# YHY138/Boosting-Fine-grained-Feature-Fusion-in-3D-Point-Cloud-Registration

Hardware: AMD Instinct MI355X
Metric: point-cloud pairs/sec (forward) on ModelNet 2048-pt pairs (higher is better)
Workload: dtype f32 (emulated on the fp16 MFMA pipe: f16x3 split products); 1 GPU; ModelNet40 2048-pt pairs, 8 pairs per GPU (BASELINE configs[1] at N=1, configs[3] at N=8); pairs_per_gpu=8, global_batch=8, points_per_cloud=717, parallelism=pair-sharded dp1, precision=fp32

## Files before the change

boosting-fine-grained-feature-fusion-in-3d-point-cloud-registration_amd/csrc/ffn.hip:

```cpp
#include <algorithm>
#include <cstdlib>

#include "mfma.h"

namespace fgr {
namespace {

constexpr int kFfnD = 256;
constexpr int kFfnKS = kFfnD / 32;
constexpr int kFfnNP = kFfnD / 16;
constexpr int kFfnMaxF = 2048;
constexpr int kUnit = 1024;
constexpr int kRing = 8;
static_assert(kFfnKS * 128 == kUnit, "a W1 panel is one ring unit");
static_assert(kFfnNP / 2 * 128 == kUnit, "half of a chunk's W2 slice is one ring unit");

struct FfnArgs {
    const float* x; int64_t ldx;
    const float* ln_g; const float* ln_b; float eps;
    const u32x4* w1; const float* wsc1; const float* b1;
    const u32x4* w2; const float* wsc2; const float* b2;
    const float* bound;
    float* out; int64_t ldo;
    int M, F;
};

__device__ __forceinline__ void wait_units(int n) {
    static_assert(kRing - 2 <= 6, "extend the switch");
    switch (n) {
        case 0: wait_vm_lgkm0<0>(); break;
        case 1: wait_vm_lgkm0<4>(); break;
        case 2: wait_vm_lgkm0<8>(); break;
        case 3: wait_vm_lgkm0<12>(); break;
        case 4: wait_vm_lgkm0<16>(); break;
        case 5: wait_vm_lgkm0<20>(); break;
        default: wait_vm_lgkm0<24>(); break;
    }
}

typedef __attribute__((address_space(3))) u32x4 lds_u4;

__shared__ u32x4 g_ffn_ring0[kUnit], g_ffn_ring1[kUnit], g_ffn_ring2[kUnit], g_ffn_ring3[kUnit],
                 g_ffn_ring4[kUnit], g_ffn_ring5[kUnit], g_ffn_ring6[kUnit], g_ffn_ring7[kUnit];
static_assert(kRing == 8, "one object per slot below");

__device__ __forceinline__ u32x4* ring_slot(int s) {
    switch (s & 7) {
        case 0: return g_ffn_ring0; case 1: return g_ffn_ring1;
        case 2: return g_ffn_ring2; case 3: return g_ffn_ring3;
        case 4: return g_ffn_ring4; case 5: return g_ffn_ring5;
        case 6: return g_ffn_ring6; default: return g_ffn_ring7;
    }
}

__device__ __forceinline__ void read_issue(const u32x4* slot, int lane_u, u32x4 (&r)[16]) {
    const uint32_t a = (uint32_t)(uintptr_t)((const lds_u4*)slot + lane_u);
    asm volatile(
        "ds_read_b128 %0, %16 offset:0\n\t"
        "ds_read_b128 %1, %16 offset:1024\n\t"
        "ds_read_b128 %2, %16 offset:2048\n\t"
        "ds_read_b128 %3, %16 offset:3072\n\t"
        "ds_read_b128 %4, %16 offset:4096\n\t"
        "ds_read_b128 %5, %16 offset:5120\n\t"
        "ds_read_b128 %6, %16 offset:6144\n\t"
        "ds_read_b128 %7, %16 offset:7168\n\t"
        "ds_read_b128 %8, %16 offset:8192\n\t"
        "ds_read_b128 %9, %16 offset:9216\n\t"
        "ds_read_b128 %10, %16 offset:10240\n\t"
        "ds_read_b128 %11, %16 offset:11264\n\t"
        "ds_read_b128 %12, %16 offset:12288\n\t"
        "ds_read_b128 %13, %16 offset:13312\n\t"
        "ds_read_b128 %14, %16 offset:14336\n\t"
        "ds_read_b128 %15, %16 offset:15360"
        : "=&v"(r[0]), "=&v"(r[1]), "=&v"(r[2]), "=&v"(r[3]), "=&v"(r[4]), "=&v"(r[5]),
          "=&v"(r[6]), "=&v"(r[7]), "=&v"(r[8]), "=&v"(r[9]), "=&v"(r[10]), "=&v"(r[11]),
          "=&v"(r[12]), "=&v"(r[13]), "=&v"(r[14]), "=&v"(r[15])
        : "v"(a)
        : "memory");
}
__device__ __forceinline__ void read_wait(u32x4 (&r)[16]) {
    asm volatile("s_waitcnt lgkmcnt(0)"
                 : "+v"(r[0]), "+v"(r[1]), "+v"(r[2]), "+v"(r[3]), "+v"(r[4]), "+v"(r[5]),
                   "+v"(r[6]), "+v"(r[7]), "+v"(r[8]), "+v"(r[9]), "+v"(r[10]), "+v"(r[11]),
                   "+v"(r[12]), "+v"(r[13]), "+v"(r[14]), "+v"(r[15])
                 :
                 : "memory");
}
__device__ __forceinline__ f16x8 frag(const u32x4 (&r)[16], int j, int t) {
    return __builtin_bit_cast(f16x8, r[2 * j + t]);
}

__global__ void __launch_bounds__(256, 1) ffn_f16x3_kernel(FfnArgs p) {
    __shared__ float4 cw1[kFfnMaxF / 4], cb1[kFfnMaxF / 4];
    __shared__ float4 cw2[kFfnD / 4], cb2[kFfnD / 4];
    __shared__ float4 lng[kFfnD / 4], lnb[kFfnD / 4];

    const int nbm = (p.M + 63) / 64;
    const int t = xcd_tile(blockIdx.x, nbm);
    const int tid = threadIdx.x, wv = tid >> 6, lane = tid & 63;
    const int g = lane >> 4, c = lane & 15;
    const int mw = t * 64 + wv * 16;
    const int64_t row = min(mw + c, p.M - 1);
    const int nch = p.F / 32;
    const int nu = 4 * nch;

    float xr[kFfnKS][8];
    {
        const float* ar = p.x + row * p.ldx;
#pragma unroll
        for (int s = 0; s < kFfnKS; ++s) {
            const float4 a0 = *reinterpret_cast<const float4*>(ar + 32 * s + 8 * g);
            const float4 a1 = *reinterpret_cast<const float4*>(ar + 32 * s + 8 * g + 4);
            xr[s][0] = a0.x; xr[s][1] = a0.y; xr[s][2] = a0.z; xr[s][3] = a0.w;
            xr[s][4] = a1.x; xr[s][5] = a1.y; xr[s][6] = a1.z; xr[s][7] = a1.w;
        }
    }
    const int nf4 = p.F / 4;
    static_assert(kFfnMaxF / 4 == 2 * 256, "two float4 per thread");
    const int j0 = min(tid, nf4 - 1), j1 = min(tid + 256, nf4 - 1);
    const float4 pw1a = reinterpret_cast<const float4*>(p.wsc1)[j0];
    const float4 pb1a = reinterpret_cast<const float4*>(p.b1)[j0];
    const float4 pw1b = reinterpret_cast<const float4*>(p.wsc1)[j1];
    const float4 pb1b = reinterpret_cast<const float4*>(p.b1)[j1];
    const int t4 = tid & (kFfnD / 4 - 1);
    const float4 pw2 = reinterpret_cast<const float4*>(p.wsc2)[t4];
    const float4 pb2 = reinterpret_cast<const float4*>(p.b2)[t4];
    const float4 pg = reinterpret_cast<const float4*>(p.ln_g)[t4];
    const float4 pbe = reinterpret_cast<const float4*>(p.ln_b)[t4];
    const float bM1 = p.bound[0], bMb = p.bound[1];

    auto unit_src = [&](int u) -> const u32x4* {
        const int ch = u >> 2, j = u & 3;
        return j < 2 ? p.w1 + (int64_t)(2 * ch + j) * kUnit
                     : p.w2 + (int64_t)ch * (2 * kUnit) + (j - 2) * kUnit;
    };
    auto dma = [&](int u, int slot) {
        const u32x4* src = unit_src(u) + wv * 64 + lane;
        __attribute__((address_space(3))) char* dst =
            (__attribute__((address_space(3))) char*)(lds_u4*)ring_slot(slot) + wv * 1024;
#pragma unroll
        for (int j = 0; j < 4; ++j)
            __builtin_amdgcn_global_load_lds((const void*)(src + j * 256),
                                             (__attribute__((address_space(3))) void*)(dst + j * 4096),
                                             16, 0, 0);
    };
#pragma unroll
    for (int u = 0; u < kRing; ++u) dma(u, u);
    wait_vm_lgkm0<4 * kRing>();
    if (tid < nf4) { cw1[tid] = pw1a; cb1[tid] = pb1a; }
    if (tid + 256 < nf4) { cw1[tid + 256] = pw1b; cb1[tid + 256] = pb1b; }
    if (tid < kFfnD / 4) { cw2[tid] = pw2; cb2[tid] = pb2; lng[tid] = pg; lnb[tid] = pbe; }
    wait_vm_lgkm0<4 * kRing - 4>();
    __builtin_amdgcn_s_barrier();
    const int lane_u = g * 16 + c;
    u32x4 wa[16], wb[16];
    read_issue(ring_slot(0), lane_u, wa);

    f16x8 af[kFfnKS][2];
    float rsS, inv_s;
    {
        float sm = 0.f;
#pragma unroll
        for (int s = 0; s < kFfnKS; ++s)
            sm += ((xr[s][0] + xr[s][1]) + (xr[s][2] + xr[s][3])) +
                  ((xr[s][4] + xr[s][5]) + (xr[s][6] + xr[s][7]));
        const float mean = xg_sum(sm) / (float)kFfnD;
        float sq = 0.f;
#pragma unroll
        for (int s = 0; s < kFfnKS; ++s)
#pragma unroll
            for (int e = 0; e < 8; ++e) {
                const float d = xr[s][e] - mean;
                sq += d * d;
            }
        const float rstd = 1.0f / sqrtf(xg_sum(sq) / (float)kFfnD + p.eps);
        float mx = 0.f, nn = 0.f;
#pragma unroll
        for (int s = 0; s < kFfnKS; ++s) {
            const int k = 32 * s + 8 * g;
            const float4 g0 = lng[k / 4], g1 = lng[k / 4 + 1];
            const float4 b0 = lnb[k / 4], b1 = lnb[k / 4 + 1];
            const float gg[8] = {g0.x, g0.y, g0.z, g0.w, g1.x, g1.y, g1.z, g1.w};
            const float bb[8] = {b0.x, b0.y, b0.z, b0.w, b1.x, b1.y, b1.z, b1.w};
#pragma unroll
            for (int e = 0; e < 8; ++e) {
                const float a = (xr[s][e] - mean) * rstd * gg[e] + bb[e];
                xr[s][e] = a;
                nn = fmaf(a, a, nn);
            }
            mx = fmaxf(mx, max3_abs(xr[s][0], xr[s][1], xr[s][2]));
            mx = fmaxf(mx, max3_abs(xr[s][3], xr[s][4], xr[s][5]));
            mx = fmaxf(mx, max3_abs(xr[s][6], xr[s][7], 0.f));
        }
        mx = xg_max(mx);
        nn = xg_sum(nn);
        const int ea = row_scale_exp(mx);
        const float sca = __builtin_ldexpf(1.f, ea);
#pragma unroll
        for (int s = 0; s < kFfnKS; ++s) {
            u32x4 h, l;
            split8_f16(xr[s], sca, h, l);
            af[s][0] = __builtin_bit_cast(f16x8, h);
            af[s][1] = __builtin_bit_cast(f16x8, l);
        }
        const float bnd = sqrtf(nn) * bM1 + bMb;
        const int eh = bnd > 0.f ? max(min(15 - __builtin_amdgcn_frexp_expf(bnd), 127), -126) : 0;
        rsS = __builtin_ldexpf(1.f, eh - ea);
        inv_s = __builtin_ldexpf(1.f, -eh);
    }
    const float sS = inv_s > 0.f ? 1.f / inv_s : 1.f;

    f32x4 accy[kFfnNP];
#pragma unroll
    for (int q = 0; q < kFfnNP; ++q) accy[q] = f32x4{0.f, 0.f, 0.f, 0.f};
    f32x4 acc1[2];
    f16x8 hb[2];
    read_wait(wa);
    for (int ch2 = 0; ch2 < nch; ch2 += 2) {
#pragma unroll
        for (int jj = 0; jj < 8; ++jj) {
            const int j = jj & 3, ch = ch2 + (jj >> 2);
            const int u = 4 * ch2 + jj;
            u32x4 (&cur)[16] = (jj & 1) ? wb : wa;
            u32x4 (&nxt)[16] = (jj & 1) ? wa : wb;
            const bool more = u + 1 < nu;
            if (more) {
                wait_units(min(kRing - 2, nu - 2 - u));
                __builtin_amdgcn_s_barrier();
                if (u + kRing < nu) dma(u + kRing, jj);
                read_issue(ring_slot(jj + 1), lane_u, nxt);
            }
            __builtin_amdgcn_sched_barrier(0);
            if (j < 2) {
                f32x4 a = f32x4{0.f, 0.f, 0.f, 0.f};
#pragma unroll
                for (int s = 0; s < kFfnKS; ++s) {
                    a = __builtin_amdgcn_mfma_f32_16x16x32_f16(frag(cur, s, 1), af[s][0], a, 0, 0, 0);
                    a = __builtin_amdgcn_mfma_f32_16x16x32_f16(frag(cur, s, 0), af[s][1], a, 0, 0, 0);
                    a = __builtin_amdgcn_mfma_f32_16x16x32_f16(frag(cur, s, 0), af[s][0], a, 0, 0, 0);
                }
                acc1[j] = a;
                if (j == 1) {
                    float hv[8];
#pragma unroll
                    for (int pp = 0; pp < 2; ++pp) {
                        const int n = 32 * ch + 16 * pp + 4 * g;
                        const float4 w4 = cw1[n / 4], b4 = cb1[n / 4];
                        hv[4 * pp + 0] = fmaxf(fmaf(acc1[pp][0], rsS * w4.x, sS * b4.x), 0.f);
                        hv[4 * pp + 1] = fmaxf(fmaf(acc1[pp][1], rsS * w4.y, sS * b4.y), 0.f);
                        hv[4 * pp + 2] = fmaxf(fmaf(acc1[pp][2], rsS * w4.z, sS * b4.z), 0.f);
                        hv[4 * pp + 3] = fmaxf(fmaf(acc1[pp][3], rsS * w4.w, sS * b4.w), 0.f);
                    }
                    u32x4 h, l;
                    split8_f16(hv, 1.f, h, l);
                    hb[0] = __builtin_bit_cast(f16x8, h);
                    hb[1] = __builtin_bit_cast(f16x8, l);
                }
            } else {
#pragma unroll
                for (int qq = 0; qq < 8; ++qq) {
                    const int q = 8 * (j - 2) + qq;
                    accy[q] = __builtin_amdgcn_mfma_f32_16x16x32_f16(frag(cur, qq, 1), hb[0], accy[q], 0, 0, 0);
                    accy[q] = __builtin_amdgcn_mfma_f32_16x16x32_f16(frag(cur, qq, 0), hb[1], accy[q], 0, 0, 0);
                    accy[q] = __builtin_amdgcn_mfma_f32_16x16x32_f16(frag(cur, qq, 0), hb[0], accy[q], 0, 0, 0);
                }
            }
            __builtin_amdgcn_sched_barrier(0);
            if (more) read_wait(nxt);
        }
    }

    const bool ok = mw + c < p.M;
    const float* xrow = p.x + row * p.ldx;
    float4 res[kFfnNP];
#pragma unroll
    for (int q = 0; q < kFfnNP; ++q) res[q] = *reinterpret_cast<const float4*>(xrow + 16 * q + 4 * g);
    float* orow = p.out + row * p.ldo;
#pragma unroll
    for (int q = 0; q < kFfnNP; ++q) {
        const int n = 16 * q + 4 * g;
        const float4 w4 = cw2[n / 4], b4 = cb2[n / 4];
        const float4 y = make_float4(fmaf(accy[q][0], w4.x * inv_s, b4.x) + res[q].x,
                                     fmaf(accy[q][1], w4.y * inv_s, b4.y) + res[q].y,
                                     fmaf(accy[q][2], w4.z * inv_s, b4.z) + res[q].z,
                                     fmaf(accy[q][3], w4.w * inv_s, b4.w) + res[q].w);
        if (ok) *reinterpret_cast<float4*>(orow + n) = y;
    }
}

constexpr int kV2Groups = 16;
constexpr int kCusFfn = 256;
#ifndef FGR_FFN_RING
#define FGR_FFN_RING 4
#endif
constexpr int kV2Ring = FGR_FFN_RING;
static_assert(kV2Groups % kV2Ring == 0, "ring slot = group index mod kV2Ring at compile time");

__device__ __forceinline__ void wait_vm_only(int n) {
    switch (n) {
        case 0: wait_vm<0>(); break;   case 4: wait_vm<4>(); break;
        case 8: wait_vm<8>(); break;   case 12: wait_vm<12>(); break;
        case 16: wait_vm<16>(); break; case 20: wait_vm<20>(); break;
        case 24: wait_vm<24>(); break; default: wait_vm<28>(); break;
    }
}

__device__ __forceinline__ float gelu_scaled(float sz, float isq) {
    const float a = sz * isq, t = fabsf(a), s = a * a;
    float r = fmaf(-1.72853470e-5f, t, 3.83197126e-4f);
    const float u = fmaf(-3.88396438e-3f, t, 2.42546219e-2f);
    r = fmaf(r, s, u);
    r = fmaf(r, t, -1.06777877e-1f);
    r = fmaf(r, t, -6.34846687e-1f);
    r = fmaf(r, t, -1.28717512e-1f);
    r = fmaf(r, t, -t);
    const float e = 0.5f * __expf(r);
    const float tail = a < 0.f ? e : 1.f - e;
    float q = -5.96761703e-4f;
    q = fmaf(q, s, 4.99119423e-3f);
    q = fmaf(q, s, -2.67681349e-2f);
    q = fmaf(q, s, 1.12819925e-1f);
    q = fmaf(q, s, -3.76125336e-1f);
    q = fmaf(q, s, 1.28379166e-1f);
    const float mid = fmaf(0.5f, fmaf(q, a, a), 0.5f);
    return sz * (t > 0.927734375f ? tail : mid);
}

template <int RT, int ACT = FGR_ACT_RELU>
__global__ void __launch_bounds__(256, 1) ffn_nsplit_kernel(FfnArgs p) {
    static_assert(RT >= 1 && RT <= 4, "row tiles");
    static_assert(ACT == FGR_ACT_RELU || ACT == FGR_ACT_GELU, "activation");
    __shared__ u32x4 act[RT * kFfnKS * 2 * 64];
    __shared__ u32x4 hbuf[2][4][RT][2][64];
    __shared__ float4 cw1[kFfnMaxF / 4], cb1[kFfnMaxF / 4];
    __shared__ float4 cw2[kFfnD / 4], cb2[kFfnD / 4];
    __shared__ float4 lng[kFfnD / 4], lnb[kFfnD / 4];
    __shared__ float2 rowpar[64];

    constexpr int BR = 16 * RT;
    const int nbm = (p.M + BR - 1) / BR;
    const int t = xcd_tile(blockIdx.x, nbm);
    const int tid = threadIdx.x, wv = tid >> 6, lane = tid & 63;
    const int g = lane >> 4, c = lane & 15;
    const int r0 = t * BR;
    const int nst = p.F / 128;

    const int nf4 = p.F / 4;
    const int j0 = min(tid, nf4 - 1), j1 = min(tid + 256, nf4 - 1);
    const float4 pw1a = reinterpret_cast<const float4*>(p.wsc1)[j0];
    const float4 pb1a = reinterpret_cast<const float4*>(p.b1)[j0];
    const float4 pw1b = reinterpret_cast<const float4*>(p.wsc1)[j1];
    const float4 pb1b = reinterpret_cast<const float4*>(p.b1)[j1];
    const int t4 = tid & (kFfnD / 4 - 1);
    const float4 pw2 = reinterpret_cast<const float4*>(p.wsc2)[t4];
    const float4 pb2 = reinterpret_cast<const float4*>(p.b2)[t4];
    const float4 pg = reinterpret_cast<const float4*>(p.ln_g)[t4];
    const float4 pbe = reinterpret_cast<const float4*>(p.ln_b)[t4];
    __builtin_amdgcn_sched_barrier(0);
    float xr[kFfnKS][8];
    {
        const int64_t row = min(r0 + 16 * min(wv, RT - 1) + c, p.M - 1);
        const float* ar = p.x + row * p.ldx;
#pragma unroll
        for (int s = 0; s < kFfnKS; ++s) {
            const float4 a0 = *reinterpret_cast<const float4*>(ar + 32 * s + 8 * g);
            const float4 a1 = *reinterpret_cast<const float4*>(ar + 32 * s + 8 * g + 4);
            xr[s][0] = a0.x; xr[s][1] = a0.y; xr[s][2] = a0.z; xr[s][3] = a0.w;
            xr[s][4] = a1.x; xr[s][5] = a1.y; xr[s][6] = a1.z; xr[s][7] = a1.w;
        }
    }
    {
        if (tid < nf4) { cw1[tid] = pw1a; cb1[tid] = pb1a; }
        if (tid + 256 < nf4) { cw1[tid + 256] = pw1b; cb1[tid + 256] = pb1b; }
        if (tid < kFfnD / 4) { cw2[tid] = pw2; cb2[tid] = pb2; lng[tid] = pg; lnb[tid] = pbe; }
    }
    const float bM1 = p.bound[0], bMb = p.bound[1];
    __syncthreads();

    {
        float sm = 0.f;
#pragma unroll
        for (int s = 0; s < kFfnKS; ++s)
            sm += ((xr[s][0] + xr[s][1]) + (xr[s][2] + xr[s][3])) +
                  ((xr[s][4] + xr[s][5]) + (xr[s][6] + xr[s][7]));
        const float mean = xg_sum(sm) / (float)kFfnD;
        float sq = 0.f;
#pragma unroll
        for (int s = 0; s < kFfnKS; ++s)
#pragma unroll
            for (int e = 0; e < 8; ++e) {
                const float d = xr[s][e] - mean;
                sq += d * d;
            }
        const float rstd = 1.0f / sqrtf(xg_sum(sq) / (float)kFfnD + p.eps);
        float mx = 0.f, nn = 0.f;
#pragma unroll
        for (int s = 0; s < kFfnKS; ++s) {
            const int k = 32 * s + 8 * g;
            const float4 g0 = lng[k / 4], g1 = lng[k / 4 + 1];
            const float4 b0 = lnb[k / 4], b1 = lnb[k / 4 + 1];
            const float gg[8] = {g0.x, g0.y, g0.z, g0.w, g1.x, g1.y, g1.z, g1.w};
            const float bb[8] = {b0.x, b0.y, b0.z, b0.w, b1.x, b1.y, b1.z, b1.w};
#pragma unroll
            for (int e = 0; e < 8; ++e) {
                const float a = (xr[s][e] - mean) * rstd * gg[e] + bb[e];
                xr[s][e] = a;
                nn = fmaf(a, a, nn);
            }
            mx = fmaxf(mx, max3_abs(xr[s][0], xr[s][1], xr[s][2]));
            mx = fmaxf(mx, max3_abs(xr[s][3], xr[s][4], xr[s][5]));
            mx = fmaxf(mx, max3_abs(xr[s][6], xr[s][7], 0.f));
        }
        mx = xg_max(mx);
        nn = xg_sum(nn);
        const int ea = row_scale_exp(mx);
        const float sca = __builtin_ldexpf(1.f, ea);
        if (wv < RT) {
#pragma unroll
            for (int s = 0; s < kFfnKS; ++s) {
                u32x4 h, l;
                split8_f16(xr[s], sca, h, l);
                act[((wv * kFfnKS + s) * 2 + 0) * 64 + lane] = h;
                act[((wv * kFfnKS + s) * 2 + 1) * 64 + lane] = l;
            }
        }
        const float bnd = sqrtf(nn) * bM1 + bMb;
        const int eh = bnd > 0.f ? max(min(15 - __builtin_amdgcn_frexp_expf(bnd), 127), -126) : 0;
        if (g == 0 && wv < RT)
            rowpar[16 * wv + c] = make_float2(__builtin_ldexpf(1.f, eh - ea), __builtin_ldexpf(1.f, eh));
    }
    __syncthreads();

    auto issue = [&](int st, int j, u32x4 (&slot)[4]) {
        if (j < 8) {
            const int ch = 4 * st + wv;
#pragma unroll
            for (int e = 0; e < 4; ++e) {
                const int pp = e >> 1, tt = e & 1;
                slot[e] = p.w1[(int64_t)(2 * ch + pp) * kUnit + (j * 2 + tt) * 64 + lane];
            }
        } else {
            const int ch = 4 * st + ((j - 8) >> 1), q0 = 4 * wv + 2 * ((j - 8) & 1);
#pragma unroll
            for (int e = 0; e < 4; ++e) {
                const int qq = e >> 1, tt = e & 1;
                slot[e] = p.w2[((int64_t)(ch * kFfnNP + q0 + qq) * 2 + tt) * 64 + lane];
            }
        }
    };
    u32x4 ring[kV2Ring][4];
    f32x4 accy[RT][4];
#pragma unroll
    for (int rt = 0; rt < RT; ++rt)
#pragma unroll
        for (int q = 0; q < 4; ++q) accy[rt][q] = f32x4{0.f, 0.f, 0.f, 0.f};
#pragma unroll
    for (int j = 0; j < kV2Ring - 1; ++j) issue(0, j, ring[j]);
    u32x4 fa[2][2 * RT];
    auto read_act = [&](int s, u32x4 (&f)[2 * RT]) {
#pragma unroll
        for (int rt = 0; rt < RT; ++rt) {
            f[2 * rt + 0] = act[((rt * kFfnKS + s) * 2 + 0) * 64 + lane];
            f[2 * rt + 1] = act[((rt * kFfnKS + s) * 2 + 1) * 64 + lane];
        }
    };
    auto read_h = [&](int buf, int sw, u32x4 (&f)[2 * RT]) {
#pragma unroll
        for (int rt = 0; rt < RT; ++rt) {
            f[2 * rt + 0] = hbuf[buf][sw][rt][0][lane];
            f[2 * rt + 1] = hbuf[buf][sw][rt][1][lane];
        }
    };

    for (int st = 0; st < nst; ++st) {
        const int ch = 4 * st + wv;
        const int stn = min(st + 1, nst - 1);
        f32x4 acc1[RT][2];
#pragma unroll
        for (int rt = 0; rt < RT; ++rt) acc1[rt][0] = acc1[rt][1] = f32x4{0.f, 0.f, 0.f, 0.f};
        read_act(0, fa[0]);
#pragma unroll
        for (int j = 0; j < kV2Groups; ++j) {
            const int jn = j + kV2Ring - 1;
            issue(jn < kV2Groups ? st : stn, jn % kV2Groups, ring[jn % kV2Ring]);
            wait_vm_only(4 * (kV2Ring - 1));
            u32x4 (&wf)[4] = ring[j % kV2Ring];
            if (j < 8) {
                u32x4 (&cur)[2 * RT] = fa[j & 1];
                if (j < 7) read_act(j + 1, fa[(j + 1) & 1]);
                __builtin_amdgcn_sched_group_barrier(0x020, 4, 0);
                if (j < 7) __builtin_amdgcn_sched_group_barrier(0x100, 2 * RT, 0);
#pragma unroll
                for (int rt = 0; rt < RT; ++rt) {
                    const f16x8 ah = __builtin_bit_cast(f16x8, cur[2 * rt + 0]);
                    const f16x8 al = __builtin_bit_cast(f16x8, cur[2 * rt + 1]);
#pragma unroll
                    for (int pp = 0; pp < 2; ++pp) {
                        const f16x8 wh = __builtin_bit_cast(f16x8, wf[2 * pp]);
                        const f16x8 wl = __builtin_bit_cast(f16x8, wf[2 * pp + 1]);
                        acc1[rt][pp] = __builtin_amdgcn_mfma_f32_16x16x32_f16(wl, ah, acc1[rt][pp], 0, 0, 0);
                        acc1[rt][pp] = __builtin_amdgcn_mfma_f32_16x16x32_f16(wh, al, acc1[rt][pp], 0, 0, 0);
                        acc1[rt][pp] = __builtin_amdgcn_mfma_f32_16x16x32_f16(wh, ah, acc1[rt][pp], 0, 0, 0);
                    }
                }
                __builtin_amdgcn_sched_group_barrier(0x008, 6 * RT, 0);
                __builtin_amdgcn_sched_barrier(0);
                if (j == 7) {
#pragma unroll
                    for (int rt = 0; rt < RT; ++rt) {
                        const float2 rp = rowpar[16 * rt + c];
                        float hv[8];
#pragma unroll
                        for (int pp = 0; pp < 2; ++pp) {
                            const int n = 32 * ch + 16 * pp + 4 * g;
                            const float4 w4 = cw1[n / 4], b4 = cb1[n / 4];
                            if constexpr (ACT == FGR_ACT_RELU) {
                                hv[4 * pp + 0] = fmaxf(fmaf(acc1[rt][pp][0], rp.x * w4.x, rp.y * b4.x), 0.f);
                                hv[4 * pp + 1] = fmaxf(fmaf(acc1[rt][pp][1], rp.x * w4.y, rp.y * b4.y), 0.f);
                                hv[4 * pp + 2] = fmaxf(fmaf(acc1[rt][pp][2], rp.x * w4.z, rp.y * b4.z), 0.f);
                                hv[4 * pp + 3] = fmaxf(fmaf(acc1[rt][pp][3], rp.x * w4.w, rp.y * b4.w), 0.f);
                            } else {
                                const float isq =
                                    __builtin_ldexpf(0.70710678118654752440f,
                                                     1 - __builtin_amdgcn_frexp_expf(rp.y));
                                hv[4 * pp + 0] = gelu_scaled(fmaf(acc1[rt][pp][0], rp.x * w4.x, rp.y * b4.x), isq);
                                hv[4 * pp + 1] = gelu_scaled(fmaf(acc1[rt][pp][1], rp.x * w4.y, rp.y * b4.y), isq);
                                hv[4 * pp + 2] = gelu_scaled(fmaf(acc1[rt][pp][2], rp.x * w4.z, rp.y * b4.z), isq);
                                hv[4 * pp + 3] = gelu_scaled(fmaf(acc1[rt][pp][3], rp.x * w4.w, rp.y * b4.w), isq);
                            }
                        }
                        u32x4 h, l;
                        split8_f16(hv, 1.f, h, l);
                        hbuf[st & 1][wv][rt][0][lane] = h;
                        hbuf[st & 1][wv][rt][1][lane] = l;
                    }
                    wait_lgkm0();
                    __builtin_amdgcn_s_barrier();
                    read_h(st & 1, 0, fa[0]);
                }
            } else {
                const int sw = (j - 8) >> 1, qh = (j - 8) & 1;
                u32x4 (&cur)[2 * RT] = fa[sw & 1];
                const bool pre = qh == 0 && sw < 3;
                if (pre) read_h(st & 1, sw + 1, fa[(sw + 1) & 1]);
                __builtin_amdgcn_sched_group_barrier(0x020, 4, 0);
                if (pre) __builtin_amdgcn_sched_group_barrier(0x100, 2 * RT, 0);
#pragma unroll
                for (int rt = 0; rt < RT; ++rt) {
                    const f16x8 hh = __builtin_bit_cast(f16x8, cur[2 * rt + 0]);
                    const f16x8 hl = __builtin_bit_cast(f16x8, cur[2 * rt + 1]);
#pragma unroll
                    for (int qq = 0; qq < 2; ++qq) {
                        const f16x8 wh = __builtin_bit_cast(f16x8, wf[2 * qq]);
                        const f16x8 wl = __builtin_bit_cast(f16x8, wf[2 * qq + 1]);
                        f32x4& a = accy[rt][2 * qh + qq];
                        a = __builtin_amdgcn_mfma_f32_16x16x32_f16(wl, hh, a, 0, 0, 0);
                        a = __builtin_amdgcn_mfma_f32_16x16x32_f16(wh, hl, a, 0, 0, 0);
                        a = __builtin_amdgcn_mfma_f32_16x16x32_f16(wh, hh, a, 0, 0, 0);
                    }
                }
                __builtin_amdgcn_sched_group_barrier(0x008, 6 * RT, 0);
                __builtin_amdgcn_sched_barrier(0);
            }
        }
    }
    wait_vm_only(0);

#pragma unroll
    for (int rt = 0; rt < RT; ++rt) {
        const int rr = r0 + 16 * rt + c;
        const int64_t row = min(rr, p.M - 1);
        const float inv_s = 1.f / rowpar[16 * rt + c].y;
        const float* xrow = p.x + row * p.ldx;
        float4 res[4];
#pragma unroll
        for (int q = 0; q < 4; ++q) res[q] = *reinterpret_cast<const float4*>(xrow + 16 * (4 * wv + q) + 4 * g);
        float* orow = p.out + row * p.ldo;
#pragma unroll
        for (int q = 0; q < 4; ++q) {
            const int n = 16 * (4 * wv + q) + 4 * g;
            const float4 w4 = cw2[n / 4], b4 = cb2[n / 4];
            const float4 y = make_float4(fmaf(accy[rt][q][0], w4.x * inv_s, b4.x) + res[q].x,
                                         fmaf(accy[rt][q][1], w4.y * inv_s, b4.y) + res[q].y,
                                         fmaf(accy[rt][q][2], w4.z * inv_s, b4.z) + res[q].z,
                                         fmaf(accy[rt][q][3], w4.w * inv_s, b4.w) + res[q].w);
            if (rr < p.M) *reinterpret_cast<float4*>(orow + n) = y;
        }
    }
}

__global__ void __launch_bounds__(256)
ffn_w2_split_kernel(const float* __restrict__ w, int n, int f, int64_t sn, int64_t sk,
                    float* __restrict__ wsc, u32x4* __restrict__ img) {
    const int tid = threadIdx.x, q = blockIdx.x, r0 = q * 16;
    const int ri = tid >> 4, kl = tid & 15;
    float mx = 0.f;
    if (r0 + ri < n)
        for (int j = kl; j < f; j += 16) mx = fmaxf(mx, fabsf(w[(int64_t)(r0 + ri) * sn + (int64_t)j * sk]));
    __shared__ float red[16][17];
    __shared__ float scale_inv[16];
    red[ri][kl] = mx;
    __syncthreads();
    if (tid < 16) {
        float m = 0.f;
#pragma unroll
        for (int z = 0; z < 16; ++z) m = fmaxf(m, red[tid][z]);
        const int e = row_scale_exp(m);
        const bool ok = r0 + tid < n;
        scale_inv[tid] = ok ? __builtin_ldexpf(1.f, e) : 0.f;
        wsc[r0 + tid] = ok ? __builtin_ldexpf(1.f, -e) : 0.f;
    }
    __syncthreads();
    const int np = (n + 15) / 16, units = (f / 32) * 128;
    for (int u = tid; u < units; u += 256) {
        const int i = u & 15, gg = (u >> 4) & 3, t = (u >> 6) & 1, cc = u >> 7;
        const int rr = r0 + i;
        const float sc = scale_inv[i];
        f16x8 out;
#pragma unroll
        for (int e = 0; e < 8; ++e) {
            const int col = 32 * cc + 16 * (e >> 2) + 4 * gg + (e & 3);
            const float v = rr < n ? w[(int64_t)rr * sn + (int64_t)col * sk] * sc : 0.f;
            const _Float16 h = (_Float16)v;
            out[e] = t == 0 ? h : (_Float16)(v - (float)h);
        }
        img[((int64_t)cc * np + q) * 128 + (u & 127)] = __builtin_bit_cast(u32x4, out);
    }
}

size_t ffn_image_bytes(int n, int f) { return (size_t)(f / 32) * ((n + 15) / 16) * 128 * 16; }

}
}

using namespace fgr;

extern "C" int fgr_split_weights_ffn2_bytes(int32_t n, int32_t k, size_t* bytes) {
    FGR_REQUIRE(bytes && n > 0 && k > 0 && k % 32 == 0,
                "fgr_split_weights_ffn2_bytes: bad arguments (n %d, k %d: k %% 32 == 0)", n, k);
    *bytes = ffn_image_bytes(n, k) + (size_t)((n + 15) / 16) * 16 * sizeof(float);
    return FGR_OK;
}

extern "C" int fgr_split_weights_ffn2(const float* w, int32_t n, int32_t k, int64_t stride_n,
                                      int64_t stride_k, void* img, void* stream) {
    FGR_REQUIRE(w && img && n > 0 && k > 0 && k % 32 == 0,
                "fgr_split_weights_ffn2: bad arguments (n %d, k %d)", n, k);
    FGR_REQUIRE((reinterpret_cast<uintptr_t>(img) & 15) == 0,
                "fgr_split_weights_ffn2: image not 16-B aligned");
    float* wsc = reinterpret_cast<float*>(static_cast<char*>(img) + ffn_image_bytes(n, k));
    hipLaunchKernelGGL(ffn_w2_split_kernel, dim3((unsigned)((n + 15) / 16)), dim3(256), 0,
                       as_stream(stream), w, n, k, stride_n, stride_k, wsc, (u32x4*)img);
    FGR_CHECK_LAUNCH("ffn_w2_split_kernel");
    return FGR_OK;
}

extern "C" int fgr_ffn_f16x3_supported(int32_t m, int32_t d, int32_t f) {
    return (m > 0 && d == kFfnD && f >= 64 && f % 64 == 0 && f <= kFfnMaxF) ? 1 : 0;
}

extern "C" int fgr_ffn_f16x3_act_supported(int32_t m, int32_t d, int32_t f, int32_t act) {
    if (act == FGR_ACT_RELU) return fgr_ffn_f16x3_supported(m, d, f);
    if (act == FGR_ACT_GELU) return (fgr_ffn_f16x3_supported(m, d, f) && f % 128 == 0) ? 1 : 0;
    return 0;
}

extern "C" int fgr_ffn_f16x3(const float* x, int64_t ldx, const float* gamma, const float* beta,
                             float eps, const void* w1_img, const float* b1, const void* w2_img,
                             const float* b2, const float* bound, float* out, int64_t ldo,
                             int32_t m, int32_t d, int32_t f, void* stream) {
    return fgr_ffn_f16x3_act(x, ldx, gamma, beta, eps, w1_img, b1, w2_img, b2, bound, out, ldo, m,
                             d, f, FGR_ACT_RELU, stream);
}

extern "C" int fgr_ffn_f16x3_act(const float* x, int64_t ldx, const float* gamma,
                                 const float* beta, float eps, const void* w1_img, const float* b1,
                                 const void* w2_img, const float* b2, const float* bound,
                                 float* out, int64_t ldo, int32_t m, int32_t d, int32_t f,
                                 int32_t act, void* stream) {
    FGR_REQUIRE(act == FGR_ACT_RELU || act == FGR_ACT_GELU,
                "fgr_ffn_f16x3_act: act %d (FGR_ACT_RELU or FGR_ACT_GELU)", act);
    FGR_REQUIRE(x && gamma && beta && w1_img && b1 && w2_img && b2 && bound && out && m >= 0 &&
                    ldx >= d && ldo >= d && eps >= 0.f,
                "fgr_ffn_f16x3: bad arguments");
    FGR_REQUIRE(m == 0 || fgr_ffn_f16x3_act_supported(m, d, f, act),
                "fgr_ffn_f16x3: d %d, hidden %d, act %d not supported (fgr_ffn_f16x3_act_supported)",
                d, f, act);
    const uintptr_t al = reinterpret_cast<uintptr_t>(x) | reinterpret_cast<uintptr_t>(gamma) |
                         reinterpret_cast<uintptr_t>(beta) | reinterpret_cast<uintptr_t>(w1_img) |
                         reinterpret_cast<uintptr_t>(b1) | reinterpret_cast<uintptr_t>(w2_img) |
                         reinterpret_cast<uintptr_t>(b2) | reinterpret_cast<uintptr_t>(out);
    FGR_REQUIRE((al & 15) == 0 && ldx % 4 == 0 && ldo % 4 == 0,
                "fgr_ffn_f16x3: operands must be 16-B aligned with row strides %% 4 == 0");
    FGR_REQUIRE(out + (size_t)m * ldo <= x || x + (size_t)m * ldx <= out || out == x,
                "fgr_ffn_f16x3: out overlaps x partially");
    if (m == 0) return FGR_OK;
    hipStream_t st = as_stream(stream);
    TimedCall timed_(st);
    const char* i1 = static_cast<const char*>(w1_img);
    const char* i2 = static_cast<const char*>(w2_img);
    FfnArgs a{x, ldx, gamma, beta, eps,
              (const u32x4*)i1, (const float*)(i1 + (size_t)(f / 16) * kFfnKS * 128 * 16), b1,
              (const u32x4*)i2, (const float*)(i2 + ffn_image_bytes(d, f)), b2,
              bound, out, ldo, m, f};
    const bool rt3 = (m + 47) / 48 <= kCusFfn && (m + 63) / 64 < kCusFfn;
    if (act == FGR_ACT_GELU) {
        const unsigned nb = (unsigned)((m + 47) / 48);
        hipLaunchKernelGGL((ffn_nsplit_kernel<3, FGR_ACT_GELU>), dim3(nb), dim3(256), 0, st, a);
    } else if (f % 128 == 0) {
        if (rt3)
            hipLaunchKernelGGL(ffn_nsplit_kernel<3>, dim3((unsigned)((m + 47) / 48)), dim3(256), 0, st, a);
        else
            hipLaunchKernelGGL(ffn_nsplit_kernel<4>, dim3((unsigned)((m + 63) / 64)), dim3(256), 0, st, a);
    } else
        hipLaunchKernelGGL(ffn_f16x3_kernel, dim3((unsigned)((m + 63) / 64)), dim3(256), 0, st, a);
    FGR_CHECK_LAUNCH("ffn_f16x3_kernel");
    return FGR_OK;
}
```

boosting-fine-grained-feature-fusion-in-3d-point-cloud-registration_amd/csrc/gemm_ws.hip:

```cpp
#include "mfma.h"


namespace fgr {
namespace {

constexpr int kWsKS = 8;
constexpr int kWsPanelU = kWsKS * 128;
#ifndef FGR_WS_RING
#define FGR_WS_RING 3
#endif
constexpr int kWsRing = FGR_WS_RING;
static_assert(kWsRing >= 2 && kWsRing <= 8, "vmcnt holds at most 63");
constexpr int kKvUnitsWs = 1024;
constexpr int kKvUnitVWs = 512;

struct WsArgs {
    const float* A; int64_t lda;
    const u32x4* W; const float* wsc; const float* bias;
    float* C; int64_t ldc;
    const float* R; int64_t ldr;
    int M, N;
    const float* ln_g; const float* ln_b; float eps;
    const float* add; int64_t ld_add;
    const float* g2; const float* b2; float* out2; int64_t ld_out2;
    char* kv_img; int2* kv_sc; int n_head, kv_col0;
};

__device__ __forceinline__ void wait_groups_ws(int n) {
    switch (n) {
        case 0: wait_vm<0>(); break;   case 1: wait_vm<8>(); break;
        case 2: wait_vm<16>(); break;  case 3: wait_vm<24>(); break;
        case 4: wait_vm<32>(); break;  case 5: wait_vm<40>(); break;
        case 6: wait_vm<48>(); break;  default: wait_vm<56>(); break;
    }
}

template <int NPW, int LNM, bool KV, bool RES, int ACT, int RT, int NPART>
__global__ void __launch_bounds__(256) __attribute__((amdgpu_waves_per_eu((NPART > 1 && !RES) ? 2 : 1)))
gemm_ws_kernel(WsArgs p) {
    static_assert(NPW % 4 == 0, "passes of 4 panels");
    static_assert(RT >= 1 && RT <= 4 && (!KV || RT == 4), "row tiles (K / V images: 64-row tiles)");
    constexpr int BR = 16 * RT;
    static_assert(!KV || (LNM >= 2 && !RES && ACT == FGR_ACT_NONE), "K / V images: the in_proj");
    constexpr int NPASS = NPW / 4;
    constexpr int N = 64 * NPW;
    constexpr bool kResEarly = RES && NPASS == 1;
    __shared__ u32x4 act[RT * kWsKS * 2 * 64];
    __shared__ float rowrs[BR];
    __shared__ float4 colw[N / 4], colb[N / 4];
    __shared__ float4 lng[LNM ? 64 : 1], lnb[LNM ? 64 : 1];
    __shared__ float4 lng2[LNM == 3 ? 64 : 1], lnb2[LNM == 3 ? 64 : 1];
    constexpr bool kSideLds = LNM == 3 && NPART == 1;
    __shared__ float4 side[kSideLds ? BR * 64 : 1];

    const int nblk = (p.M + BR - 1) / BR * NPART;
    int t = xcd_tile(blockIdx.x, nblk);
    const int part = t % NPART;
    t /= NPART;
    const int cb4 = part * (N / 4);
    const int tid = threadIdx.x, wv = tid >> 6, lane = tid & 63;
    const int g = lane >> 4, c = lane & 15;
    const int r0 = t * BR;
    const int rrow = r0 + 16 * min(wv, RT - 1) + c;
    const int64_t row = min(rrow, p.M - 1);
    const int pw0 = part * 4 * NPW + wv * NPW;

    float4 lpg = make_float4(0.f, 0.f, 0.f, 0.f), lpb = lpg, lpg2 = lpg, lpb2 = lpg;
    if constexpr (LNM > 0) {
        const int t4 = tid & 63;
        lpg = reinterpret_cast<const float4*>(p.ln_g)[t4];
        lpb = reinterpret_cast<const float4*>(p.ln_b)[t4];
        if constexpr (LNM == 3) {
            lpg2 = reinterpret_cast<const float4*>(p.g2)[t4];
            lpb2 = reinterpret_cast<const float4*>(p.b2)[t4];
        }
    }
    constexpr int NC4 = (N / 4 + 255) / 256;
    float4 pcw[NC4], pcb[NC4];
#pragma unroll
    for (int i = 0; i < NC4; ++i) {
        const int j = min(tid + 256 * i, N / 4 - 1);
        pcw[i] = reinterpret_cast<const float4*>(p.wsc)[cb4 + j];
        pcb[i] = p.bias ? reinterpret_cast<const float4*>(p.bias)[cb4 + j] : make_float4(0.f, 0.f, 0.f, 0.f);
    }
    __builtin_amdgcn_sched_barrier(0);
    float xr[kWsKS][8];
    float dr[LNM >= 2 ? kWsKS : 1][8];
    {
        const float* ar = p.A + row * p.lda;
#pragma unroll
        for (int s = 0; s < kWsKS; ++s) {
            const float4 a0 = *reinterpret_cast<const float4*>(ar + 32 * s + 8 * g);
            const float4 a1 = *reinterpret_cast<const float4*>(ar + 32 * s + 8 * g + 4);
            xr[s][0] = a0.x; xr[s][1] = a0.y; xr[s][2] = a0.z; xr[s][3] = a0.w;
            xr[s][4] = a1.x; xr[s][5] = a1.y; xr[s][6] = a1.z; xr[s][7] = a1.w;
        }
        if constexpr (LNM >= 2) {
            const float* dp = p.add + row * p.ld_add;
#pragma unroll
            for (int s = 0; s < kWsKS; ++s) {
                const float4 d0 = *reinterpret_cast<const float4*>(dp + 32 * s + 8 * g);
                const float4 d1 = *reinterpret_cast<const float4*>(dp + 32 * s + 8 * g + 4);
                dr[s][0] = d0.x; dr[s][1] = d0.y; dr[s][2] = d0.z; dr[s][3] = d0.w;
                dr[s][4] = d1.x; dr[s][5] = d1.y; dr[s][6] = d1.z; dr[s][7] = d1.w;
            }
        }
    }
    float4 rres[kResEarly ? RT : 1][4];
    if constexpr (kResEarly) {
        const int col0 = pw0 * 16;
#pragma unroll
        for (int rt = 0; rt < RT; ++rt) {
            const int64_t orow = min(r0 + 16 * rt + c, p.M - 1);
#pragma unroll
            for (int pp = 0; pp < 4; ++pp)
                rres[rt][pp] = *reinterpret_cast<const float4*>(p.R + orow * p.ldr + col0 + 16 * pp + 4 * g);
        }
    }
    __builtin_amdgcn_sched_barrier(0);
    auto issue = [&](int G, u32x4 (&slot)[8]) {
        const int pass = G / kWsKS, s = G % kWsKS;
#pragma unroll
        for (int e = 0; e < 8; ++e) {
            const int pp = e >> 1, tt = e & 1;
            slot[e] = p.W[(int64_t)(pw0 + 4 * pass + pp) * kWsPanelU + (s * 2 + tt) * 64 + lane];
        }
    };
    constexpr int NG = NPASS * kWsKS;
    u32x4 ring[kWsRing][8];
#pragma unroll
    for (int G = 0; G < kWsRing - 1; ++G) issue(G, ring[G]);
    __builtin_amdgcn_sched_barrier(0);

#pragma unroll
    for (int i = 0; i < NC4; ++i) {
        const int j = tid + 256 * i;
        if (j < N / 4) { colw[j] = pcw[i]; colb[j] = pcb[i]; }
    }
    float ln_mean = 0.f, ln_rstd = 0.f;
    if constexpr (LNM > 0) {
        if (tid < 64) { lng[tid] = lpg; lnb[tid] = lpb; }
        if constexpr (LNM == 3)
            if (tid < 64) { lng2[tid] = lpg2; lnb2[tid] = lpb2; }
        __syncthreads();
        float sm = 0.f;
#pragma unroll
        for (int s = 0; s < kWsKS; ++s)
            sm += ((xr[s][0] + xr[s][1]) + (xr[s][2] + xr[s][3])) +
                  ((xr[s][4] + xr[s][5]) + (xr[s][6] + xr[s][7]));
        const float mean = xg_sum(sm) / 256.f;
        float sq = 0.f;
#pragma unroll
        for (int s = 0; s < kWsKS; ++s)
#pragma unroll
            for (int e = 0; e < 8; ++e) {
                const float d = xr[s][e] - mean;
                sq += d * d;
            }
        const float rstd = 1.0f / sqrtf(xg_sum(sq) / 256.f + p.eps);
        ln_mean = mean;
        ln_rstd = rstd;
        if (kSideLds && wv < RT) {
#pragma unroll
            for (int s = 0; s < kWsKS; ++s) {
                const int k = 32 * s + 8 * g;
                const float4 h0 = lng2[k / 4], h1 = lng2[k / 4 + 1];
                const float4 c0 = lnb2[k / 4], c1 = lnb2[k / 4 + 1];
                float4* o2 = side + (16 * wv + c) * 64 + k / 4;
                o2[0] = make_float4((xr[s][0] - mean) * rstd * h0.x + c0.x, (xr[s][1] - mean) * rstd * h0.y + c0.y,
                                    (xr[s][2] - mean) * rstd * h0.z + c0.z, (xr[s][3] - mean) * rstd * h0.w + c0.w);
                o2[1] = make_float4((xr[s][4] - mean) * rstd * h1.x + c1.x, (xr[s][5] - mean) * rstd * h1.y + c1.y,
                                    (xr[s][6] - mean) * rstd * h1.z + c1.z, (xr[s][7] - mean) * rstd * h1.w + c1.w);
            }
        }
#pragma unroll
        for (int s = 0; s < kWsKS; ++s) {
            const int k = 32 * s + 8 * g;
            const float4 g0 = lng[k / 4], g1 = lng[k / 4 + 1];
            const float4 b0 = lnb[k / 4], b1 = lnb[k / 4 + 1];
            const float gg[8] = {g0.x, g0.y, g0.z, g0.w, g1.x, g1.y, g1.z, g1.w};
            const float bb[8] = {b0.x, b0.y, b0.z, b0.w, b1.x, b1.y, b1.z, b1.w};
#pragma unroll
            for (int e = 0; e < 8; ++e) {
                xr[s][e] = (xr[s][e] - mean) * rstd * gg[e] + bb[e];
                if constexpr (LNM >= 2) xr[s][e] += dr[s][e];
            }
        }
    }
    {
        float mx = 0.f;
#pragma unroll
        for (int s = 0; s < kWsKS; ++s) {
            mx = fmaxf(mx, max3_abs(xr[s][0], xr[s][1], xr[s][2]));
            mx = fmaxf(mx, max3_abs(xr[s][3], xr[s][4], xr[s][5]));
            mx = fmaxf(mx, max3_abs(xr[s][6], xr[s][7], 0.f));
        }
        mx = xg_max(mx);
        const int e = row_scale_exp(mx);
        const float sc = __builtin_ldexpf(1.f, e);
        if (wv < RT) {
#pragma unroll
            for (int s = 0; s < kWsKS; ++s) {
                u32x4 h, l;
                split8_f16(xr[s], sc, h, l);
                act[((wv * kWsKS + s) * 2 + 0) * 64 + lane] = h;
                act[((wv * kWsKS + s) * 2 + 1) * 64 + lane] = l;
            }
            if (g == 0) rowrs[16 * wv + c] = __builtin_ldexpf(1.f, -e);
        }
    }
    wait_lgkm0();
    __builtin_amdgcn_s_barrier();

    auto read_act = [&](int s, u32x4 (&f)[2 * RT]) {
#pragma unroll
        for (int rt = 0; rt < RT; ++rt) {
            f[2 * rt + 0] = act[((rt * kWsKS + s) * 2 + 0) * 64 + lane];
            f[2 * rt + 1] = act[((rt * kWsKS + s) * 2 + 1) * 64 + lane];
        }
    };
    u32x4 fa[2][2 * RT];
    u32x4 fin[NPASS][RT][4];
    int kv_e[NPASS][2];
    float rs[RT];
#pragma unroll
    for (int pass = 0; pass < NPASS; ++pass) {
        const int col0 = (pw0 + 4 * pass) * 16;
        const bool kvp = KV && col0 >= p.kv_col0;
        f32x4 acc[RT][4];
#pragma unroll
        for (int rt = 0; rt < RT; ++rt)
#pragma unroll
            for (int pp = 0; pp < 4; ++pp) acc[rt][pp] = f32x4{0.f, 0.f, 0.f, 0.f};
        read_act(0, fa[0]);
#pragma unroll
        for (int s = 0; s < kWsKS; ++s) {
            const int G = pass * kWsKS + s;
            if (G + kWsRing - 1 < NG) issue(G + kWsRing - 1, ring[(G + kWsRing - 1) % kWsRing]);
            wait_groups_ws(NG - 1 - G < kWsRing - 1 ? NG - 1 - G : kWsRing - 1);
            u32x4 (&wf)[8] = ring[G % kWsRing];
            u32x4 (&cur)[2 * RT] = fa[s & 1];
            if (s + 1 < kWsKS) read_act(s + 1, fa[(s + 1) & 1]);
            __builtin_amdgcn_sched_group_barrier(0x020, 8, 0);
            if (s + 1 < kWsKS) __builtin_amdgcn_sched_group_barrier(0x100, 2 * RT, 0);
#pragma unroll
            for (int rt = 0; rt < RT; ++rt) {
                const f16x8 ah = __builtin_bit_cast(f16x8, cur[2 * rt + 0]);
                const f16x8 al = __builtin_bit_cast(f16x8, cur[2 * rt + 1]);
#pragma unroll
                for (int pp = 0; pp < 4; ++pp) {
                    const f16x8 wh = __builtin_bit_cast(f16x8, wf[2 * pp]);
                    const f16x8 wl = __builtin_bit_cast(f16x8, wf[2 * pp + 1]);
                    acc[rt][pp] = __builtin_amdgcn_mfma_f32_16x16x32_f16(wl, ah, acc[rt][pp], 0, 0, 0);
                    acc[rt][pp] = __builtin_amdgcn_mfma_f32_16x16x32_f16(wh, al, acc[rt][pp], 0, 0, 0);
                    acc[rt][pp] = __builtin_amdgcn_mfma_f32_16x16x32_f16(wh, ah, acc[rt][pp], 0, 0, 0);
                }
            }
            __builtin_amdgcn_sched_group_barrier(0x008, 12 * RT, 0);
            __builtin_amdgcn_sched_barrier(0);
        }
        if (pass == 0)
#pragma unroll
            for (int rt = 0; rt < RT; ++rt) rs[rt] = rowrs[16 * rt + c];
        if (kvp) {
#pragma unroll
            for (int hh = 0; hh < 2; ++hh) {
                float y[4][2][4];
                float mx = 0.f;
#pragma unroll
                for (int pp = 0; pp < 2; ++pp) {
                    const int n = col0 + 32 * hh + 16 * pp + 4 * g;
                    const float4 ws = colw[n / 4 - cb4], bv = colb[n / 4 - cb4];
#pragma unroll
                    for (int rt = 0; rt < RT; ++rt) {
                        const bool ok = r0 + 16 * rt + c < p.M;
                        const f32x4 a = acc[rt][2 * hh + pp];
                        y[rt][pp][0] = ok ? a[0] * (rs[rt] * ws.x) + bv.x : 0.f;
                        y[rt][pp][1] = ok ? a[1] * (rs[rt] * ws.y) + bv.y : 0.f;
                        y[rt][pp][2] = ok ? a[2] * (rs[rt] * ws.z) + bv.z : 0.f;
                        y[rt][pp][3] = ok ? a[3] * (rs[rt] * ws.w) + bv.w : 0.f;
                        mx = fmaxf(mx, max3_abs(y[rt][pp][0], y[rt][pp][1], fmaxf(fabsf(y[rt][pp][2]), fabsf(y[rt][pp][3]))));
                    }
                }
                mx = xg_max(row16_max(mx));
                const int e = row_scale_exp(mx);
                kv_e[pass][hh] = e;
                const float sc = __builtin_ldexpf(1.f, e);
#pragma unroll
                for (int rt = 0; rt < RT; rt += 2)
#pragma unroll
                    for (int pp = 0; pp < 2; ++pp) {
                        const float v8[8] = {y[rt][pp][0], y[rt][pp][1], y[rt][pp][2], y[rt][pp][3],
                                             y[rt + 1][pp][0], y[rt + 1][pp][1], y[rt + 1][pp][2], y[rt + 1][pp][3]};
                        u32x4 h, l;
                        split8_f16(v8, sc, h, l);
                        fin[pass][rt][2 * hh + pp] = u32x4{h[0], h[1], l[0], l[1]};
                        fin[pass][rt + 1][2 * hh + pp] = u32x4{h[2], h[3], l[2], l[3]};
                    }
            }
        } else {
#pragma unroll
            for (int pp = 0; pp < 4; ++pp) {
                const int n = col0 + 16 * pp + 4 * g;
                const float4 ws = colw[n / 4 - cb4], bv = colb[n / 4 - cb4];
#pragma unroll
                for (int rt = 0; rt < RT; ++rt) {
                    float4 r4 = make_float4(0.f, 0.f, 0.f, 0.f);
                    if constexpr (kResEarly) r4 = rres[rt][pp];
                    const f32x4 a = acc[rt][pp];
                    constexpr int A1 = (RES && !kResEarly) ? FGR_ACT_NONE : ACT;
                    const float4 yv = make_float4(finish_ct<A1, kResEarly>(a[0] * (rs[rt] * ws.x), bv.x, r4.x),
                                                  finish_ct<A1, kResEarly>(a[1] * (rs[rt] * ws.y), bv.y, r4.y),
                                                  finish_ct<A1, kResEarly>(a[2] * (rs[rt] * ws.z), bv.z, r4.z),
                                                  finish_ct<A1, kResEarly>(a[3] * (rs[rt] * ws.w), bv.w, r4.w));
                    fin[pass][rt][pp] = __builtin_bit_cast(u32x4, yv);
                }
            }
        }
    }

#pragma unroll
    for (int pass = 0; pass < NPASS; ++pass) {
        const int col0 = (pw0 + 4 * pass) * 16;
        const bool kvp = KV && col0 >= p.kv_col0;
        if (kvp) {
#pragma unroll
            for (int hh = 0; hh < 2; ++hh) {
                const int hd = (col0 + 32 * hh - p.kv_col0) >> 5;
                const int isv = hd >= p.n_head ? 1 : 0, head = hd - isv * p.n_head;
                const int64_t tile = (int64_t)t * p.n_head + head;
                if (lane == 0) reinterpret_cast<int*>(p.kv_sc + tile)[isv] = kv_e[pass][hh];
                char* base = p.kv_img + tile * (kKvUnitsWs * 16);
#pragma unroll
                for (int rt = 0; rt < RT; ++rt) {
                    const int key = 16 * rt + c;
#pragma unroll
                    for (int pp = 0; pp < 2; ++pp) {
                        const int gq = 2 * pp + (g >> 1);
                        const u32x4 f = fin[pass][rt][2 * hh + pp];
#pragma unroll
                        for (int tt = 0; tt < 2; ++tt) {
                            char* dst;
                            if (isv)
                                dst = base + kKvUnitVWs * 16 + tt * (128 * 32) + key * 64 +
                                      (gq ^ (((key >> 2) & 1) << 1)) * 16 + 8 * (g & 1);
                            else
                                dst = base + ((tt * 4 + gq) * 64 + key) * 16 + 8 * (g & 1);
                            *reinterpret_cast<uint2*>(dst) = tt ? uint2{f[2], f[3]} : uint2{f[0], f[1]};
                        }
                    }
                }
            }
        } else {
#pragma unroll
            for (int rt = 0; rt < RT; ++rt) {
                const int rr = r0 + 16 * rt + c;
                if (rr < p.M) {
#pragma unroll
                    for (int pp = 0; pp < 4; ++pp) {
                        u32x4 v = fin[pass][rt][pp];
                        if constexpr (RES && !kResEarly) {
                            const float4 r4 = *reinterpret_cast<const float4*>(p.R + (int64_t)rr * p.ldr + col0 + 16 * pp + 4 * g);
                            const float4 y = __builtin_bit_cast(float4, v);
                            v = __builtin_bit_cast(u32x4, make_float4(finish_ct<ACT, true>(y.x, 0.f, r4.x),
                                                                      finish_ct<ACT, true>(y.y, 0.f, r4.y),
                                                                      finish_ct<ACT, true>(y.z, 0.f, r4.z),
                                                                      finish_ct<ACT, true>(y.w, 0.f, r4.w)));
                        }
                        *reinterpret_cast<u32x4*>(p.C + (int64_t)rr * p.ldc + col0 + 16 * pp + 4 * g) = v;
                    }
                }
            }
        }
    }
    if (LNM == 3 && !kSideLds && wv < RT) {
        const int s_lo = part * kWsKS / NPART, s_hi = (part + 1) * kWsKS / NPART;
        constexpr int SPP = (kWsKS + NPART - 1) / NPART;
        const float* ar = p.A + row * p.lda;
        float4 a0[SPP], a1[SPP];
#pragma unroll
        for (int j = 0; j < SPP; ++j) {
            const int kk = 32 * min(s_lo + j, kWsKS - 1) + 8 * g;
            a0[j] = *reinterpret_cast<const float4*>(ar + kk);
            a1[j] = *reinterpret_cast<const float4*>(ar + kk + 4);
        }
#pragma unroll
        for (int j = 0; j < SPP; ++j) {
            const int k = 32 * (s_lo + j) + 8 * g;
            if (s_lo + j < s_hi && rrow < p.M) {
                const float4 h0 = lng2[k / 4], h1 = lng2[k / 4 + 1];
                const float4 c0 = lnb2[k / 4], c1 = lnb2[k / 4 + 1];
                float* o2 = p.out2 + (int64_t)rrow * p.ld_out2 + k;
                *reinterpret_cast<float4*>(o2) = make_float4(
                    (a0[j].x - ln_mean) * ln_rstd * h0.x + c0.x, (a0[j].y - ln_mean) * ln_rstd * h0.y + c0.y,
                    (a0[j].z - ln_mean) * ln_rstd * h0.z + c0.z, (a0[j].w - ln_mean) * ln_rstd * h0.w + c0.w);
                *reinterpret_cast<float4*>(o2 + 4) = make_float4(
                    (a1[j].x - ln_mean) * ln_rstd * h1.x + c1.x, (a1[j].y - ln_mean) * ln_rstd * h1.y + c1.y,
                    (a1[j].z - ln_mean) * ln_rstd * h1.z + c1.z, (a1[j].w - ln_mean) * ln_rstd * h1.w + c1.w);
            }
        }
    }
    if (kSideLds) {
#pragma unroll
        for (int i = 0; i < 4 * RT; ++i) {
            const int u = tid + 256 * i;
            const int rr = r0 + (u >> 6);
            if (rr < p.M) *reinterpret_cast<float4*>(p.out2 + (int64_t)rr * p.ld_out2 + 4 * (u & 63)) = side[u];
        }
    }
}

constexpr int kCusWs = 256;
template <int NPW, int LNM, bool KV, bool RES, int ACT, int NPART = 1>
void launch_ws(const WsArgs& a, hipStream_t st) {
    if (!KV && (a.M + 47) / 48 <= kCusWs && (a.M + 63) / 64 < kCusWs)
        hipLaunchKernelGGL((gemm_ws_kernel<NPW, LNM, KV, RES, ACT, KV ? 4 : 3, NPART>),
                           dim3((unsigned)((a.M + 47) / 48 * NPART)), dim3(256), 0, st, a);
    else
        hipLaunchKernelGGL((gemm_ws_kernel<NPW, LNM, KV, RES, ACT, 4, NPART>),
                           dim3((unsigned)((a.M + 63) / 64 * NPART)), dim3(256), 0, st, a);
}

}

bool gemm_ws_supported(int m, int n, int k) {
    if (k != 256 || m < 4096) return false;
    return n == 256 || n == 768 || n == 512 || n == 1024;
}

bool gemm_ws_ln_supported(int m, int n, int k) {
    return (n == 256 || n == 768) && gemm_ws_supported(m, n, k);
}

bool gemm_ws_f16x3(const float* A, int64_t lda, const void* W, const float* wsc, float* C,
                   int64_t ldc, const float* bias, const float* R, int64_t ldr, int M, int N,
                   int K, int act, hipStream_t st, const WsLn* ln) {
    if (!gemm_ws_supported(M, N, K)) return false;
    if (ln && R) return false;
    if (act != FGR_ACT_NONE && act != FGR_ACT_RELU) return false;
    WsArgs a{A, lda, (const u32x4*)W, wsc, bias, C, ldc, R, ldr, M, N,
             ln ? ln->g : nullptr, ln ? ln->b : nullptr, ln ? ln->eps : 0.f,
             ln ? ln->add : nullptr, ln ? ln->ld_add : 0,
             ln ? ln->g2 : nullptr, ln ? ln->b2 : nullptr, ln ? ln->out2 : nullptr,
             ln ? ln->ld_out2 : 0, ln ? ln->kv_img : nullptr, ln ? ln->kv_sc : nullptr,
             ln ? ln->n_head : 0, ln ? ln->kv_col0 : N};
    const bool relu = act == FGR_ACT_RELU;
    if (N != 256 && N != 768) {
        if (ln) return false;
#define FGR_WS_PARTS(P)                                                                         \
        if (R) { if (relu) launch_ws<4, 0, false, true, FGR_ACT_RELU, P>(a, st);                \
                 else launch_ws<4, 0, false, true, FGR_ACT_NONE, P>(a, st); }                   \
        else if (relu) launch_ws<4, 0, false, false, FGR_ACT_RELU, P>(a, st);                   \
        else launch_ws<4, 0, false, false, FGR_ACT_NONE, P>(a, st);
        if (N == 512) { FGR_WS_PARTS(2) }
        else { FGR_WS_PARTS(4) }
#undef FGR_WS_PARTS
        return true;
    }
    if (N == 768) {
        if (!ln) {
            if (R) launch_ws<12, 0, false, true, FGR_ACT_NONE>(a, st);
            else if (relu) launch_ws<12, 0, false, false, FGR_ACT_RELU>(a, st);
            else launch_ws<12, 0, false, false, FGR_ACT_NONE>(a, st);
            return true;
        }
        if (ln->kv_img) {
            if (relu || !ln->add || ln->n_head * 64 + ln->kv_col0 != N || ln->kv_col0 != 256) return false;
            if (ln->out2) launch_ws<4, 3, true, false, FGR_ACT_NONE, 3>(a, st);
            else launch_ws<4, 2, true, false, FGR_ACT_NONE, 3>(a, st);
            return true;
        }
        if (relu) return false;
        if (ln->out2) launch_ws<12, 3, false, false, FGR_ACT_NONE>(a, st);
        else if (ln->add) launch_ws<12, 2, false, false, FGR_ACT_NONE>(a, st);
        else launch_ws<12, 1, false, false, FGR_ACT_NONE>(a, st);
        return true;
    }
    if (ln) return false;
    if (R) {
        if (relu) launch_ws<4, 0, false, true, FGR_ACT_RELU>(a, st);
        else launch_ws<4, 0, false, true, FGR_ACT_NONE>(a, st);
    } else {
        if (relu) launch_ws<4, 0, false, false, FGR_ACT_RELU>(a, st);
        else launch_ws<4, 0, false, false, FGR_ACT_NONE>(a, st);
    }
    return true;
}

}
```

boosting-fine-grained-feature-fusion-in-3d-point-cloud-registration_amd/fgreg/_lib.py:

```python
import ctypes
import os
import subprocess

HERE = os.path.dirname(os.path.abspath(__file__))
LIB_PATH = os.environ.get('FGREG_LIB_PATH') or os.path.join(HERE, 'libfgreg.so')
CSRC = os.path.join(os.path.dirname(HERE), 'csrc')

_vp = ctypes.c_void_p
_i32 = ctypes.c_int32
_i64 = ctypes.c_int64
_f32 = ctypes.c_float
_sz = ctypes.c_size_t

ABI_VERSION = 2

SIGNATURES = {
    'fgr_grid_subsample_workspace': [_i64, _i32, _i64, ctypes.POINTER(_sz)],
    'fgr_grid_subsample_count': [_vp, _vp, _i32, _i64, _f32, _i64, _vp, _sz, _vp, _vp],
    'fgr_grid_subsample_fill': [_i64, _i32, _i64, _i64, _vp, _sz, _vp, _vp, _vp, _vp],
    'fgr_grid_subsample_sparse_workspace': [_i64, _i32, ctypes.POINTER(_sz)],
    'fgr_grid_subsample_sparse_count': [_vp, _vp, _i32, _i64, _f32, _i32, _vp, _sz, _vp, _vp],
    'fgr_grid_subsample_sparse_fill': [_i64, _i32, _i64, _vp, _sz, _vp, _vp, _vp, _vp],
    'fgr_radius_grid_workspace': [_i64, _i32, ctypes.POINTER(_sz)],
    'fgr_radius_grid_build': [_vp, _vp, _i32, _i64, _f32, _vp, _sz, _vp],
    'fgr_radius_search_grid': [_vp, _vp, _i32, _i64, _i32, _vp, _vp, _i64, _vp, _sz, _f32, _i32,
                               _i32, _vp, _vp, _vp, _vp],
    'fgr_radius_count': [_vp, _vp, _vp, _vp, _i32, _i64, _i32, _f32, _vp, _vp, _vp],
    'fgr_radius_search': [_vp, _vp, _vp, _vp, _i32, _i64, _i64, _i32, _f32, _i32, _i32, _vp, _vp],
    'fgr_kpconv_gather_workspace': [_i64, _i32, ctypes.POINTER(_sz)],
    'fgr_kpconv_gather': [_vp, _vp, _i64, _i64, _vp, _i32, _vp, _i32, _vp, _i32, _f32, _vp, _vp,
                          _vp, _sz, _vp],
    'fgr_kpconv_gather_mode': [_vp, _vp, _i64, _i64, _vp, _i32, _vp, _i32, _vp, _i32, _f32, _i32,
                               _i32, _vp, _vp, _vp, _sz, _vp],
    'fgr_kpconv_deform_points': [_vp, _vp, _vp, _vp, _i64, _i32, _f32, _vp, _vp, _vp],
    'fgr_kpconv_gather_deform_workspace': [_i64, _i32, ctypes.POINTER(_sz)],
    'fgr_kpconv_gather_deform': [_vp, _vp, _i64, _i64, _vp, _i32, _vp, _i32, _vp, _vp, _i32, _f32,
                                 _i32, _i32, _vp, _vp, _vp, _sz, _vp],
    'fgr_kpconv_scatter_deform_workspace': [_i64, _i32, _i32, ctypes.POINTER(_sz)],
    'fgr_kpconv_scatter_deform': [_vp, _vp, _i64, _i64, _vp, _i32, _vp, _i32, _vp, _vp, _i32, _f32,
                                  _i32, _i32, _vp, _vp, _vp, _vp, _sz, _vp],
    'fgr_kpconv_deform_grad': [_vp, _vp, _i64, _i64, _vp, _i32, _vp, _i32, _vp, _vp, _vp, _i32,
                               _f32, _i32, _i32, _vp, _vp, _vp],
    'fgr_max_pool': [_vp, _i64, _i32, _vp, _i64, _i32, _vp, _vp],
    'fgr_instnorm_workspace': [_i64, _i32, _i32, ctypes.POINTER(_sz)],
    'fgr_instnorm': [_vp, _i64, _i32, _vp, _i32, _i64, _vp, _f32, _i32, _vp, _i32, _vp, _vp, _sz,
                     _vp],
    'fgr_layernorm': [_vp, _i64, _i32, _vp, _vp, _f32, _vp, _vp, _vp, _vp],
    'fgr_sine_pos_embed': [_vp, _i64, _i32, _f32, _f32, _vp, _vp],
    'fgr_add': [_vp, _vp, _i64, _vp, _vp],
    'fgr_layernorm_dual': [_vp, _i64, _i32, _vp, _vp, _vp, _vp, _vp, _vp, _vp, _vp, _f32, _vp],
    'fgr_attention': [_vp, _i64, _vp, _i64, _vp, _i64, _vp, _i64, _vp, _vp, _vp, _i32, _i32, _i32,
                      _i32, _f32, _vp],
    'fgr_attention_weights': [_vp, _i64, _vp, _i64, _vp, _i64, _vp, _vp, _vp, _i32, _i32, _i32, _i32,
                              _i32, _f32, _vp],
    'fgr_attention_f16x3_workspace': [_i64, _i32, _i32, ctypes.POINTER(_sz)],
    'fgr_attention_f16x3': [_vp, _i64, _vp, _i64, _vp, _i64, _vp, _i64, _vp, _vp, _vp, _i32, _i32,
                            _i64, _i32, _i32, _i32, _i32, _f32, _vp, _i64, _vp],
    'fgr_attention_f16x3_drop': [_vp, _i64, _vp, _i64, _vp, _i64, _vp, _i64, _vp, _vp, _vp, _i32,
                                 _i32, _i64, _i32, _i32, _i32, _i32, _f32, _vp, _i64,
                                 ctypes.c_uint32, _f32, _vp],
    'fgr_attention_f16x3_train': [_vp, _i64, _vp, _i64, _vp, _i64, _vp, _i64, _vp, _vp, _vp, _i32,
                                  _i32, _i64, _i32, _i32, _i32, _i32, _f32, _vp, _i64,
                                  ctypes.c_uint32, _f32, _vp, _vp],
    'fgr_attention_bf16_workspace': [_i64, _i32, _i32, ctypes.POINTER(_sz)],
    'fgr_attention_bf16': [_vp, _i64, _vp, _i64, _vp, _i64, _vp, _i64, _vp, _vp, _vp, _i32, _i32,
                           _i64, _i32, _i32, _i32, _i32, _f32, _vp, _i64, _vp],
    'fgr_res2net_chain6': [_vp, _i64, _i32, _i32, _vp, _vp, _vp, _i32, _vp, _i64, _vp],
    'fgr_res2net_chain_h3': [_vp, _i64, _i32, _i32, _vp, _vp, _vp, _vp, _i32, _vp, _i64, _vp],
    'fgr_res2net_block_h3': [_vp, _i64, _i32, _i32, _i32, _vp, _vp, _vp, _vp, _vp, _vp, _vp, _i64,
                             _vp],
    'fgr_res2net_block6': [_vp, _i64, _i32, _i32, _i32, _vp, _vp, _vp, _vp, _vp, _vp, _i64, _vp],
    'fgr_split_weights_h3_bytes': [_i32, _i32, ctypes.POINTER(_sz)],
    'fgr_split_weights_h3_batch': [_vp, _i32, _i64, _vp],
    'fgr_split_weights_h3': [_vp, _i32, _i32, _i64, _i64, _vp, _vp],
    'fgr_gemm_f16x3': [_vp, _i64, _vp, _vp, _i64, _vp, _vp, _i64, _i32, _i32, _i32, _i32, _vp],
    'fgr_gemm_f16x3_ln_supported': [_i32, _i32, _i32],
    'fgr_gemm_f16x3_ln': [_vp, _i64, _vp, _vp, _f32, _vp, _i64, _vp, _vp, _i64, _vp, _i32, _i32,
                          _i32, _i32, _vp],
    'fgr_gemm_f16x3_ln_out2': [_vp, _i64, _vp, _vp, _f32, _vp, _i64, _vp, _vp, _i64, _vp, _i32,
                               _i32, _i32, _i32, _vp, _vp, _vp, _i64, _vp],
    'fgr_split_weights_ffn2_bytes': [_i32, _i32, ctypes.POINTER(_sz)],
    'fgr_split_weights_ffn2': [_vp, _i32, _i32, _i64, _i64, _vp, _vp],
    'fgr_ffn_f16x3_supported': [_i32, _i32, _i32],
    'fgr_ffn_f16x3': [_vp, _i64, _vp, _vp, _f32, _vp, _vp, _vp, _vp, _vp, _vp, _i64, _i32, _i32,
                      _i32, _vp],
    'fgr_ffn_f16x3_act_supported': [_i32, _i32, _i32, _i32],
    'fgr_ffn_f16x3_act': [_vp, _i64, _vp, _vp, _f32, _vp, _vp, _vp, _vp, _vp, _vp, _i64, _i32,
                          _i32, _i32, _i32, _vp],
    'fgr_gelu_fwd': [_vp, _vp, _i64, _vp],
    'fgr_gelu_bwd': [_vp, _vp, _vp, _i64, _vp],
    'fgr_pos_mlp_f16x3_supported': [_i64, _i32],
    'fgr_pos_mlp_f16x3': [_vp, _i64, _vp, _vp, _vp, _vp, _vp, _vp, _vp, _vp, _vp, _vp, _i32, _vp,
                          _i64, _vp],
    'fgr_geo_embed_indices': [_vp, _i64, _vp, _i32, _i32, _f32, _f32, _vp, _vp, _vp, _vp],
    'fgr_geo_embed_f16x3_supported': [_i64, _i32, _i32],
    'fgr_geo_embed_f16x3': [_vp, _vp, _i64, _i32, _vp, _vp, _vp, _vp, _vp, _i32, _i32, _vp, _i64,
                            _vp],
    'fgr_split_weights_bf16_bytes': [_i32, _i32, ctypes.POINTER(_sz)],
    'fgr_split_weights_bf16': [_vp, _i32, _i32, _i64, _i64, _vp, _vp],
    'fgr_gemm_bf16': [_vp, _i64, _vp, _vp, _i64, _vp, _vp, _i64, _i32, _i32, _i32, _i32, _vp],
    'fgr_gemm_workspace': [_i32, _i32, _i32, _i32, ctypes.POINTER(_sz)],
    'fgr_gemm_f16x3_ws': [_vp, _i64, _vp, _vp, _i64, _vp, _vp, _i64, _i32, _i32, _i32, _i32, _vp,
                          _sz, _vp],
    'fgr_gemm_bf16_ws': [_vp, _i64, _vp, _vp, _i64, _vp, _vp, _i64, _i32, _i32, _i32, _i32, _vp,
                         _sz, _vp],
    'fgr_kv_image_bytes': [_i64, _i32, _i32, ctypes.POINTER(_sz)],
    'fgr_gemm_f16x3_ln_qkv_supported': [_i32, _i32, _i32],
    'fgr_gemm_f16x3_ln_qkv': [_vp, _i64, _vp, _vp, _f32, _vp, _i64, _vp, _vp, _i64, _vp, _i32, _i32,
                              _i32, _vp, _vp, _vp, _vp, _i64, _vp],
    'fgr_gemm_f16x3_qkv_supported': [_i32, _i32, _i32],
    'fgr_gemm_f16x3_qkv': [_vp, _i64, _vp, _vp, _i64, _vp, _i32, _i32, _i32, _vp, _vp],
    'fgr_kv_image_bf16_bytes': [_i64, _i32, _i32, ctypes.POINTER(_sz)],
    'fgr_gemm_bf16_qkv_supported': [_i32, _i32, _i32],
    'fgr_gemm_bf16_qkv': [_vp, _i64, _vp, _vp, _i64, _vp, _i32, _i32, _i32, _vp, _vp],
    'fgr_attention_bf16_img': [_vp, _i64, _vp, _i64, _vp, _i64, _vp, _vp, _vp, _i32, _i32, _i32,
                               _i32, _f32, _vp],
    'fgr_attention_f16x3_img': [_vp, _i64, _vp, _i64, _vp, _i64, _vp, _vp, _vp, _i32, _i32, _i32,
                                _i32, _f32, _vp],
    'fgr_corr_head_supported': [_i32, _i32],
    'fgr_corr_head_f16x3': [_vp, _i64, _i32, _i32, _vp, _vp, _vp, _vp, _vp, _vp, _vp, _vp, _vp, _vp],
    'fgr_copy_batch': [_i32, _vp, _vp, _vp, _vp],
    'fgr_lengths_to_offsets': [_vp, _i32, _vp, _vp],
    'fgr_overlap_pool': [_vp, _i64, _vp, _i64, _i32, _vp, _vp],
    'fgr_bce_logits_mean': [_vp, _i64, _vp, _i64, _vp, _vp],
    'fgr_transform_points': [_vp, _i64, _vp, _i32, _vp, _i32, _vp, _vp],
    'fgr_infonce_rows': [_vp, _i64, _vp, _vp, _vp, _vp, _i32, _i64, _f32, _f32, _vp, _vp, _vp],
    'fgr_infonce_reduce': [_vp, _vp, _vp, _i32, _vp, _vp],
    'fgr_infonce_rows_bwd': [_vp, _i64, _vp, _vp, _vp, _vp, _i32, _i64, _i64, _f32, _vp, _vp, _vp, _i64,
                             _vp],
    'fgr_circle_loss_workspace': [_i64, _i64, _i64, ctypes.POINTER(_sz)],
    'fgr_circle_loss': [_vp, _vp, _i32, _vp, _vp, _vp, _vp, _vp, _i32, _i64, _i64, _i32, _i32,
                        _i64, _f32, _f32, _vp, _sz, _vp, _vp],
    'fgr_pair_cdist': [_vp, _vp, _i32, _vp, _vp, _vp, _i32, _i32, _i32, _vp, _vp],
    'fgr_corr_loss': [_vp, _vp, _vp, _vp, _i32, _vp, _vp, _vp],
    'fgr_se3_compare': [_vp, _vp, _i32, _i32, _vp, _vp, _vp],
    'fgr_corr_attention': [_vp, _i64, _vp, _i64, _vp, _vp, _vp, _vp, _vp, _vp, _i32, _i32, _i32,
                           _f32, _vp],
    'fgr_corr_topk_workspace': [_i64, _i32, ctypes.POINTER(_sz)],
    'fgr_corr_topk_mask': [_vp, _i64, _vp, _i64, _vp, _vp, _vp, _vp, _i32, _i32, _i64, _i32, _i32,
                           _i32, _f32, _i32, _vp, _vp, _sz, _vp],
    'fgr_procrustes': [_vp, _vp, _vp, _i64, _i64, _f32, _vp, _vp],
    'fgr_time_next_call': [_vp, _vp],
    'fgr_pair_pose': [_vp, _vp, _vp, _i64, _vp, _i32, _i32, _f32, _vp, _vp],
    'fgr_nbr_inverse_workspace': [_i64, _i32, _i64, ctypes.POINTER(_sz)],
    'fgr_nbr_inverse': [_vp, _i64, _i32, _i64, _vp, _vp, _vp, _vp, _sz, _vp],
    'fgr_kpconv_scatter_workspace': [_i64, _i32, _i32, ctypes.POINTER(_sz)],
    'fgr_kpconv_scatter': [_vp, _vp, _i64, _i64, _vp, _i32, _vp, _i32, _vp, _i32, _f32, _vp, _vp,
                           _vp, _vp, _sz, _vp],
    'fgr_kpconv_scatter_mode': [_vp, _vp, _i64, _i64, _vp, _i32, _vp, _i32, _vp, _i32, _f32, _i32,
                                _i32, _vp, _vp, _vp, _vp, _sz, _vp],
    'fgr_max_pool_bwd_workspace': [_i64, _i32, ctypes.POINTER(_sz)],
    'fgr_max_pool_bwd': [_vp, _i64, _i32, _vp, _i64, _i32, _vp, _vp, _vp, _vp, _vp, _sz, _vp],
    'fgr_corr_attention_bwd_workspace': [_i64, ctypes.POINTER(_sz)],
    'fgr_corr_attention_bwd': [_vp, _i64, _vp, _i64, _vp, _vp, _vp, _i64, _vp, _i64, _vp, _vp, _vp,
                               _vp, _i32, _i32, _i64, _i32, _i32, _i32, _f32, _vp, _sz, _vp],
    'fgr_segnorm_workspace': [_i64, _i32, _i32, ctypes.POINTER(_sz)],
    'fgr_segnorm_stats': [_vp, _i64, _i32, _vp, _i32, _i64, _vp, _f32, _vp, _vp, _vp, _vp, _sz, _vp],
    'fgr_segnorm_apply': [_vp, _i64, _i32, _vp, _i32, _vp, _vp, _vp, _vp, _vp, _i32, _vp, _i32, _vp,
                          _vp],
    'fgr_segnorm_fwd': [_vp, _i64, _i32, _vp, _i32, _i64, _vp, _f32, _vp, _vp, _vp, _vp, _vp, _i32, _vp,
                        _i32, _vp, _vp, _sz, _vp],
    'fgr_segnorm_bwd': [_vp, _i64, _i32, _vp, _i32, _i64, _vp, _vp, _vp, _vp, _vp, _i32, _i32, _i32,
                        _vp, _vp, _vp, _vp, _vp, _vp, _vp, _sz, _vp],
    'fgr_colsum_workspace': [_i64, _i32, ctypes.POINTER(_sz)],
    'fgr_colsum': [_vp, _i64, _i32, _i64, _vp, _vp, _sz, _vp],
    'fgr_gemm_wgrad_workspace': [_i64, _i32, _i32, _i32, ctypes.POINTER(_sz)],
    'fgr_gemm_f16x3_wgrad': [_vp, _i64, _vp, _i64, _i64, _i32, _i32, _vp, _i64, _vp, _vp, _sz, _vp],
    'fgr_layernorm_bwd_workspace': [_i64, _i32, ctypes.POINTER(_sz)],
    'fgr_layernorm_bwd': [_vp, _i64, _i32, _vp, _f32, _vp, _vp, _vp, _vp, _sz, _vp],
    'fgr_attention_bwd_workspace': [_i64, _i32, ctypes.POINTER(_sz)],
    'fgr_attention_bwd': [_vp, _i64, _vp, _i64, _vp, _i64, _vp, _i64, _vp, _i64, _vp, _i64, _vp, _i64,
                          _vp, _i64, _vp, _vp, _vp, _i32, _i32, _i64, _i64, _i64, _i32, _i32, _f32,
                          _vp, _sz, _vp],
    'fgr_attention_bwd_drop': [_vp, _i64, _vp, _i64, _vp, _i64, _vp, _i64, _vp, _i64, _vp, _i64,
                               _vp, _i64, _vp, _i64, _vp, _vp, _vp, _i32, _i32, _i64, _i64, _i64,
                               _i32, _i32, _f32, _vp, _sz, ctypes.c_uint32, _f32, _vp],
    'fgr_attention_bwd_train': [_vp, _i64, _vp, _i64, _vp, _i64, _vp, _i64, _vp, _i64, _vp, _i64,
                                _vp, _i64, _vp, _i64, _vp, _vp, _vp, _i32, _i32, _i64, _i64, _i64,
                                _i32, _i32, _f32, _vp, _sz, ctypes.c_uint32, _f32, _vp, _i64, _vp],
    'fgr_attention_bwd_train_workspace': [_i64, _i32, _i64, _i32, _i32, _i32, ctypes.POINTER(_sz)],
    'fgr_modelnet_metrics_workspace': [_i32, _i32, ctypes.POINTER(_sz)],
    'fgr_modelnet_metrics': [_vp, _vp, _vp, _vp, _vp, _i32, _i32, _i32, _vp, _sz, _vp, _vp],
    'fgr_crop_max_points': [ctypes.POINTER(_i32)],
    'fgr_crop_pairs_mask': [_vp, _i32, _vp, _i32, _vp, _vp, _vp, _vp, _vp, _vp, _vp],
    'fgr_crop_pairs_assemble': [_vp, _i32, _vp, _i32, _vp, _vp, _vp, _vp, _vp, _i32, _vp, _vp, _vp,
                                _vp, _vp],
    'fgr_augment_workspace_bytes': [_i64, _i32, ctypes.POINTER(_sz)],
    'fgr_augment_pairs': [_vp, _i32, _vp, _i64, _vp, _vp, _i64, _vp, _vp, _vp, _vp, _vp, _vp, _i32,
                          _vp, _i32, _vp, _vp, _vp, _vp, _vp, _vp, _sz, _vp],
    'fgr_icp_workspace': [_i64, _i64, _i32, ctypes.POINTER(_sz)],
    'fgr_icp': [_vp, _vp, _i64, _vp, _vp, _i64, _i32, _i32, _vp, _f32, _i32, _f32, _f32, _vp, _sz,
                _vp, _vp, _vp, _vp, _vp],
    'fgr_registration_score': [_vp, _vp, _i64, _vp, _vp, _i64, _i32, _i32, _vp, _f32, _vp, _sz,
                               _vp, _vp, _vp, _vp, _vp, _vp],
}

NB_INDEX, NB_DIST = 0, 1
ACT_NONE, ACT_LEAKY, ACT_RELU, ACT_RELU_RES_LEAKY = 0, 1, 2, 3
ACT_GELU = 4

_lib = None


class FgrError(RuntimeError):
    pass


def build(jobs=8):
    subprocess.check_call(['make', '-s', '-C', CSRC, f'-j{jobs}'])


def load():
    global _lib
    if _lib is not None:
        return _lib
    if not os.path.exists(LIB_PATH):
        raise FgrError(f'{LIB_PATH} not built: run `make -C {CSRC}` (or __graft_entry__.build())')
    L = ctypes.CDLL(LIB_PATH)
    L.fgr_abi_version.restype = ctypes.c_int
    L.fgr_last_error.restype = ctypes.c_char_p
    if L.fgr_abi_version() != ABI_VERSION:
        raise FgrError(f'libfgreg ABI version mismatch: {LIB_PATH} has {L.fgr_abi_version()}, '
                       f'fgreg expects {ABI_VERSION} (rebuild: make -C {CSRC})')
    for name, argtypes in SIGNATURES.items():
        fn = getattr(L, name)
        fn.restype = ctypes.c_int
        fn.argtypes = argtypes
    _lib = L
    return L


def check(rc, name):
    if rc != 0:
        msg = load().fgr_last_error().decode(errors='replace')
        raise FgrError(f'{name} failed ({rc}): {msg}')


_WS_SIZES = {}


def ws_size(name, *args):
    key = (name,) + args
    v = _WS_SIZES.get(key)
    if v is None:
        nb = _sz(0)
        check(getattr(load(), name)(*args, nb), name)
        v = nb.value
        if len(_WS_SIZES) > 65536:
            _WS_SIZES.clear()
        _WS_SIZES[key] = v
    return v
```

boosting-fine-grained-feature-fusion-in-3d-point-cloud-registration_amd/fgreg/ops.py:

```python
import ctypes
import math
from typing import Optional, Sequence, Tuple

import torch

from . import _lib
from ._lib import (ACT_GELU, ACT_LEAKY, ACT_NONE, ACT_RELU, ACT_RELU_RES_LEAKY,
                   NB_DIST, NB_INDEX)


def _ptr(t):
    return None if t is None else t.data_ptr()


class KernelTimer:

    def __init__(self, names):
        self.names = set(names)
        self.events = {n: [] for n in names}
        self.work = {n: [] for n in names}
        self.labels = {n: [] for n in names}
        self.count = False
        self.pool = []
        self.lead_cycles = 0
# ... 584 lines not shown
    wp = torch.zeros((scale, kt * 16, cin), dtype=torch.float32, device=w1.device)
    wp[:, :w] = (w1 * sc[:, None]).reshape(scale, w, cin)
    hi = wp.to(torch.float16)
    lo = (wp - hi.float()).to(torch.float16)
    t = torch.stack([hi, lo], 0).reshape(2, scale * kt, 16, cin // 32, 4, 8)
    img = t.permute(1, 3, 0, 4, 2, 5).contiguous()
    return img, (1.0 / sc).contiguous()


def res2net_block_supported(w, cin, h3=True):
    if not h3:
        return (w, cin) == (224, 256)
    return w > 0 and w % 4 == 0 and ((w + 15) // 16, cin) in ((2, 32), (4, 64), (7, 128))


def res2net_block(x, w, scale, w1_img, w1_scale, b1, w_frag, bias, cat, w_scale=None):
    _dev(x, w1_img, w1_scale, b1, w_frag, w_scale, bias, cat)
    x = _c(x, torch.float32)
    n, cin = x.shape
    h3 = w_scale is not None
    if not res2net_block_supported(w, cin, h3):
        raise _lib.FgrError(f'res2net_block: no fused instance for w {w}, cin {cin}, '
                            f'{"f16x3" if h3 else "bf16x6"}')
    assert cat.shape[0] == n and cat.stride(1) == 1
    L = _lib.load()
    t0 = _begin('res2net', 'h3' if h3 else 'x6')
    work = 2 * n * w * w * (scale - 1) * (3 if h3 else 6) + 3 * 2 * n * cin * scale * w
    if h3:
        _lib.check(L.fgr_res2net_block_h3(
            _ptr(x), n, w, cin, scale, _ptr(w1_img), _ptr(w1_scale), _ptr(b1), _ptr(w_frag),
            _ptr(w_scale), _ptr(bias), _ptr(cat), cat.stride(0), _stream()),
            'fgr_res2net_block_h3')
    else:
        _lib.check(L.fgr_res2net_block6(
            _ptr(x), n, w, cin, scale, _ptr(w1_img), _ptr(w1_scale), _ptr(b1), _ptr(w_frag),
            _ptr(bias), _ptr(cat), cat.stride(0), _stream()), 'fgr_res2net_block6')
    _end('res2net', t0, work)
    return cat


ATTN_MODE = 'f16x3'


def attention(q, k, v, q_off, kv_off, kv_seg, max_q_len, n_head, out=None,
              max_kv_len=None, dropout=None, lse=None) -> torch.Tensor:
    _dev(q, k, v, q_off, kv_off, kv_seg)
    for t in (q, k, v):
        assert t.dtype == torch.float32 and t.dim() == 2 and t.stride(1) == 1
    d = q.shape[1]
    assert k.shape[1] == d and v.shape[1] == d and d % n_head == 0 and k.shape[0] == v.shape[0]
    dh = d // n_head
    if out is None:
        out = torch.empty((q.shape[0], d), dtype=torch.float32, device=q.device)
    n_seg = q_off.numel() - 1
    n_kv_seg = kv_off.numel() - 1
    assert kv_seg.dtype == torch.int32 and kv_seg.numel() == n_seg
    max_kv_len = max_q_len if max_kv_len is None else max_kv_len
    L = _lib.load()
    split = (dh in (32, 64)
             and all(t.stride(0) % 4 == 0 and t.data_ptr() % 16 == 0 for t in (q, k, v, out)))
    t0 = _begin('attention')
    if lse is not None:
        assert split and ATTN_MODE == 'f16x3' and lse.is_contiguous() and lse.shape == (q.shape[0], n_head)
        seed, p = (int(dropout[0]), float(dropout[1])) if dropout is not None else (0, 0.0)
        nb = _lib.ws_size('fgr_attention_f16x3_workspace', k.shape[0], n_kv_seg, n_head)
        ws = _workspace(q.device, nb)
        _lib.check(L.fgr_attention_f16x3_train(
            _ptr(q), q.stride(0), _ptr(k), k.stride(0), _ptr(v), v.stride(0), _ptr(out),
            out.stride(0), _ptr(q_off), _ptr(kv_off), _ptr(kv_seg), n_seg, n_kv_seg, k.shape[0],
            int(max_q_len), int(max_kv_len), n_head, dh, float(math.sqrt(1.0 / float(dh))),
            _ptr(ws), ws.numel(), seed & 0xFFFFFFFF, p, _ptr(lse), _stream()),
            'fgr_attention_f16x3_train')
    elif dropout is not None and float(dropout[1]) > 0.0:
        if not split:
            raise NotImplementedError('attention dropout needs head dim 32 / 64 and 16-B aligned '
                                      'rows')
        nb = _lib._sz(0)
        _lib.check(L.fgr_attention_f16x3_workspace(k.shape[0], n_kv_seg, n_head, nb),
                   'fgr_attention_f16x3_workspace')
        ws = _workspace(q.device, nb.value)
        _lib.check(L.fgr_attention_f16x3_drop(
            _ptr(q), q.stride(0), _ptr(k), k.stride(0), _ptr(v), v.stride(0), _ptr(out),
            out.stride(0), _ptr(q_off), _ptr(kv_off), _ptr(kv_seg), n_seg, n_kv_seg, k.shape[0],
            int(max_q_len), int(max_kv_len), n_head, dh, float(math.sqrt(1.0 / float(dh))),
            _ptr(ws), ws.numel(), int(dropout[0]) & 0xFFFFFFFF, float(dropout[1]), _stream()),
            'fgr_attention_f16x3_drop')
    elif split:
        name = 'fgr_attention_' + ATTN_MODE
        nb = _lib._sz(0)
        _lib.check(getattr(L, name + '_workspace')(k.shape[0], n_kv_seg, n_head, nb),
                   name + '_workspace')
        ws = _workspace(q.device, nb.value)
        _lib.check(getattr(L, name)(
            _ptr(q), q.stride(0), _ptr(k), k.stride(0), _ptr(v), v.stride(0), _ptr(out),
            out.stride(0), _ptr(q_off), _ptr(kv_off), _ptr(kv_seg), n_seg, n_kv_seg, k.shape[0],
            int(max_q_len), int(max_kv_len), n_head, dh, float(math.sqrt(1.0 / float(dh))),
            _ptr(ws), ws.numel(), _stream()), name)
    else:
        _lib.check(L.fgr_attention(_ptr(q), q.stride(0), _ptr(k), k.stride(0), _ptr(v),
                                   v.stride(0), _ptr(out), out.stride(0), _ptr(q_off),
                                   _ptr(kv_off), _ptr(kv_seg), n_seg, int(max_q_len), n_head,
                                   dh, float(math.sqrt(1.0 / float(dh))), _stream()),
                   'fgr_attention')
    _end('attention', t0, lambda: attention_flops(q_off, kv_off, kv_seg, d))
    return out


def attention_weights(q, k, q_off, kv_off, kv_seg, max_q_len, n_head, max_kv_len=None,
                      out=None) -> torch.Tensor:
    _dev(q, k, q_off, kv_off, kv_seg, out)
    for t in (q, k):
        assert t.dtype == torch.float32 and t.dim() == 2 and t.stride(1) == 1
    d = q.shape[1]
    assert k.shape[1] == d and d % n_head == 0
    dh = d // n_head
    n_seg = q_off.numel() - 1
    assert kv_seg.dtype == torch.int32 and kv_seg.numel() == n_seg
    max_kv_len = int(max_q_len if max_kv_len is None else max_kv_len)
    if out is None:
        out = torch.empty((q.shape[0], max_kv_len), dtype=torch.float32, device=q.device)
    assert (out.dtype == torch.float32 and out.dim() == 2 and out.shape[0] == q.shape[0]
            and out.shape[1] >= max_kv_len and (out.stride(1) == 1 or out.shape[1] <= 1))
    if q.shape[0] == 0 or max_kv_len == 0:
        return out[:, :max_kv_len]
    ld_w = out.stride(0) if out.shape[0] > 1 else max(out.stride(0), out.shape[1])
    t0 = _begin('attention_weights')
    _lib.check(_lib.load().fgr_attention_weights(
        _ptr(q), q.stride(0), _ptr(k), k.stride(0), _ptr(out), ld_w, _ptr(q_off), _ptr(kv_off),
        _ptr(kv_seg), n_seg, int(max_q_len), max_kv_len, n_head, dh,
        float(math.sqrt(1.0 / float(dh))), _stream()), 'fgr_attention_weights')
    _end('attention_weights', t0)
    return out[:, :max_kv_len] if out.shape[1] != max_kv_len else out


def attention_lse_ok(q, k, v, n_head) -> bool:
    dh = q.shape[1] // n_head
    return (ATTN_MODE == 'f16x3' and dh in (32, 64)
            and all(t.stride(0) % 4 == 0 and t.data_ptr() % 16 == 0 for t in (q, k, v)))


def copy_batch(srcs, dsts):
    n = len(srcs)
    if n == 0:
        return
    for a, b in zip(srcs, dsts):
        assert a.shape == b.shape and a.dtype == b.dtype and a.is_contiguous() and b.is_contiguous()
    _dev(*srcs, *dsts)
    arr = ctypes.c_void_p * n
    src = arr(*[t.data_ptr() for t in srcs])
    dst = arr(*[t.data_ptr() for t in dsts])
    nb = (ctypes.c_int64 * n)(*[t.numel() * t.element_size() for t in srcs])
    _lib.check(_lib.load().fgr_copy_batch(n, src, dst, nb, _stream()), 'fgr_copy_batch')


_WS = {}
_WS_RETIRED = []
_WS_SCOPE = None


class PrivateWorkspace:

    def __init__(self):
        self.bufs, self.retired, self._prev = {}, [], []

    def get(self, device, nbytes):
        buf = self.bufs.get(device)
        if buf is None or buf.numel() < nbytes:
            if buf is not None:
                self.retired.append(buf)
            buf = torch.empty(max(nbytes, 1 << 20), dtype=torch.uint8, device=device)
            self.bufs[device] = buf
        return buf

    def __enter__(self):
        global _WS_SCOPE
        self._prev.append(_WS_SCOPE)
        _WS_SCOPE = self
        return self

    def __exit__(self, *exc):
        global _WS_SCOPE
        _WS_SCOPE = self._prev.pop()
        return False


def scratch(device, nbytes):
    return torch.empty(nbytes, dtype=torch.uint8, device=device)


def _workspace(device, nbytes):
    if _WS_SCOPE is not None:
        return _WS_SCOPE.get(device, nbytes)
    key = (device, _raw_stream(device.index) if _raw_stream is not None and device.index is not None
           else torch.cuda.current_stream(device).cuda_stream)
    buf = _WS.get(key)
    if buf is None or buf.numel() < nbytes:
        if buf is not None:
            _WS_RETIRED.append(buf)
        buf = torch.empty(max(nbytes, 1 << 20), dtype=torch.uint8, device=device)
        _WS[key] = buf
    return buf


def attention_flops(q_off, kv_off, kv_seg, d):
    qo, ko, ks = q_off.tolist(), kv_off.tolist(), kv_seg.tolist()
    return sum(4 * (qo[i + 1] - qo[i]) * (ko[ks[i] + 1] - ko[ks[i]]) * d for i in range(len(ks)))


def ln_qkv_supported(m, d, n_head) -> bool:
    return bool(_lib.load().fgr_gemm_f16x3_ln_qkv_supported(int(m), int(d), int(n_head)))


def ln_qkv_attention(x, norm, w_img, bias, pos, q_off, kv_seg, max_len, n_head, side=None):
    _dev(x, bias, pos, q_off, kv_seg)
    n, d = x.shape
    x, pos = x.contiguous(), pos.contiguous()
    gamma, beta = norm.weight.contiguous(), norm.bias.contiguous()
    L = _lib.load()
    nb = _lib._sz(0)
    _lib.check(L.fgr_kv_image_bytes(n, n_head, d // n_head, nb), 'fgr_kv_image_bytes')
    img = _workspace(x.device, nb.value)
    q = torch.empty((n, d), dtype=torch.float32, device=x.device)
    g2 = b2 = out2 = None
    if side is not None:
        g2, b2, out2 = side[0].weight.contiguous(), side[0].bias.contiguous(), side[1]
        assert out2.shape == x.shape and out2.stride(1) == 1
    t0 = _begin('gemm', (n, 3 * d, d))
    _lib.check(L.fgr_gemm_f16x3_ln_qkv(
        _ptr(x), x.stride(0), _ptr(gamma), _ptr(beta), float(norm.eps), _ptr(pos), pos.stride(0),
        _ptr(w_img.img), _ptr(q), q.stride(0), _ptr(bias), n, d, n_head, _ptr(img), _ptr(g2),
        _ptr(b2), _ptr(out2), out2.stride(0) if out2 is not None else 0, _stream()),
        'fgr_gemm_f16x3_ln_qkv')
    _end('gemm', t0, 2 * n * 3 * d * d)
    o = torch.empty((n, d), dtype=torch.float32, device=x.device)
    t0 = _begin('attention')
    _lib.check(L.fgr_attention_f16x3_img(
        _ptr(q), q.stride(0), _ptr(img), n, _ptr(o), o.stride(0), _ptr(q_off), _ptr(q_off),
        _ptr(kv_seg), q_off.numel() - 1, int(max_len), n_head, d // n_head,
        float(math.sqrt(1.0 / float(d // n_head))), _stream()), 'fgr_attention_f16x3_img')
    _end('attention', t0, lambda: attention_flops(q_off, q_off, kv_seg, d))
    return o


def qkv_supported(m, d, n_head) -> bool:
    return bool(_lib.load().fgr_gemm_f16x3_qkv_supported(int(m), int(d), int(n_head)))


def qkv_bf16_supported(m, d, n_head) -> bool:
    return bool(_lib.load().fgr_gemm_bf16_qkv_supported(int(m), int(d), int(n_head)))


def qkv_attention(h, w_img, bias, q_off, kv_seg, max_len, n_head, mode='f16x3'):
    _dev(h, bias, q_off, kv_seg)
    n, d = h.shape
    h = h.contiguous()
    L = _lib.load()
    nb = _lib._sz(0)
    bytes_fn = 'fgr_kv_image_bytes' if mode == 'f16x3' else 'fgr_kv_image_bf16_bytes'
    _lib.check(getattr(L, bytes_fn)(n, n_head, d // n_head, nb), bytes_fn)
    img = _workspace(h.device, nb.value)
    q = torch.empty((n, d), dtype=torch.float32, device=h.device)
    t0 = _begin('gemm', (n, 3 * d, d))
    gemm_fn = 'fgr_gemm_f16x3_qkv' if mode == 'f16x3' else 'fgr_gemm_bf16_qkv'
    _lib.check(getattr(L, gemm_fn)(_ptr(h), h.stride(0), _ptr(w_img.img), _ptr(q), q.stride(0),
                                   _ptr(bias), n, d, n_head, _ptr(img), _stream()), gemm_fn)
    _end('gemm', t0, 2 * n * 3 * d * d)
    o = torch.empty((n, d), dtype=torch.float32, device=h.device)
    t0 = _begin('attention')
    attn_fn = 'fgr_attention_f16x3_img' if mode == 'f16x3' else 'fgr_attention_bf16_img'
    _lib.check(getattr(L, attn_fn)(
        _ptr(q), q.stride(0), _ptr(img), n, _ptr(o), o.stride(0), _ptr(q_off), _ptr(q_off),
        _ptr(kv_seg), q_off.numel() - 1, int(max_len), n_head, d // n_head,
        float(math.sqrt(1.0 / float(d // n_head))), _stream()), attn_fn)
    _end('attention', t0, lambda: attention_flops(q_off, q_off, kv_seg, d))
    return o


FFN_FUSE = True


def ffn_supported(m, d, f, act=ACT_RELU) -> bool:
    return FFN_FUSE and bool(_lib.load().fgr_ffn_f16x3_act_supported(m, d, f, act))


def ffn(x, norm, w1_img, b1, w2_img, b2, bound, out=None, act=ACT_RELU) -> torch.Tensor:
    _dev(x, b1, b2, bound)
    m, d = x.shape
    f = b1.numel()
    assert x.dtype == torch.float32 and x.stride(1) == 1 and b2.numel() == d
    x = x if (x.stride(0) % 4 == 0 and x.data_ptr() % 16 == 0) else x.contiguous()
    g, b = norm.weight.contiguous(), norm.bias.contiguous()
    b1, b2, bound = b1.contiguous(), b2.contiguous(), bound.contiguous()
    if out is None:
        out = torch.empty((m, d), dtype=torch.float32, device=x.device)
    t0 = _begin('gemm', ('ffn', m, d, f))
    _lib.check(_lib.load().fgr_ffn_f16x3_act(
        _ptr(x), x.stride(0), _ptr(g), _ptr(b), float(norm.eps), _ptr(w1_img.img), _ptr(b1),
        _ptr(w2_img.img), _ptr(b2), _ptr(bound), _ptr(out), out.stride(0), m, d, f, int(act),
        _stream()), 'fgr_ffn_f16x3_act')
    _end('gemm', t0, 4 * m * d * f)
    return out


def gelu(z, out=None) -> torch.Tensor:
    _dev(z, out)
    assert z.dtype == torch.float32 and z.is_contiguous()
    if out is None:
        out = torch.empty_like(z)
    assert out.dtype == torch.float32 and out.is_contiguous() and out.shape == z.shape
    _lib.check(_lib.load().fgr_gelu_fwd(_ptr(z), _ptr(out), z.numel(), _stream()), 'fgr_gelu_fwd')
    return out


def gelu_(z) -> torch.Tensor:
    return gelu(z, out=z)


def gelu_backward(z, dy, out=None) -> torch.Tensor:
    _dev(z, dy, out)
    assert z.dtype == torch.float32 and z.is_contiguous()
    dy = _c(dy, torch.float32)
    assert dy.shape == z.shape
    if out is None:
        out = torch.empty_like(z)
    assert out.dtype == torch.float32 and out.is_contiguous() and out.shape == z.shape
    _lib.check(_lib.load().fgr_gelu_bwd(_ptr(z), _ptr(dy), _ptr(out), z.numel(), _stream()),
               'fgr_gelu_bwd')
    return out


def pos_mlp_supported(n, d) -> bool:
    return bool(_lib.load().fgr_pos_mlp_f16x3_supported(int(n), int(d)))


def pos_mlp(xyz, w0, b0, imgs, biases, out=None) -> torch.Tensor:
    _dev(xyz, w0, b0, *biases)
    xyz = _c(xyz, torch.float32)
    n, d = xyz.shape[0], biases[3].numel()
    assert xyz.dim() == 2 and xyz.shape[1] == 3 and len(imgs) == 4 and len(biases) == 4
    w0, b0 = _c(w0, torch.float32), _c(b0, torch.float32)
    assert w0.shape == (32, 3) and b0.numel() == 32
    biases = [_c(b, torch.float32) for b in biases]
    if out is None:
        out = torch.empty((n, d), dtype=torch.float32, device=xyz.device)
    assert out.shape == (n, d) and out.dtype == torch.float32 and (n == 0 or out.stride(1) == 1)
    t0 = _begin('gemm', ('pos_mlp', n, d))
    _lib.check(_lib.load().fgr_pos_mlp_f16x3(
        _ptr(xyz), n, _ptr(w0), _ptr(b0), _ptr(imgs[0].img), _ptr(biases[0]), _ptr(imgs[1].img),
        _ptr(biases[1]), _ptr(imgs[2].img), _ptr(biases[2]), _ptr(imgs[3].img), _ptr(biases[3]),
        d, _ptr(out), out.stride(0) if n > 1 else max(out.stride(0), d), _stream()),
        'fgr_pos_mlp_f16x3')
    _end('gemm', t0, 2 * n * (3 * 32 + 32 * 64 + 64 * 128 + 128 * 256 + 256 * d))
    return out


GEO_MAX, GEO_MEAN = 0, 1
GEO_MAX_K = 4


def geo_embed_indices(xyz, cloud_off, k, sigma_d, sigma_a):
    _dev(xyz, cloud_off)
    xyz = _c(xyz, torch.float32)
    cloud_off = _c(cloud_off, torch.int64)
    n, k = xyz.shape[0], int(k)
    assert xyz.dim() == 2 and xyz.shape[1] == 3 and cloud_off.dim() == 1
    if not 1 <= k <= GEO_MAX_K:
        raise _lib.FgrError(f'geo_embed_indices: k {k} not supported (1..{GEO_MAX_K})')
    nn = torch.empty((n, k), dtype=torch.int32, device=xyz.device)
    d = torch.empty((n, k), dtype=torch.float32, device=xyz.device)
    a = torch.empty((n, k, k), dtype=torch.float32, device=xyz.device)
    factor_a = 180.0 / (float(sigma_a) * math.pi)
    _lib.check(_lib.load().fgr_geo_embed_indices(
        _ptr(xyz), n, _ptr(cloud_off), cloud_off.numel() - 1, k, float(sigma_d), factor_a,
        _ptr(nn), _ptr(d), _ptr(a), _stream()), 'fgr_geo_embed_indices')
    return nn, d, a


def geo_embed_supported(n, d_model, k) -> bool:
    return bool(_lib.load().fgr_geo_embed_f16x3_supported(int(n), int(d_model), int(k)))


def geo_embed(d, a, div_term, img_d, bias_d, img_a, bias_a, reduction, out=None) -> torch.Tensor:
    _dev(d, a, div_term, bias_d, bias_a)
    d, a = _c(d, torch.float32), _c(a, torch.float32)
    n, k = d.shape
    assert a.shape == (n, k, k)
    div_term = _c(div_term, torch.float32)
    bias_d, bias_a = _c(bias_d, torch.float32), _c(bias_a, torch.float32)
    D = bias_d.numel()
    assert bias_a.numel() == D and div_term.numel() * 2 == D
    assert (img_d.n, img_d.k) == (D, D) and (img_a.n, img_a.k) == (D, D)
    if out is None:
        out = torch.empty((n, D), dtype=torch.float32, device=d.device)
    assert out.shape == (n, D) and out.dtype == torch.float32 and (n == 0 or out.stride(1) == 1)
    rows = n * k * (1 + k)
    t0 = _begin('gemm', ('geo_embed', n, D, k))
    _lib.check(_lib.load().fgr_geo_embed_f16x3(
        _ptr(d), _ptr(a), n, k, _ptr(div_term), _ptr(img_d.img), _ptr(bias_d), _ptr(img_a.img),
        _ptr(bias_a), D, int(reduction), _ptr(out),
        out.stride(0) if n > 1 else max(out.stride(0), D), _stream()), 'fgr_geo_embed_f16x3')
    _end('gemm', t0, 2 * rows * D * D)
    return out


def corr_head_supported(m, d) -> bool:
    return bool(_lib.load().fgr_corr_head_supported(int(m), int(d)))


def corr_head(f, img0c, b0c, img2, b2, w4, b4):
    _dev(f, b0c, b2, w4, b4)
    m, d = f.shape
    assert f.stride(1) == 1 and f.stride(0) % 4 == 0 and f.data_ptr() % 16 == 0
    w4, b4 = _c(w4, torch.float32), _c(b4, torch.float32)
    assert w4.shape == (3, d) and b0c.numel() == d + 16 and b2.numel() == d
    hidden = _workspace(f.device, 4 * m * d)
    corr = torch.empty((m, 3), dtype=torch.float32, device=f.device)
    logits = torch.empty((m, 1), dtype=torch.float32, device=f.device)
    t0 = _begin('gemm', (m, 2 * d + 16, d))
    _lib.check(_lib.load().fgr_corr_head_f16x3(
        _ptr(f), f.stride(0), m, d, _ptr(img0c.img), _ptr(_c(b0c, torch.float32)), _ptr(img2.img),
        _ptr(_c(b2, torch.float32)), _ptr(w4), _ptr(b4), _ptr(hidden), _ptr(corr), _ptr(logits),
        _stream()), 'fgr_corr_head_f16x3')
    _end('gemm', t0, 2 * m * (d + 16) * d + 2 * m * d * d + 6 * m * d)
    return corr, logits


def corr_attention(q, k, xyz, q_off, kv_off, kv_seg, v_off, max_q_len, scale) -> torch.Tensor:
    _dev(q, k, xyz, q_off, kv_off, kv_seg, v_off)
    for t in (q, k):
        assert t.dtype == torch.float32 and t.dim() == 2 and t.stride(1) == 1
    xyz = _c(xyz, torch.float32)
    d = q.shape[1]
    assert k.shape[1] == d and xyz.dim() == 2 and xyz.shape[1] == 3
    assert kv_seg.dtype == torch.int32 and kv_seg.numel() == q_off.numel() - 1
    out = torch.empty((q.shape[0], 3), dtype=torch.float32, device=q.device)
    t0 = _begin('attention')
    _lib.check(_lib.load().fgr_corr_attention(
        _ptr(q), q.stride(0), _ptr(k), k.stride(0), _ptr(xyz), _ptr(out), _ptr(q_off),
        _ptr(kv_off), _ptr(kv_seg), _ptr(v_off), q_off.numel() - 1, int(max_q_len), d,
        float(scale), _stream()), 'fgr_corr_attention')
    _end('attention', t0, lambda: attention_flops(q_off, kv_off, kv_seg, d) // 2)
    return out


def corr_topk_mask(corr, q, k, q_off, kv_off, kv_seg, n_clouds, max_q_len, max_kv_len, scale,
                   n_top) -> torch.Tensor:
    _dev(corr, q, k, q_off, kv_off, kv_seg)
    for t in (q, k):
        assert t.dtype == torch.float32 and t.dim() == 2 and t.stride(1) == 1
    assert corr.dtype == torch.float32 and corr.is_contiguous() and corr.shape == (q.shape[0], 3)
    d = q.shape[1]
    flags = torch.empty((2, max_kv_len), dtype=torch.uint8, device=q.device)
    L = _lib.load()
    nb = _lib._sz(0)
    _lib.check(L.fgr_corr_topk_workspace(q.shape[0], max_kv_len, nb), 'fgr_corr_topk_workspace')
    ws = scratch(q.device, max(nb.value, 1))
    _lib.check(L.fgr_corr_topk_mask(
        _ptr(q), q.stride(0), _ptr(k), k.stride(0), _ptr(corr), _ptr(q_off), _ptr(kv_off),
        _ptr(kv_seg), q_off.numel() - 1, n_clouds, q.shape[0], int(max_q_len), int(max_kv_len), d,
        float(scale), int(n_top), _ptr(flags), _ptr(ws), nb.value, _stream()), 'fgr_corr_topk_mask')
    return flags


def procrustes(a, b, w, threshold=0.85) -> torch.Tensor:
    _dev(a, b, w)
    lead = a.shape[:-2]
    n = a.shape[-2]
    a2 = _c(a, torch.float32).reshape(-1, n, 3)
    b2 = _c(b, torch.float32).reshape(-1, n, 3)
    w2 = _c(w, torch.float32).reshape(-1, n)
    out = torch.empty((a2.shape[0], 3, 4), dtype=torch.float32, device=a.device)
    thr = -1.0 if threshold is None else float(threshold)
    _lib.check(_lib.load().fgr_procrustes(_ptr(a2), _ptr(b2), _ptr(w2), a2.shape[0], n, thr,
                                          _ptr(out), _stream()), 'fgr_procrustes')
    return out.reshape(*lead, 3, 4)


def pair_pose(xyz, corr, logits, seg_off, n_pairs, threshold=0.85) -> torch.Tensor:
    _dev(xyz, corr, logits, seg_off)
    xyz, corr, logits = (_c(t, torch.float32) for t in (xyz, corr, logits))
    n_layers, n_tot = corr.shape[0], corr.shape[1]
    assert xyz.shape == (n_tot, 3) and logits.shape == (n_layers, n_tot)
    assert seg_off.numel() == 2 * n_pairs + 1
    out = torch.empty((n_layers, n_pairs, 3, 4), dtype=torch.float32, device=xyz.device)
    t0 = _begin('pose')
    _lib.check(_lib.load().fgr_pair_pose(_ptr(xyz), _ptr(corr), _ptr(logits), n_tot,
                                         _ptr(seg_off), n_pairs, n_layers, float(threshold),
                                         _ptr(out), _stream()), 'fgr_pair_pose')
    _end('pose', t0, n_layers * (28 * n_tot + 48 * n_pairs))
    return out
```

boosting-fine-grained-feature-fusion-in-3d-point-cloud-registration_amd/fgreg/transformer.py:

```python
import copy
import math

import torch
import torch.nn as nn

from . import linear as lin
from . import ops
from .linear import linear, linear_ln, ln_fusable

class Segments:

    def __init__(self, lengths, device, n_layers=0, phantoms=None):
        self.lengths = [int(n) for n in lengths]
        n = len(self.lengths)
        assert n % 2 == 0
        self.B = n // 2
        self.phantoms = [int(p) for p in phantoms] if phantoms is not None else [0] * n
        assert len(self.phantoms) == n and min(self.phantoms, default=0) >= 0
        self.seg_cloud = list(range(n)) + [c for c in range(n) if self.phantoms[c] > 0]
        self.seg_lengths = self.lengths + [p for p in self.phantoms if p > 0]
        self.n_phantom = sum(self.phantoms)
        self.off = ops.offsets(self.seg_lengths, device)
        self.cloud_off = self.off[:n + 1]
        self.self_seg = ops.to_device(self.seg_cloud, torch.int32, device)
        self.cross_seg = ops.to_device([(c + self.B) % n for c in self.seg_cloud], torch.int32,
                                       device)
        self.max_len = max(self.seg_lengths) if n else 0
        self.layer_tables = None
        if n_layers:
            N = sum(self.seg_lengths)
            S = len(self.seg_lengths)
            host_off = [0]
            for ln in self.seg_lengths[:-1]:
                host_off.append(host_off[-1] + ln)
            q_off = [l * N + o for l in range(n_layers) for o in host_off]
            q_off.append(n_layers * N)
            kv_seg = [l * S + (c + self.B) % n for l in range(n_layers) for c in self.seg_cloud]
            v_off = host_off * n_layers
            self.layer_tables = (ops.to_device(q_off, torch.int64, device),
                                 ops.to_device(kv_seg, torch.int32, device),
                                 ops.to_device(v_off, torch.int64, device))


class _QKTap(nn.Module):

    def forward(self, q, k):
        return q, k


class TransformerCrossEncoderLayer(nn.Module):

    def __init__(self, d_model, nhead, dim_feedforward=2048, dropout=0.1, activation='relu',
                 normalize_before=False, sa_val_has_pos_emb=False, ca_val_has_pos_emb=False,
                 attention_type='dot_prod'):
        super().__init__()
        if attention_type != 'dot_prod':
            raise NotImplementedError(attention_type)
        if activation == 'glu':
            raise NotImplementedError(
                "transformer_act 'glu': the reference's own F.glu halves the hidden width "
                '(dim_feedforward -> dim_feedforward / 2), so the reference itself fails in '
                'linear2; there is nothing to reproduce')
        if activation not in ('relu', 'gelu'):
            raise RuntimeError(f'transformer_act must be relu or gelu, not {activation!r}')
        self.activation = activation
        self.act = ops.ACT_GELU if activation == 'gelu' else ops.ACT_RELU
        self.self_attn = nn.MultiheadAttention(d_model, nhead, dropout=dropout)
        self.multihead_attn = nn.MultiheadAttention(d_model, nhead, dropout=dropout)
        self.linear1 = nn.Linear(d_model, dim_feedforward)
        self.linear2 = nn.Linear(dim_feedforward, d_model)
        self.norm1 = nn.LayerNorm(d_model)
        self.norm2 = nn.LayerNorm(d_model)
        self.norm3 = nn.LayerNorm(d_model)
        self.nhead = nhead
        self.normalize_before = normalize_before
        self.sa_val_has_pos_emb = sa_val_has_pos_emb
        self.ca_val_has_pos_emb = ca_val_has_pos_emb
        self.satt_weights, self.xatt_weights = None, None
        self.in_proj_tap = _QKTap()

    def _attention(self, q, k, v, seg, kv_seg, record):
        if record is not None:
            q, k = self.in_proj_tap(q, k)
            record.append(ops.attention_weights(q, k, seg.off, seg.off, kv_seg, seg.max_len,
                                                self.nhead))
        return ops.attention(q, k, v, seg.off, seg.off, kv_seg, seg.max_len, self.nhead)

    def _attend(self, mha, h_pos, h_nopos, val_has_pos, seg, kv_seg, ln=None, side=None,
                record=None):
        W, b = mha.in_proj_weight, mha.in_proj_bias
        if ln is not None:
            x, norm, pos = ln
            d = x.shape[1]
            if (record is None and lin.MODE == 'f16x3' and ops.ATTN_MODE == 'f16x3'
                    and pos is not None and ops.ln_qkv_supported(x.shape[0], d, self.nhead)
                    and (side is None or side[0].eps == norm.eps)):
                return ops.ln_qkv_attention(x, norm, lin.weight_image(W, mode='f16x3'), b, pos,
                                            seg.off, kv_seg, seg.max_len, self.nhead, side=side)
            qkv = linear_ln(x, norm, W, b, add=pos, side=side)
            q, k, v = qkv[:, :d], qkv[:, d:2 * d], qkv[:, 2 * d:]
            return self._attention(q, k, v, seg, kv_seg, record)
        d = h_pos.shape[1]
        if (record is None and val_has_pos and lin.MODE == 'f16x3' and ops.ATTN_MODE == 'f16x3'
                and ops.qkv_supported(h_pos.shape[0], d, self.nhead)):
            return ops.qkv_attention(h_pos, lin.weight_image(W, mode='f16x3'), b, seg.off, kv_seg,
                                     seg.max_len, self.nhead)
        if (record is None and val_has_pos and lin.MODE == 'bf16' and ops.ATTN_MODE == 'bf16'
                and ops.qkv_bf16_supported(h_pos.shape[0], d, self.nhead)):
            return ops.qkv_attention(h_pos, lin.weight_image(W, mode='bf16'), b, seg.off, kv_seg,
                                     seg.max_len, self.nhead, mode='bf16')
        if val_has_pos:
            qkv = linear(h_pos, W, b)
            q, k, v = qkv[:, :d], qkv[:, d:2 * d], qkv[:, 2 * d:]
        else:
            qk = linear(h_pos, W, b[:2 * d], rows=(0, 2 * d))
            q, k = qk[:, :d], qk[:, d:]
            v = linear(h_nopos, W, b[2 * d:], rows=(2 * d, 3 * d))
        return self._attention(q, k, v, seg, kv_seg, record)

    def _store_maps(self, packed, seg):
        B, lens = seg.B, seg.lengths
        start = [0]
        for n in lens:
            start.append(start[-1] + n)

        def padded(w, cross):
            sides = []
            for s in (0, 1):
                clouds = range(s * B, (s + 1) * B)
                keys = [(c + B) % (2 * B) if cross else c for c in clouds]
                t = w.new_zeros((B, max(lens[c] for c in clouds), max(lens[c] for c in keys)))
                for b, (c, kc) in enumerate(zip(clouds, keys)):
                    t[b, :lens[c], :lens[kc]] = w[start[c]:start[c + 1], :lens[kc]]
                sides.append(t)
            return tuple(sides)

        self.satt_weights = padded(packed[0], False)
        self.xatt_weights = padded(packed[1], True)

    def takes_side(self, x, pos):
        n, d = x.shape
        return (self.normalize_before and self.sa_val_has_pos_emb and pos is not None
                and ln_fusable(n, 3 * d, d))

    def wants_h1(self, x):
        n, d = x.shape
        return (self.normalize_before and self.sa_val_has_pos_emb
                and not ln_fusable(n, 3 * d, d))

    def forward_packed(self, x, pos, seg: Segments, pending_bias=None, h1=None, side=None,
                       record=False):
        if not self.normalize_before:
            return self._forward_post(x, pos, seg, pending_bias, record), None
        rec = [] if record else None
        n, d = x.shape
        fuse_in = ln_fusable(n, 3 * d, d)
        if fuse_in and self.sa_val_has_pos_emb and pending_bias is None:
            o = self._attend(self.self_attn, None, None, True, seg, seg.self_seg,
                             ln=(x, self.norm1, pos), side=side, record=rec)
            side = None
        elif h1 is not None:
            assert pending_bias is None and self.sa_val_has_pos_emb
            o = self._attend(self.self_attn, h1, None, True, seg, seg.self_seg, record=rec)
        else:
            if side is not None:
                ops.layernorm(x, side[0].weight, side[0].bias, side[0].eps, out=side[1])
                side = None
            h = ops.layernorm(x, self.norm1.weight, self.norm1.bias, self.norm1.eps, add=pos,
                              pre_bias=pending_bias)
            h0 = None if self.sa_val_has_pos_emb else ops.layernorm(
                x, self.norm1.weight, self.norm1.bias, self.norm1.eps)
            o = self._attend(self.self_attn, h, h0, self.sa_val_has_pos_emb, seg, seg.self_seg,
                             record=rec)
        x = linear(o, self.self_attn.out_proj.weight, self.self_attn.out_proj.bias, residual=x)
        if fuse_in and self.ca_val_has_pos_emb:
            o = self._attend(self.multihead_attn, None, None, True, seg, seg.cross_seg,
                             ln=(x, self.norm2, pos), record=rec)
        else:
            h = ops.layernorm(x, self.norm2.weight, self.norm2.bias, self.norm2.eps, add=pos)
            h0 = None if self.ca_val_has_pos_emb else ops.layernorm(
                x, self.norm2.weight, self.norm2.bias, self.norm2.eps)
            o = self._attend(self.multihead_attn, h, h0, self.ca_val_has_pos_emb, seg,
                             seg.cross_seg, record=rec)
        if rec is not None:
            self._store_maps(rec, seg)
        x = linear(o, self.multihead_attn.out_proj.weight, self.multihead_attn.out_proj.bias,
                   residual=x)
        if lin.MODE == 'f16x3' and ops.ffn_supported(n, d, self.linear1.out_features, self.act):
            return ops.ffn(x, self.norm3, lin.weight_image(self.linear1.weight, mode='f16x3'),
                           self.linear1.bias, lin.weight_image(self.linear2.weight, mode='ffn2'),
                           self.linear2.bias, self._ffn_bound(), act=self.act), None
        if self.act == ops.ACT_GELU:
            h = ops.gelu_(linear_ln(x, self.norm3, self.linear1.weight, self.linear1.bias))
        else:
            h = linear_ln(x, self.norm3, self.linear1.weight, self.linear1.bias, act=ops.ACT_RELU)
        return linear(h, self.linear2.weight, self.linear2.bias, residual=x), None

    def _ffn_bound(self):
        w, b = self.linear1.weight, self.linear1.bias
        key = (w.data_ptr(), w._version, b.data_ptr(), b._version)
        st = self.__dict__.get('_ffn_bound_cache')
        if st is None or st[0] != key:
            with torch.no_grad():
                bound = torch.stack([w.detach().norm(dim=1).max(),
                                     b.detach().abs().max()]).float().contiguous()
            st = (key, bound)
            self.__dict__['_ffn_bound_cache'] = st
            ops.note_state(bound)
        return st[1]

    def _forward_post(self, x, pos, seg: Segments, pending_bias=None, record=False):
        assert pending_bias is None
        rec = [] if record else None
        h = ops.add(x, pos)
        o = self._attend(self.self_attn, h, x, self.sa_val_has_pos_emb, seg, seg.self_seg,
                         record=rec)
        t = linear(o, self.self_attn.out_proj.weight, self.self_attn.out_proj.bias, residual=x)
        x = ops.layernorm(t, self.norm1.weight, self.norm1.bias, self.norm1.eps)
        h = ops.layernorm(t, self.norm1.weight, self.norm1.bias, self.norm1.eps, add=pos)
        o = self._attend(self.multihead_attn, h, x, self.ca_val_has_pos_emb, seg, seg.cross_seg,
                         record=rec)
        if rec is not None:
            self._store_maps(rec, seg)
        t = linear(o, self.multihead_attn.out_proj.weight, self.multihead_attn.out_proj.bias,
                   residual=x)
        x = ops.layernorm(t, self.norm2.weight, self.norm2.bias, self.norm2.eps)
        if self.act == ops.ACT_GELU:
            h = ops.gelu_(linear(x, self.linear1.weight, self.linear1.bias))
        else:
            h = linear(x, self.linear1.weight, self.linear1.bias, act=ops.ACT_RELU)
        t = linear(h, self.linear2.weight, self.linear2.bias, residual=x)
        return ops.layernorm(t, self.norm3.weight, self.norm3.bias, self.norm3.eps)


class TransformerCrossEncoder(nn.Module):

    record_attention = False

    def __init__(self, cross_encoder_layer, num_layers, norm=None, return_intermediate=False):
        super().__init__()
        self.layers = nn.ModuleList([copy.deepcopy(cross_encoder_layer) for _ in range(num_layers)])
        self.num_layers = num_layers
        self.norm = norm
        self.return_intermediate = return_intermediate

    def forward_packed(self, x, pos, seg: Segments):
        L = len(self.layers)
        n, d = x.shape
        inter = torch.empty((L if self.return_intermediate else 1, n, d), dtype=x.dtype,
                            device=x.device)
        x = x.clone()
        pending = None
        h1 = side = None
        for l, layer in enumerate(self.layers):
            x, pending = layer.forward_packed(x, pos, seg, pending, h1=h1, side=side,
                                              record=self.record_attention)
            h1 = side = None
            if self.return_intermediate or l == L - 1:
                nxt = self.layers[l + 1] if l + 1 < L else None
                if (nxt is not None and self.norm is not None and pending is None
                        and nxt.takes_side(x, pos) and self.norm.eps == nxt.norm1.eps):
                    side = (self.norm, inter[l if self.return_intermediate else 0])
                elif (nxt is not None and self.norm is not None and pending is None
                        and nxt.wants_h1(x) and self.norm.eps == nxt.norm1.eps):
                    _, h1 = ops.layernorm_dual(x, self.norm, nxt.norm1, add_b=pos,
                                               out_a=inter[l if self.return_intermediate else 0])
                else:
                    self._norm(x, pending, inter[l if self.return_intermediate else 0])
                pending = None
        return inter

    def get_attentions(self):
        if any(l.satt_weights is None or l.xatt_weights is None for l in self.layers):
            raise RuntimeError('no attention maps recorded: set record_attention = True and '
                               'run a forward')
        satt = tuple(torch.stack([l.satt_weights[s] for l in self.layers]) for s in (0, 1))
        xatt = tuple(torch.stack([l.xatt_weights[s] for l in self.layers]) for s in (0, 1))
        return satt, xatt

    def _norm(self, x, pending, out):
        if self.norm is None:
            if pending is not None:
                x.add_(pending)
            out.copy_(x)
            return out
        return ops.layernorm(x, self.norm.weight, self.norm.bias, self.norm.eps,
                             pre_bias=pending, out=out)


class PositionEmbeddingCoordsSine(nn.Module):

    def __init__(self, n_dim=1, d_model=256, temperature=10000, scale=None):
        super().__init__()
        if n_dim != 3:
            raise NotImplementedError('coordinates are 3-D in this path')
        self.n_dim, self.d_model, self.temperature = n_dim, d_model, temperature
        self.scale = 1.0 if scale is None else scale

    def forward(self, xyz):
        return ops.sine_pos_embed(xyz, self.d_model, self.temperature, self.scale)


class PositionEmbeddingLearned(nn.Module):

    def __init__(self, n_dim=3, d_model=256):
        super().__init__()
        if n_dim != 3:
            raise NotImplementedError('coordinates are 3-D in this path')
        self.n_dim, self.d_model = n_dim, d_model
        self.mlp = nn.Sequential(
            nn.Linear(n_dim, 32), nn.ReLU(),
            nn.Linear(32, 64), nn.ReLU(),
            nn.Linear(64, 128), nn.ReLU(),
            nn.Linear(128, 256), nn.ReLU(),
            nn.Linear(256, d_model))

    def _linears(self):
        return [self.mlp[i] for i in (0, 2, 4, 6, 8)]

    def forward(self, xyz):
        ls = self._linears()
        with lin.mode_scope('f16x3'):
            if ops.pos_mlp_supported(xyz.shape[0], self.d_model):
                imgs = [lin.weight_image(m.weight, mode='f16x3') for m in ls[1:]]
                return ops.pos_mlp(xyz, ls[0].weight, ls[0].bias, imgs, [m.bias for m in ls[1:]])
            return self.forward_chain(xyz)

    def forward_chain(self, xyz):
        ls = self._linears()
        h = xyz.contiguous()
        with lin.mode_scope('f16x3'):
            for i, m in enumerate(ls):
                h = lin.linear(h, m.weight, m.bias, act=ops.ACT_RELU if i < 4 else ops.ACT_NONE)
        return h

    def train_forward(self, xyz):
        from .autograd import linear_t
        ls = self._linears()
        h = xyz.contiguous()
        with lin.mode_scope('f16x3'):
            for i, m in enumerate(ls):
                h = linear_t(h, m.weight, m.bias, act=ops.ACT_RELU if i < 4 else ops.ACT_NONE)
        return h


class SinusoidalPositionalEmbedding(nn.Module):

    def __init__(self, d_model):
        super().__init__()
        if d_model % 2 != 0:
            raise ValueError(f'Sinusoidal positional encoding with odd d_model: {d_model}')
        self.d_model = d_model
        div_indices = torch.arange(0, d_model, 2).float()
        self.register_buffer('div_term', torch.exp(div_indices * (-math.log(10000.0) / d_model)))

    def forward(self, emb_indices):
        omegas = emb_indices.reshape(-1, 1) * self.div_term.view(1, -1)
        emb = torch.stack([torch.sin(omegas), torch.cos(omegas)], dim=2)
        return emb.view(*emb_indices.shape, self.d_model).detach()


class GeometricStructureEmbedding(nn.Module):

    def __init__(self, hidden_dim, sigma_d=0.2, sigma_a=15, angle_k=3, reduction_a='max'):
        super().__init__()
        self.sigma_d = sigma_d
        self.sigma_a = sigma_a
        self.factor_a = 180.0 / (self.sigma_a * math.pi)
        self.angle_k = angle_k
        self.hidden_dim = hidden_dim
        self.embedding = SinusoidalPositionalEmbedding(hidden_dim)
        self.proj_d = nn.Linear(hidden_dim, hidden_dim)
        self.proj_a = nn.Linear(hidden_dim, hidden_dim)
        self.reduction_a = reduction_a
        if self.reduction_a not in ['max', 'mean']:
            raise ValueError(f'Unsupported reduction mode: {self.reduction_a}.')

    def _indices(self, xyz, cloud_off, lengths):
        k = self.angle_k
        short = [int(n) for n in lengths if int(n) <= k]
        if short:
            raise ValueError(f'GeometricStructureEmbedding: a cloud of {short[0]} points has no '
                             f'{k} nearest neighbours (angle_k {k} needs more than {k} points)')
        if sum(int(n) for n in lengths) != xyz.shape[0]:
            raise ValueError('GeometricStructureEmbedding: lengths do not sum to the rows of xyz')
        with torch.no_grad():
            return ops.geo_embed_indices(xyz, cloud_off, k, self.sigma_d, self.sigma_a)

    def forward(self, xyz, cloud_off, lengths):
        k, D = self.angle_k, self.hidden_dim
        if not ops.geo_embed_supported(max(xyz.shape[0], 1), D, k):
            return self.forward_composed(xyz, cloud_off, lengths)
        _, d, a = self._indices(xyz, cloud_off, lengths)
        return ops.geo_embed(d, a, self.embedding.div_term,
                             lin.weight_image(self.proj_d.weight, mode='f16x3'), self.proj_d.bias,
                             lin.weight_image(self.proj_a.weight, mode='f16x3'), self.proj_a.bias,
                             ops.GEO_MEAN if self.reduction_a == 'mean' else ops.GEO_MAX)

    def _reduce(self, pd, pa, n):
        k, D = self.angle_k, self.hidden_dim
        pa = pa.view(n, k, k, D)
        pa = pa.max(dim=2)[0] if self.reduction_a == 'max' else pa.mean(dim=2)
        return (pd.view(n, k, D) + pa).max(dim=1)[0]

    def forward_composed(self, xyz, cloud_off, lengths):
        _, d, a = self._indices(xyz, cloud_off, lengths)
        with lin.mode_scope('f16x3'):
            pd = linear(self.embedding(d.reshape(-1)), self.proj_d.weight, self.proj_d.bias)
            pa = linear(self.embedding(a.reshape(-1)), self.proj_a.weight, self.proj_a.bias)
        return self._reduce(pd, pa, xyz.shape[0])

    def train_forward(self, xyz, cloud_off, lengths):
        from .autograd import linear_t
        _, d, a = self._indices(xyz, cloud_off, lengths)
        with lin.mode_scope('f16x3'):
            pd = linear_t(self.embedding(d.reshape(-1)), self.proj_d.weight, self.proj_d.bias)
            pa = linear_t(self.embedding(a.reshape(-1)), self.proj_a.weight, self.proj_a.bias)
        return self._reduce(pd, pa, xyz.shape[0])
```

include/fgreg.h:

```cpp
#ifndef FGREG_H
#define FGREG_H

#include <stddef.h>
#include <stdint.h>

#ifdef __cplusplus
extern "C" {
#endif

#define FGR_ABI_VERSION 2

enum {
    FGR_OK = 0,
    FGR_E_ARG = -1,
    FGR_E_LAUNCH = -2,
    FGR_E_WORKSPACE = -3
};

enum {
    FGR_NB_INDEX = 0,
    FGR_NB_DIST = 1
};

enum { FGR_ACT_NONE = 0, FGR_ACT_LEAKY = 1, FGR_ACT_RELU = 2, FGR_ACT_RELU_RES_LEAKY = 3,
       FGR_ACT_GELU = 4 };

int fgr_abi_version(void);
const char* fgr_last_error(void);

int fgr_time_next_call(void* start_event, void* end_event);

int fgr_grid_subsample_workspace(int64_t n_points, int32_t n_clouds, int64_t max_cells,
                                 size_t* bytes);
int fgr_grid_subsample_count(const float* points, const int64_t* off, int32_t n_clouds,
                             int64_t n_points, float dl, int64_t max_cells, void* ws,
                             size_t ws_bytes, int64_t* counts, void* stream);
int fgr_grid_subsample_fill(int64_t n_points, int32_t n_clouds, int64_t max_cells, int64_t n_out,
                            void* ws, size_t ws_bytes, const float* points, float* out_points,
                            int64_t* out_keys, void* stream);

int fgr_grid_subsample_sparse_workspace(int64_t n_points, int32_t n_clouds, size_t* bytes);
int fgr_grid_subsample_sparse_count(const float* points, const int64_t* off, int32_t n_clouds,
                                    int64_t n_points, float dl, int32_t key_bits, void* ws,
                                    size_t ws_bytes, int64_t* counts, void* stream);
int fgr_grid_subsample_sparse_fill(int64_t n_points, int32_t n_clouds, int64_t n_out, void* ws,
                                   size_t ws_bytes, const float* points, float* out_points,
                                   int64_t* out_keys, void* stream);

int fgr_radius_count(const float* q, const int64_t* q_off, const float* s, const int64_t* s_off,
                     int32_t n_clouds, int64_t nq, int32_t max_q_len, float radius,
                     int32_t* counts, int32_t* max_count, void* stream);
int fgr_radius_search(const float* q, const int64_t* q_off, const float* s, const int64_t* s_off,
                      int32_t n_clouds, int64_t nq, int64_t ns, int32_t max_q_len, float radius,
                      int32_t mode, int32_t width, int64_t* out, void* stream);

int fgr_radius_grid_workspace(int64_t ns, int32_t n_clouds, size_t* bytes);
int fgr_radius_grid_build(const float* s, const int64_t* s_off, int32_t n_clouds, int64_t ns,
                          float radius, void* grid, size_t grid_bytes, void* stream);
int fgr_radius_search_grid(const float* q, const int64_t* q_off, int32_t n_clouds, int64_t nq,
                           int32_t max_q_len, const float* s, const int64_t* s_off, int64_t ns,
                           const void* grid, size_t grid_bytes, float radius, int32_t mode,
                           int32_t width, int64_t* out, int32_t* counts, int32_t* max_count,
                           void* stream);

int fgr_kpconv_gather_workspace(int64_t ns, int32_t cin, size_t* bytes);
int fgr_kpconv_gather(const float* q, const float* s, int64_t nq, int64_t ns, const int64_t* idx,
                      int32_t width, const float* x, int32_t cin, const float* kp, int32_t n_kp,
                      float extent, float* wf, float* nnorm, void* workspace, size_t ws_bytes,
                      void* stream);

#define FGR_KP_LINEAR 0
#define FGR_KP_GAUSSIAN 1
#define FGR_KP_CONSTANT 2
#define FGR_AGG_SUM 0
#define FGR_AGG_CLOSEST 1
int fgr_kpconv_gather_mode(const float* q, const float* s, int64_t nq, int64_t ns,
                           const int64_t* idx, int32_t width, const float* x, int32_t cin,
                           const float* kp, int32_t n_kp, float extent, int32_t influence,
                           int32_t aggregation, float* wf, float* nnorm, void* workspace,
                           size_t ws_bytes, void* stream);

int fgr_kpconv_deform_points(const float* offset_raw, const float* offset_nnorm,
                             const float* offset_bias, const float* kp, int64_t nq, int32_t n_kp,
                             float extent, float* kp_q, float* mod, void* stream);
int fgr_kpconv_gather_deform_workspace(int64_t ns, int32_t cin, size_t* bytes);
int fgr_kpconv_gather_deform(const float* q, const float* s, int64_t nq, int64_t ns,
                             const int64_t* idx, int32_t width, const float* x, int32_t cin,
                             const float* kp_q, const float* mod, int32_t n_kp, float extent,
                             int32_t influence, int32_t aggregation, float* wf, float* nnorm,
                             void* workspace, size_t ws_bytes, void* stream);
int fgr_kpconv_scatter_deform_workspace(int64_t nq, int32_t width, int32_t cin, size_t* bytes);
int fgr_kpconv_scatter_deform(const float* q, const float* s, int64_t nq, int64_t ns,
                              const int64_t* idx, int32_t width, const float* dwf, int32_t cin,
                              const float* kp_q, const float* mod, int32_t n_kp, float extent,
                              int32_t influence, int32_t aggregation, const int32_t* start,
                              const int32_t* pos, float* dx, void* ws, size_t ws_bytes,
                              void* stream);
int fgr_kpconv_deform_grad(const float* q, const float* s, int64_t nq, int64_t ns,
                           const int64_t* idx, int32_t width, const float* x, int32_t cin,
                           const float* dwf, const float* kp_q, const float* mod, int32_t n_kp,
                           float extent, int32_t influence, int32_t aggregation, float* d_kp,
                           float* d_mod, void* stream);

int fgr_max_pool(const float* x, int64_t ns, int32_t c, const int64_t* idx, int64_t nq,
                 int32_t width, float* out, void* stream);

int fgr_instnorm_workspace(int64_t max_seg_len, int32_t c, int32_t n_seg, size_t* bytes);
int fgr_instnorm(const float* x, int64_t n, int32_t c, const int64_t* seg_off, int32_t n_seg,
                 int64_t max_seg_len, const float* row_div, float eps, int32_t act,
                 const float* residual, int32_t post_act, float* out, void* ws, size_t ws_bytes,
                 void* stream);

int fgr_layernorm(float* x, int64_t n, int32_t d, const float* gamma, const float* beta,
                  float eps, const float* add, const float* pre_bias, float* out, void* stream);
int fgr_layernorm_dual(const float* x, int64_t n, int32_t d, const float* gamma,
                       const float* beta, const float* add, float* out, const float* gamma2,
                       const float* beta2, const float* add2, float* out2, float eps,
                       void* stream);

int fgr_add(const float* a, const float* b, int64_t n, float* out, void* stream);

int fgr_gelu_fwd(const float* z, float* y, int64_t n, void* stream);
int fgr_gelu_bwd(const float* z, const float* dy, float* dz, int64_t n, void* stream);

int fgr_sine_pos_embed(const float* xyz, int64_t n, int32_t d_model, float temperature,
                       float scale, float* out, void* stream);

int fgr_res2net_chain6(const float* h, int64_t n, int32_t w, int32_t scale, const void* w_img,
                       const float* bias, const float* x, int32_t cin, float* cat,
                       int64_t ld_cat, void* stream);

int fgr_res2net_chain_h3(const float* h, int64_t n, int32_t w, int32_t scale, const void* w_img,
                         const float* w_scale, const float* bias, const float* x, int32_t cin,
                         float* cat, int64_t ld_cat, void* stream);

int fgr_res2net_block_h3(const float* x, int64_t n, int32_t w, int32_t cin, int32_t scale,
                         const void* w1_img, const float* w1_scale, const float* b1,
                         const void* w_img, const float* w_scale, const float* bias, float* cat,
                         int64_t ld_cat, void* stream);

int fgr_res2net_block6(const float* x, int64_t n, int32_t w, int32_t cin, int32_t scale,
                       const void* w1_img, const float* w1_scale, const float* b1,
                       const void* w_img, const float* bias, float* cat, int64_t ld_cat,
                       void* stream);

int fgr_split_weights_h3_bytes(int32_t n, int32_t k, size_t* bytes);
int fgr_split_weights_h3(const float* w, int32_t n, int32_t k, int64_t stride_n,
                         int64_t stride_k, void* img, void* stream);
typedef struct {
    const float* w;
    void* img;
    int64_t stride_n;
    int64_t stride_k;
    int64_t panel0;
    int32_t n;
    int32_t k;
} fgr_split_desc;
int fgr_split_weights_h3_batch(const void* descs, int32_t count, int64_t total_panels,
                               void* stream);
int fgr_gemm_f16x3(const float* a, int64_t lda, const void* w_img, float* c, int64_t ldc,
                   const float* bias, const float* r, int64_t ldr, int32_t m, int32_t n,
                   int32_t k, int32_t act, void* stream);

int fgr_gemm_workspace(int32_t m, int32_t n, int32_t k, int32_t mode, size_t* bytes);
int fgr_gemm_f16x3_ws(const float* a, int64_t lda, const void* w_img, float* c, int64_t ldc,
                      const float* bias, const float* r, int64_t ldr, int32_t m, int32_t n,
                      int32_t k, int32_t act, void* ws, size_t ws_bytes, void* stream);
int fgr_gemm_bf16_ws(const float* a, int64_t lda, const void* w_img, float* c, int64_t ldc,
                     const float* bias, const float* r, int64_t ldr, int32_t m, int32_t n,
                     int32_t k, int32_t act, void* ws, size_t ws_bytes, void* stream);

int fgr_gemm_f16x3_ln_supported(int32_t m, int32_t n, int32_t k);
int fgr_gemm_f16x3_ln(const float* x, int64_t ldx, const float* gamma, const float* beta,
                      float eps, const float* add, int64_t ld_add, const void* w_img, float* c,
                      int64_t ldc, const float* bias, int32_t m, int32_t n, int32_t k,
                      int32_t act, void* stream);
int fgr_gemm_f16x3_ln_out2(const float* x, int64_t ldx, const float* gamma, const float* beta,
                           float eps, const float* add, int64_t ld_add, const void* w_img,
                           float* c, int64_t ldc, const float* bias, int32_t m, int32_t n,
                           int32_t k, int32_t act, const float* gamma2, const float* beta2,
                           float* out2, int64_t ld_out2, void* stream);

int fgr_split_weights_ffn2_bytes(int32_t n, int32_t k, size_t* bytes);
int fgr_split_weights_ffn2(const float* w, int32_t n, int32_t k, int64_t stride_n,
                           int64_t stride_k, void* img, void* stream);
int fgr_ffn_f16x3_supported(int32_t m, int32_t d, int32_t f);
int fgr_ffn_f16x3(const float* x, int64_t ldx, const float* gamma, const float* beta, float eps,
                  const void* w1_img, const float* b1, const void* w2_img, const float* b2,
                  const float* bound, float* out, int64_t ldo, int32_t m, int32_t d, int32_t f,
                  void* stream);
int fgr_ffn_f16x3_act_supported(int32_t m, int32_t d, int32_t f, int32_t act);
int fgr_ffn_f16x3_act(const float* x, int64_t ldx, const float* gamma, const float* beta,
                      float eps, const void* w1_img, const float* b1, const void* w2_img,
                      const float* b2, const float* bound, float* out, int64_t ldo, int32_t m,
                      int32_t d, int32_t f, int32_t act, void* stream);

int fgr_pos_mlp_f16x3_supported(int64_t n, int32_t d_model);
int fgr_pos_mlp_f16x3(const float* xyz, int64_t n, const float* w0, const float* b0,
                      const void* w1_img, const float* b1, const void* w2_img, const float* b2,
                      const void* w3_img, const float* b3, const void* w4_img, const float* b4,
                      int32_t d_model, float* out, int64_t ldo, void* stream);

#define FGR_GEO_MAX 0
#define FGR_GEO_MEAN 1
int fgr_geo_embed_indices(const float* xyz, int64_t n, const int64_t* cloud_off, int32_t n_clouds,
                          int32_t k, float sigma_d, float factor_a, int32_t* nn, float* d,
                          float* a, void* stream);
int fgr_geo_embed_f16x3_supported(int64_t n, int32_t d_model, int32_t k);
int fgr_geo_embed_f16x3(const float* d, const float* a, int64_t n, int32_t k,
                        const float* div_term, const void* wd_img, const float* bd,
                        const void* wa_img, const float* ba, int32_t d_model, int32_t reduction,
                        float* out, int64_t ldo, void* stream);

int fgr_split_weights_bf16_bytes(int32_t n, int32_t k, size_t* bytes);
int fgr_split_weights_bf16(const float* w, int32_t n, int32_t k, int64_t stride_n,
                           int64_t stride_k, void* img, void* stream);
int fgr_gemm_bf16(const float* a, int64_t lda, const void* w_img, float* c, int64_t ldc,
                  const float* bias, const float* r, int64_t ldr, int32_t m, int32_t n, int32_t k,
                  int32_t act, void* stream);

int fgr_attention(const float* q, int64_t ld_q, const float* k, int64_t ld_k, const float* v,
                  int64_t ld_v, float* o, int64_t ld_o, const int64_t* q_off,
                  const int64_t* kv_off, const int32_t* kv_seg, int32_t n_seg,
                  int32_t max_q_len, int32_t n_head, int32_t head_dim, float scale, void* stream);

int fgr_attention_weights(const float* q, int64_t ld_q, const float* k, int64_t ld_k, float* w,
                          int64_t ld_w, const int64_t* q_off, const int64_t* kv_off,
                          const int32_t* kv_seg, int32_t n_seg, int32_t max_q_len,
                          int32_t max_kv_len, int32_t n_head, int32_t head_dim, float scale,
                          void* stream);

int fgr_attention_f16x3_workspace(int64_t n_kv_rows, int32_t n_kv_seg, int32_t n_head,
                                  size_t* bytes);
int fgr_attention_f16x3(const float* q, int64_t ld_q, const float* k, int64_t ld_k,
                        const float* v, int64_t ld_v, float* o, int64_t ld_o,
                        const int64_t* q_off, const int64_t* kv_off, const int32_t* kv_seg,
                        int32_t n_seg, int32_t n_kv_seg, int64_t n_kv_rows, int32_t max_q_len,
                        int32_t max_kv_len, int32_t n_head, int32_t head_dim, float scale,
                        void* workspace, int64_t ws_bytes, void* stream);

int fgr_attention_bf16_workspace(int64_t n_kv_rows, int32_t n_kv_seg, int32_t n_head,
                                 size_t* bytes);
int fgr_attention_bf16(const float* q, int64_t ld_q, const float* k, int64_t ld_k,
                       const float* v, int64_t ld_v, float* o, int64_t ld_o,
                       const int64_t* q_off, const int64_t* kv_off, const int32_t* kv_seg,
                       int32_t n_seg, int32_t n_kv_seg, int64_t n_kv_rows, int32_t max_q_len,
                       int32_t max_kv_len, int32_t n_head, int32_t head_dim, float scale,
                       void* workspace, int64_t ws_bytes, void* stream);

int fgr_corr_attention(const float* q, int64_t ld_q, const float* k, int64_t ld_k,
                       const float* xyz, float* out, const int64_t* q_off, const int64_t* kv_off,
                       const int32_t* kv_seg, const int64_t* v_off, int32_t n_seg,
                       int32_t max_q_len, int32_t d, float scale, void* stream);

int fgr_corr_topk_workspace(int64_t n_rows, int32_t max_kv_len, size_t* bytes);
int fgr_corr_topk_mask(const float* q, int64_t ld_q, const float* k, int64_t ld_k, float* out,
                       const int64_t* q_off, const int64_t* kv_off, const int32_t* kv_seg,
                       int32_t n_seg, int32_t n_clouds, int64_t n_rows, int32_t max_q_len,
                       int32_t max_kv_len, int32_t d, float scale, int32_t n_top, uint8_t* flags,
                       void* ws, size_t ws_bytes, void* stream);

int fgr_copy_batch(int32_t n, const void* const* src, void* const* dst, const int64_t* bytes,
                   void* stream);

int fgr_lengths_to_offsets(const int64_t* lengths, int32_t n, int64_t* offsets, void* stream);

int fgr_procrustes(const float* a, const float* b, const float* w, int64_t n_batch, int64_t n_pts,
                   float threshold, float* out, void* stream);

int fgr_pair_pose(const float* xyz, const float* corr, const float* logits, int64_t n_tot,
                  const int64_t* seg_off, int32_t n_pairs, int32_t n_layers, float threshold,
                  float* out, void* stream);

int fgr_overlap_pool(const float* prev, int64_t n_prev, const int64_t* idx, int64_t nq,
                     int32_t width, float* out, void* stream);
int fgr_bce_logits_mean(const float* x, int64_t stride_x, const float* y, int64_t n, float* out,
                        void* stream);
int fgr_transform_points(const float* xyz, int64_t n, const int64_t* seg_off, int32_t n_seg,
                         const float* pose, int32_t inverse, float* out, void* stream);
int fgr_infonce_rows(const float* logits, int64_t ld, const float* axyz, const float* pxyz,
                     const int64_t* a_off, const int64_t* p_off, int32_t n_pairs, int64_t n_anchor,
                     float r_p, float r_n, float* row_loss, float* row_mask, void* stream);
int fgr_infonce_rows_bwd(const float* logits, int64_t ld, const float* axyz, const float* pxyz,
                         const int64_t* a_off, const int64_t* p_off, int32_t n_pairs,
                         int64_t n_anchor, int64_t n_cols, float r_n, const float* row_weight,
                         const float* grad, float* dlogits, int64_t ld_d, void* stream);
int fgr_infonce_reduce(const float* row_loss, const float* row_mask, const int64_t* a_off,
                       int32_t n_pairs, float* out, void* stream);
int fgr_circle_loss_workspace(int64_t fd_elems, int64_t n_anchor, int64_t n_pos, size_t* bytes);
int fgr_circle_loss(const float* anchor_feat, const float* pos_feat, int32_t d, const float* axyz,
                    const float* pxyz, const int64_t* a_off, const int64_t* p_off,
                    const int64_t* fd_off, int32_t n_pairs, int64_t n_anchor, int64_t n_pos,
                    int32_t max_anchor, int32_t max_pos, int64_t fd_elems, float r_p, float r_n,
                    void* ws, size_t ws_bytes, float* out, void* stream);
int fgr_pair_cdist(const float* anchor_feat, const float* pos_feat, int32_t d, const int64_t* a_off,
                   const int64_t* p_off, const int64_t* fd_off, int32_t n_pairs, int32_t max_anchor,
                   int32_t max_pos, float* fd, void* stream);
int fgr_corr_loss(const float* xyz, const float* corr, const float* w, const int64_t* seg_off,
                  int32_t n_pairs, const float* pose, float* out, void* stream);
int fgr_se3_compare(const float* pred, const float* gt, int32_t n_layers, int32_t n_pairs,
                    float* rot_deg, float* trans, void* stream);

int fgr_modelnet_metrics_workspace(int32_t n_pairs, int32_t n_pts, size_t* bytes);
int fgr_modelnet_metrics(const float* pred, const float* gt, const float* src, const float* ref,
                         const float* raw, int32_t n_pairs, int32_t n_pts, int32_t n_raw, void* ws,
                         size_t ws_bytes, double* out, void* stream);

int fgr_crop_max_points(int32_t* n_max);
int fgr_crop_pairs_mask(const float* raw, int32_t ld, const int64_t* offsets, int32_t n_pairs,
                        const double* dirs, const int32_t* crop_k, const double* gamma,
                        uint8_t* mask, int32_t* keep, int32_t* count, void* stream);
int fgr_crop_pairs_assemble(const float* raw, int32_t ld, const int64_t* offsets, int32_t n_pairs,
                            const uint8_t* mask, const int32_t* keep, const int32_t* sel,
                            const double* noise, const float* rt, int32_t m, float* xyz,
                            uint8_t* overlap, int64_t* corr, int32_t* n_corr, void* stream);

#define FGR_AUG_PERTURB 1
#define FGR_AUG_SOURCE 2
#define FGR_AUG_CENTRE 4
#define FGR_AUG_SWAP 8
int fgr_augment_workspace_bytes(int64_t n_points, int32_t n_pairs, size_t* bytes);
int fgr_augment_pairs(const float* xyz, int32_t ld, const int64_t* in_off, int64_t n_points,
                      const uint8_t* overlap, const int64_t* corr, int64_t corr_ld,
                      const int64_t* corr_off, const float* pose, const float* perturb,
                      const int32_t* flags, const int32_t* perm, const int64_t* out_off,
                      int32_t max_out, const float* noise, int32_t n_pairs, float* xyz_out,
                      uint8_t* overlap_out, int64_t* corr_out, int32_t* n_corr, float* pose_out,
                      void* ws, size_t ws_bytes, void* stream);

int fgr_kv_image_bytes(int64_t n_rows, int32_t n_head, int32_t head_dim, size_t* bytes);
int fgr_gemm_f16x3_ln_qkv_supported(int32_t m, int32_t d, int32_t n_head);
int fgr_gemm_f16x3_ln_qkv(const float* x, int64_t ldx, const float* gamma, const float* beta,
                          float eps, const float* add, int64_t ld_add, const void* w_img, float* q,
                          int64_t ld_q, const float* bias, int32_t m, int32_t d, int32_t n_head,
                          void* kv_img, const float* gamma2, const float* beta2, float* out2,
                          int64_t ld_out2, void* stream);
int fgr_gemm_f16x3_qkv_supported(int32_t m, int32_t d, int32_t n_head);
int fgr_gemm_f16x3_qkv(const float* a, int64_t lda, const void* w_img, float* q, int64_t ld_q,
                       const float* bias, int32_t m, int32_t d, int32_t n_head, void* kv_img,
                       void* stream);
int fgr_kv_image_bf16_bytes(int64_t n_rows, int32_t n_head, int32_t head_dim, size_t* bytes);
int fgr_gemm_bf16_qkv_supported(int32_t m, int32_t d, int32_t n_head);
int fgr_gemm_bf16_qkv(const float* a, int64_t lda, const void* w_img, float* q, int64_t ld_q,
                      const float* bias, int32_t m, int32_t d, int32_t n_head, void* kv_img,
                      void* stream);
int fgr_attention_bf16_img(const float* q, int64_t ld_q, const void* kv_img, int64_t n_kv_rows,
                           float* o, int64_t ld_o, const int64_t* q_off, const int64_t* kv_off,
                           const int32_t* kv_seg, int32_t n_seg, int32_t max_q_len,
                           int32_t n_head, int32_t head_dim, float scale, void* stream);
int fgr_attention_f16x3_img(const float* q, int64_t ld_q, const void* kv_img, int64_t n_kv_rows,
                            float* o, int64_t ld_o, const int64_t* q_off, const int64_t* kv_off,
                            const int32_t* kv_seg, int32_t n_seg, int32_t max_q_len,
                            int32_t n_head, int32_t head_dim, float scale, void* stream);

int fgr_corr_head_supported(int32_t m, int32_t d);
int fgr_corr_head_f16x3(const float* f, int64_t ldf, int32_t m, int32_t d, const void* w0c_img,
                        const float* b0c, const void* w2_img, const float* b2, const float* w4,
                        const float* b4, float* hidden, float* corr, float* logits, void* stream);

int fgr_nbr_inverse_workspace(int64_t nq, int32_t width, int64_t ns, size_t* bytes);
int fgr_nbr_inverse(const int64_t* idx, int64_t nq, int32_t width, int64_t ns, int32_t* start,
                    int32_t* pos, int32_t* ent, void* ws, size_t ws_bytes, void* stream);
int fgr_kpconv_scatter_workspace(int64_t nq, int32_t width, int32_t cin, size_t* bytes);
int fgr_kpconv_scatter(const float* q, const float* s, int64_t nq, int64_t ns, const int64_t* idx,
                       int32_t width, const float* dwf, int32_t cin, const float* kernel_points,
                       int32_t n_kp, float extent, const int32_t* start, const int32_t* pos,
                       float* dx, void* ws, size_t ws_bytes, void* stream);
int fgr_kpconv_scatter_mode(const float* q, const float* s, int64_t nq, int64_t ns,
                            const int64_t* idx, int32_t width, const float* dwf, int32_t cin,
                            const float* kernel_points, int32_t n_kp, float extent,
                            int32_t influence, int32_t aggregation, const int32_t* start,
                            const int32_t* pos, float* dx, void* ws, size_t ws_bytes,
                            void* stream);
int fgr_max_pool_bwd_workspace(int64_t nq, int32_t c, size_t* bytes);
int fgr_max_pool_bwd(const float* x, int64_t ns, int32_t c, const int64_t* idx, int64_t nq,
                     int32_t width, const float* dy, const int32_t* start, const int32_t* ent,
                     float* dx, void* ws, size_t ws_bytes, void* stream);
int fgr_corr_attention_bwd_workspace(int64_t n_rows, size_t* bytes);
int fgr_corr_attention_bwd(const float* q, int64_t ld_q, const float* k, int64_t ld_k,
                           const float* xyz, const float* dout, float* dq, int64_t ld_dq, float* dk,
                           int64_t ld_dk, const int64_t* q_off, const int64_t* kv_off,
                           const int32_t* kv_seg, const int64_t* v_off, int32_t n_seg,
                           int32_t n_kv_seg, int64_t n_rows, int32_t max_q_len, int32_t max_kv_len,
                           int32_t d, float scale, void* ws, size_t ws_bytes, void* stream);
int fgr_segnorm_workspace(int64_t max_seg_len, int32_t c, int32_t n_seg, size_t* bytes);
int fgr_segnorm_stats(const float* x, int64_t n, int32_t c, const int64_t* seg_off, int32_t n_seg,
                      int64_t max_seg_len, const float* row_div, float eps, float* mean, float* rstd,
                      float* var, void* ws, size_t ws_bytes, void* stream);
int fgr_segnorm_apply(const float* x, int64_t n, int32_t c, const int64_t* seg_off, int32_t n_seg,
                      const float* row_div, const float* mean, const float* rstd, const float* gamma,
                      const float* beta, int32_t act, const float* residual, int32_t post_act,
                      float* out, void* stream);
int fgr_segnorm_fwd(const float* x, int64_t n, int32_t c, const int64_t* seg_off, int32_t n_seg,
                    int64_t max_seg_len, const float* row_div, float eps, float* mean, float* rstd,
                    float* var, const float* gamma, const float* beta, int32_t act,
                    const float* residual, int32_t post_act, float* out, void* ws, size_t ws_bytes,
                    void* stream);
int fgr_segnorm_bwd(const float* x, int64_t n, int32_t c, const int64_t* seg_off, int32_t n_seg,
                    int64_t max_seg_len, const float* row_div, const float* mean, const float* rstd,
                    const float* gamma, const float* beta, int32_t act, int32_t has_residual,
                    int32_t post_act, const float* y, const float* dy, float* dx, float* dres,
                    float* dgamma, float* dbeta, void* ws, size_t ws_bytes, void* stream);
int fgr_colsum_workspace(int64_t n, int32_t c, size_t* bytes);
int fgr_colsum(const float* x, int64_t n, int32_t c, int64_t ldx, float* out, void* ws,
               size_t ws_bytes, void* stream);
int fgr_layernorm_bwd_workspace(int64_t n, int32_t d, size_t* bytes);
int fgr_layernorm_bwd(const float* x, int64_t n, int32_t d, const float* gamma, float eps,
                      const float* dy, float* dx, float* dgamma_dbeta, void* ws, size_t ws_bytes,
                      void* stream);
int fgr_attention_bwd_workspace(int64_t nq, int32_t nhead, size_t* bytes);
int fgr_attention_bwd(const float* q, int64_t ldq, const float* k, int64_t ldk, const float* v,
                      int64_t ldv, const float* o, int64_t ldo, const float* dout, int64_t lddo,
                      float* dq, int64_t lddq, float* dk, int64_t lddk, float* dv, int64_t lddv,
                      const int64_t* q_off, const int64_t* kv_off, const int32_t* kv_seg,
                      int32_t n_seg, int32_t n_kv_seg, int64_t nq, int64_t max_q_len,
                      int64_t max_kv_len, int32_t nhead, int32_t dh, float scale, void* ws,
                      size_t ws_bytes, void* stream);
int fgr_attention_f16x3_drop(const float* q, int64_t ld_q, const float* k, int64_t ld_k,
                             const float* v, int64_t ld_v, float* o, int64_t ld_o,
                             const int64_t* q_off, const int64_t* kv_off, const int32_t* kv_seg,
                             int32_t n_seg, int32_t n_kv_seg, int64_t n_kv_rows, int32_t max_q_len,
                             int32_t max_kv_len, int32_t n_head, int32_t head_dim, float scale,
                             void* workspace, int64_t ws_bytes, uint32_t seed, float p,
                             void* stream);
int fgr_attention_f16x3_train(const float* q, int64_t ld_q, const float* k, int64_t ld_k,
                              const float* v, int64_t ld_v, float* o, int64_t ld_o,
                              const int64_t* q_off, const int64_t* kv_off, const int32_t* kv_seg,
                              int32_t n_seg, int32_t n_kv_seg, int64_t n_kv_rows, int32_t max_q_len,
                              int32_t max_kv_len, int32_t n_head, int32_t head_dim, float scale,
                              void* workspace, int64_t ws_bytes, uint32_t seed, float p, float* lse,
                              void* stream);
int fgr_attention_bwd_train(const float* q, int64_t ldq, const float* k, int64_t ldk,
                            const float* v, int64_t ldv, const float* o, int64_t ldo,
                            const float* dout, int64_t lddo, float* dq, int64_t lddq, float* dk,
                            int64_t lddk, float* dv, int64_t lddv, const int64_t* q_off,
                            const int64_t* kv_off, const int32_t* kv_seg, int32_t n_seg,
                            int32_t n_kv_seg, int64_t nq, int64_t max_q_len, int64_t max_kv_len,
                            int32_t nhead, int32_t dh, float scale, void* ws, size_t ws_bytes,
                            uint32_t seed, float p, const float* lse, int64_t n_kv_rows,
                            void* stream);
int fgr_attention_bwd_train_workspace(int64_t nq, int32_t n_seg, int64_t n_kv_rows,
                                      int32_t n_kv_seg, int32_t nhead, int32_t dh, size_t* bytes);
int fgr_attention_bwd_drop(const float* q, int64_t ldq, const float* k, int64_t ldk,
                           const float* v, int64_t ldv, const float* o, int64_t ldo,
                           const float* dout, int64_t lddo, float* dq, int64_t lddq, float* dk,
                           int64_t lddk, float* dv, int64_t lddv, const int64_t* q_off,
                           const int64_t* kv_off, const int32_t* kv_seg, int32_t n_seg,
                           int32_t n_kv_seg, int64_t nq, int64_t max_q_len, int64_t max_kv_len,
                           int32_t nhead, int32_t dh, float scale, void* ws, size_t ws_bytes,
                           uint32_t seed, float p, void* stream);

int fgr_gemm_wgrad_workspace(int64_t rows, int32_t m, int32_t n, int32_t with_bias, size_t* bytes);
int fgr_gemm_f16x3_wgrad(const float* dy, int64_t ld_dy, const float* x, int64_t ld_x,
                         int64_t rows, int32_t m, int32_t n, float* dw, int64_t ld_dw, float* db,
                         void* ws, size_t ws_bytes, void* stream);

int fgr_icp_workspace(int64_t n_src_tot, int64_t n_tgt_tot, int32_t n_pairs, size_t* bytes);
int fgr_icp(const float* src, const int64_t* src_off, int64_t n_src_tot, const float* tgt,
            const int64_t* tgt_off, int64_t n_tgt_tot, int32_t n_pairs, int32_t max_src_len,
            const float* pose_in, float max_dist, int32_t max_iters, float rel_fitness,
            float rel_rmse, void* ws, size_t ws_bytes, float* pose_out, float* fitness,
            float* rmse, int32_t* n_iters, void* stream);
int fgr_registration_score(const float* src, const int64_t* src_off, int64_t n_src_tot,
                           const float* tgt, const int64_t* tgt_off, int64_t n_tgt_tot,
                           int32_t n_pairs, int32_t max_src_len, const float* pose,
                           float max_dist, void* ws, size_t ws_bytes, float* fitness, float* rmse,
                           int32_t* idx, float* d2, double* info, void* stream);

#ifdef __cplusplus
}
#endif
#endif
```

Baseline: 3297 pairs/s.

## Fuse attention out-projection with residual into the FFN kernel

Adds a PROJ variant of the FFN kernel that first computes the attention out-projection GEMM plus bias and residual for its row block. It writes the result to the output and to LDS, then runs the LayerNorm, FFN1 and FFN2 stages from that LDS copy. This removes a separate kernel launch and the global round trip of the intermediate x. The shared weight-streaming helpers are moved into a common header so gemm_ws and ffn can both use them. The cost is more LDS and register pressure in the FFN kernel and a serialized projection phase before the FFN pipeline starts.

```diff
diff --git a/boosting-fine-grained-feature-fusion-in-3d-point-cloud-registration_amd/csrc/ffn.hip b/boosting-fine-grained-feature-fusion-in-3d-point-cloud-registration_amd/csrc/ffn.hip
--- a/boosting-fine-grained-feature-fusion-in-3d-point-cloud-registration_amd/csrc/ffn.hip
+++ b/boosting-fine-grained-feature-fusion-in-3d-point-cloud-registration_amd/csrc/ffn.hip
@@ -1,7 +1,7 @@
 #include <algorithm>
 #include <cstdlib>
 
-#include "mfma.h"
+#include "ws_parts.h"
 
 namespace fgr {
 namespace {
@@ -23,6 +23,8 @@
     const float* bound;
     float* out; int64_t ldo;
     int M, F;
+    const float* o; int64_t ld_o;
+    const u32x4* wo; const float* wosc; const float* bo;
 };
 
 __device__ __forceinline__ void wait_units(int n) {
@@ -326,16 +328,20 @@
     return sz * (t > 0.927734375f ? tail : mid);
 }
 
-template <int RT, int ACT = FGR_ACT_RELU>
+template <int RT, int ACT = FGR_ACT_RELU, bool PROJ = false>
 __global__ void __launch_bounds__(256, 1) ffn_nsplit_kernel(FfnArgs p) {
     static_assert(RT >= 1 && RT <= 4, "row tiles");
     static_assert(ACT == FGR_ACT_RELU || ACT == FGR_ACT_GELU, "activation");
+    static_assert(kFfnKS == kWsKS, "the front stage's image is the ws kernels'");
     __shared__ u32x4 act[RT * kFfnKS * 2 * 64];
     __shared__ u32x4 hbuf[2][4][RT][2][64];
     __shared__ float4 cw1[kFfnMaxF / 4], cb1[kFfnMaxF / 4];
     __shared__ float4 cw2[kFfnD / 4], cb2[kFfnD / 4];
     __shared__ float4 lng[kFfnD / 4], lnb[kFfnD / 4];
     __shared__ float2 rowpar[64];
+    __shared__ float4 cwo[PROJ ? kFfnD / 4 : 1], cbo[PROJ ? kFfnD / 4 : 1];
+    __shared__ float rowrs[PROJ ? 64 : 1];
+    static_assert(sizeof(hbuf) == 16 * RT * kFfnD * sizeof(float), "hbuf holds the block's fp32 rows");
 
     constexpr int BR = 16 * RT;
     const int nbm = (p.M + BR - 1) / BR;
@@ -356,43 +362,108 @@
     const float4 pb2 = reinterpret_cast<const float4*>(p.b2)[t4];
     const float4 pg = reinterpret_cast<const float4*>(p.ln_g)[t4];
     const float4 pbe = reinterpret_cast<const float4*>(p.ln_b)[t4];
+    float4 pwo = make_float4(0.f, 0.f, 0.f, 0.f), pbo = pwo;
+    if constexpr (PROJ) {
+        pwo = reinterpret_cast<const float4*>(p.wosc)[t4];
+        pbo = reinterpret_cast<const float4*>(p.bo)[t4];
+    }
     __builtin_amdgcn_sched_barrier(0);
     float xr[kFfnKS][8];
+    const int rl = 16 * min(wv, RT - 1) + c;
     {
-        const int64_t row = min(r0 + 16 * min(wv, RT - 1) + c, p.M - 1);
-        const float* ar = p.x + row * p.ldx;
+        const int64_t row = min(r0 + rl, p.M - 1);
+        ws_load_row(PROJ ? p.o + row * p.ld_o : p.x + row * p.ldx, g, xr);
+    }
+    const float bM1 = p.bound[0], bMb = p.bound[1];
+    if constexpr (PROJ) {
+        float4 rres[RT][4];
+#pragma unroll
+        for (int rt = 0; rt < RT; ++rt) {
+            const int64_t orow = min(r0 + 16 * rt + c, p.M - 1);
+#pragma unroll
+            for (int q = 0; q < 4; ++q)
+                rres[rt][q] = *reinterpret_cast<const float4*>(p.x + orow * p.ldx + 16 * (4 * wv + q) + 4 * g);
+        }
+        __builtin_amdgcn_sched_barrier(0);
+        u32x4 wring[kWsRing][8];
+#pragma unroll
+        for (int G = 0; G < kWsRing - 1; ++G) ws_issue_group(p.wo, 4 * wv, G, lane, wring[G]);
+        __builtin_amdgcn_sched_barrier(0);
+        if (tid < nf4) { cw1[tid] = pw1a; cb1[tid] = pb1a; }
+        if (tid + 256 < nf4) { cw1[tid + 256] = pw1b; cb1[tid + 256] = pb1b; }
+        if (tid < kFfnD / 4) {
+            cw2[tid] = pw2; cb2[tid] = pb2; lng[tid] = pg; lnb[tid] = pbe;
+            cwo[tid] = pwo; cbo[tid] = pbo;
+        }
+        {
+            const int e = row_scale_exp(ws_row_absmax(xr));
+            if (wv < RT) {
+                ws_write_image(xr, __builtin_ldexpf(1.f, e), wv, lane, act);
+                if (g == 0) rowrs[16 * wv + c] = __builtin_ldexpf(1.f, -e);
+            }
+        }
+        wait_lgkm0();
+        __builtin_amdgcn_s_barrier();
+        f32x4 acco[RT][4];
+#pragma unroll
+        for (int rt = 0; rt < RT; ++rt)
+#pragma unroll
+            for (int q = 0; q < 4; ++q) acco[rt][q] = f32x4{0.f, 0.f, 0.f, 0.f};
+        ws_pass<RT>(p.wo, 4 * wv, lane, act, wring, acco);
+        float4* xs = reinterpret_cast<float4*>(&hbuf[0][0][0][0][0]);
+        float4 xp[RT][4];
+#pragma unroll
+        for (int rt = 0; rt < RT; ++rt) {
+            const float rs = rowrs[16 * rt + c];
+#pragma unroll
+            for (int q = 0; q < 4; ++q) {
+                const int u = 4 * (4 * wv + q) + g;
+                const float4 ws = cwo[u], bv = cbo[u];
+                const f32x4 a = acco[rt][q];
+                xp[rt][q] = make_float4(
+                    finish_ct<FGR_ACT_NONE, true>(a[0] * (rs * ws.x), bv.x, rres[rt][q].x),
+                    finish_ct<FGR_ACT_NONE, true>(a[1] * (rs * ws.y), bv.y, rres[rt][q].y),
+                    finish_ct<FGR_ACT_NONE, true>(a[2] * (rs * ws.z), bv.z, rres[rt][q].z),
+                    finish_ct<FGR_ACT_NONE, true>(a[3] * (rs * ws.w), bv.w, rres[rt][q].w));
+            }
+        }
+        __builtin_amdgcn_sched_barrier(0);
+#pragma unroll
+        for (int rt = 0; rt < RT; ++rt)
+#pragma unroll
+            for (int q = 0; q < 4; ++q) {
+                const int u = 4 * (4 * wv + q) + g;
+                xs[(16 * rt + c) * (kFfnD / 4) + (u ^ c)] = xp[rt][q];
+            }
+#pragma unroll
+        for (int rt = 0; rt < RT; ++rt) {
+            const int rr = r0 + 16 * rt + c;
+            if (rr < p.M) {
+#pragma unroll
+                for (int q = 0; q < 4; ++q)
+                    *reinterpret_cast<float4*>(p.out + (int64_t)rr * p.ldo + 16 * (4 * wv + q) + 4 * g) = xp[rt][q];
+            }
+        }
+        __builtin_amdgcn_sched_barrier(0);
+        wait_lgkm0();
+        __builtin_amdgcn_s_barrier();
 #pragma unroll
         for (int s = 0; s < kFfnKS; ++s) {
-            const float4 a0 = *reinterpret_cast<const float4*>(ar + 32 * s + 8 * g);
-            const float4 a1 = *reinterpret_cast<const float4*>(ar + 32 * s + 8 * g + 4);
+            const float4 a0 = xs[rl * (kFfnD / 4) + ((8 * s + 2 * g) ^ c)];
+            const float4 a1 = xs[rl * (kFfnD / 4) + ((8 * s + 2 * g + 1) ^ c)];
             xr[s][0] = a0.x; xr[s][1] = a0.y; xr[s][2] = a0.z; xr[s][3] = a0.w;
             xr[s][4] = a1.x; xr[s][5] = a1.y; xr[s][6] = a1.z; xr[s][7] = a1.w;
         }
-    }
-    {
+    } else {
         if (tid < nf4) { cw1[tid] = pw1a; cb1[tid] = pb1a; }
         if (tid + 256 < nf4) { cw1[tid + 256] = pw1b; cb1[tid + 256] = pb1b; }
         if (tid < kFfnD / 4) { cw2[tid] = pw2; cb2[tid] = pb2; lng[tid] = pg; lnb[tid] = pbe; }
-    }
-    const float bM1 = p.bound[0], bMb = p.bound[1];
-    __syncthreads();
+        __syncthreads();
+    }
 
     {
-        float sm = 0.f;
-#pragma unroll
-        for (int s = 0; s < kFfnKS; ++s)
-            sm += ((xr[s][0] + xr[s][1]) + (xr[s][2] + xr[s][3])) +
-                  ((xr[s][4] + xr[s][5]) + (xr[s][6] + xr[s][7]));
-        const float mean = xg_sum(sm) / (float)kFfnD;
-        float sq = 0.f;
-#pragma unroll
-        for (int s = 0; s < kFfnKS; ++s)
-#pragma unroll
-            for (int e = 0; e < 8; ++e) {
-                const float d = xr[s][e] - mean;
-                sq += d * d;
-            }
-        const float rstd = 1.0f / sqrtf(xg_sum(sq) / (float)kFfnD + p.eps);
+        float mean, rstd;
+        ws_ln_stats(xr, p.eps, mean, rstd);
         float mx = 0.f, nn = 0.f;
 #pragma unroll
         for (int s = 0; s < kFfnKS; ++s) {
@@ -429,7 +500,12 @@
         if (g == 0 && wv < RT)
             rowpar[16 * wv + c] = make_float2(__builtin_ldexpf(1.f, eh - ea), __builtin_ldexpf(1.f, eh));
     }
-    __syncthreads();
+    if constexpr (PROJ) {
+        wait_lgkm0();
+        __builtin_amdgcn_s_barrier();
+    } else {
+        __syncthreads();
+    }
 
     auto issue = [&](int st, int j, u32x4 (&slot)[4]) {
         if (j < 8) {
@@ -571,7 +647,7 @@
         const int rr = r0 + 16 * rt + c;
         const int64_t row = min(rr, p.M - 1);
         const float inv_s = 1.f / rowpar[16 * rt + c].y;
-        const float* xrow = p.x + row * p.ldx;
+        const float* xrow = PROJ ? p.out + row * p.ldo : p.x + row * p.ldx;
         float4 res[4];
 #pragma unroll
         for (int q = 0; q < 4; ++q) res[q] = *reinterpret_cast<const float4*>(xrow + 16 * (4 * wv + q) + 4 * g);
@@ -717,3 +793,66 @@
     FGR_CHECK_LAUNCH("ffn_f16x3_kernel");
     return FGR_OK;
 }
+
+extern "C" int fgr_ffn_f16x3_proj_supported(int32_t m, int32_t d, int32_t f, int32_t act) {
+    return (fgr_ffn_f16x3_act_supported(m, d, f, act) && f % 128 == 0) ? 1 : 0;
+}
+
+namespace {
+bool rows_overlap(const float* a, int64_t lda, const float* b, int64_t ldb, int m, int d) {
+    if (m <= 0) return false;
+    const float* ae = a + (size_t)(m - 1) * lda + d;
+    const float* be = b + (size_t)(m - 1) * ldb + d;
+    return a < be && b < ae;
+}
+}
+
+extern "C" int fgr_ffn_f16x3_proj(const float* o, int64_t ld_o, const void* wo_img, const float* bo,
+                                  const float* x, int64_t ldx, const float* gamma,
+                                  const float* beta, float eps, const void* w1_img,
+                                  const float* b1, const void* w2_img, const float* b2,
+                                  const float* bound, float* out, int64_t ldo, int32_t m,
+                                  int32_t d, int32_t f, int32_t act, void* stream) {
+    FGR_REQUIRE(act == FGR_ACT_RELU || act == FGR_ACT_GELU,
+                "fgr_ffn_f16x3_proj: act %d (FGR_ACT_RELU or FGR_ACT_GELU)", act);
+    FGR_REQUIRE(o && wo_img && bo && x && gamma && beta && w1_img && b1 && w2_img && b2 && bound &&
+                    out && m >= 0 && d > 0 && ld_o >= d && ldx >= d && ldo >= d && eps >= 0.f,
+                "fgr_ffn_f16x3_proj: bad arguments");
+    FGR_REQUIRE(fgr_ffn_f16x3_proj_supported(m > 0 ? m : 1, d, f, act),
+                "fgr_ffn_f16x3_proj: d %d, hidden %d, act %d not supported "
+                "(fgr_ffn_f16x3_proj_supported)", d, f, act);
+    const uintptr_t al = reinterpret_cast<uintptr_t>(o) | reinterpret_cast<uintptr_t>(wo_img) |
+                         reinterpret_cast<uintptr_t>(bo) | reinterpret_cast<uintptr_t>(x) |
+                         reinterpret_cast<uintptr_t>(gamma) | reinterpret_cast<uintptr_t>(beta) |
+                         reinterpret_cast<uintptr_t>(w1_img) | reinterpret_cast<uintptr_t>(b1) |
+                         reinterpret_cast<uintptr_t>(w2_img) | reinterpret_cast<uintptr_t>(b2) |
+                         reinterpret_cast<uintptr_t>(out);
+    FGR_REQUIRE((al & 15) == 0 && ld_o % 4 == 0 && ldx % 4 == 0 && ldo % 4 == 0,
+                "fgr_ffn_f16x3_proj: operands must be 16-B aligned with row strides %% 4 == 0");
+    FGR_REQUIRE((out == x && ldo == ldx) || !rows_overlap(out, ldo, x, ldx, m, d),
+                "fgr_ffn_f16x3_proj: out overlaps x partially");
+    FGR_REQUIRE(!rows_overlap(out, ldo, o, ld_o, m, d), "fgr_ffn_f16x3_proj: out overlaps o");
+    if (m == 0) return FGR_OK;
+    hipStream_t st = as_stream(stream);
+    TimedCall timed_(st);
+    const char* io = static_cast<const char*>(wo_img);
+    const char* i1 = static_cast<const char*>(w1_img);
+    const char* i2 = static_cast<const char*>(w2_img);
+    FfnArgs a{x, ldx, gamma, beta, eps,
+              (const u32x4*)i1, (const float*)(i1 + (size_t)(f / 16) * kFfnKS * 128 * 16), b1,
+              (const u32x4*)i2, (const float*)(i2 + ffn_image_bytes(d, f)), b2,
+              bound, out, ldo, m, f,
+              o, ld_o, (const u32x4*)io, (const float*)(io + (size_t)(kFfnD / 16) * kWsPanelU * 16), bo};
+    const bool rt3 = (m + 47) / 48 <= kCusFfn && (m + 63) / 64 < kCusFfn;
+    if (act == FGR_ACT_GELU)
+        hipLaunchKernelGGL((ffn_nsplit_kernel<3, FGR_ACT_GELU, true>), dim3((unsigned)((m + 47) / 48)),
+                           dim3(256), 0, st, a);
+    else if (rt3)
+        hipLaunchKernelGGL((ffn_nsplit_kernel<3, FGR_ACT_RELU, true>), dim3((unsigned)((m + 47) / 48)),
+                           dim3(256), 0, st, a);
+    else
+        hipLaunchKernelGGL((ffn_nsplit_kernel<4, FGR_ACT_RELU, true>), dim3((unsigned)((m + 63) / 64)),
+                           dim3(256), 0, st, a);
+    FGR_CHECK_LAUNCH("ffn_nsplit_kernel (proj)");
+    return FGR_OK;
+}
diff --git a/boosting-fine-grained-feature-fusion-in-3d-point-cloud-registration_amd/csrc/gemm_ws.hip b/boosting-fine-grained-feature-fusion-in-3d-point-cloud-registration_amd/csrc/gemm_ws.hip
--- a/boosting-fine-grained-feature-fusion-in-3d-point-cloud-registration_amd/csrc/gemm_ws.hip
+++ b/boosting-fine-grained-feature-fusion-in-3d-point-cloud-registration_amd/csrc/gemm_ws.hip
@@ -1,16 +1,9 @@
-#include "mfma.h"
+#include "ws_parts.h"
 
 
 namespace fgr {
 namespace {
 
-constexpr int kWsKS = 8;
-constexpr int kWsPanelU = kWsKS * 128;
-#ifndef FGR_WS_RING
-#define FGR_WS_RING 3
-#endif
-constexpr int kWsRing = FGR_WS_RING;
-static_assert(kWsRing >= 2 && kWsRing <= 8, "vmcnt holds at most 63");
 constexpr int kKvUnitsWs = 1024;
 constexpr int kKvUnitVWs = 512;
 
@@ -25,15 +18,6 @@
     const float* g2; const float* b2; float* out2; int64_t ld_out2;
     char* kv_img; int2* kv_sc; int n_head, kv_col0;
 };
-
-__device__ __forceinline__ void wait_groups_ws(int n) {
-    switch (n) {
-        case 0: wait_vm<0>(); break;   case 1: wait_vm<8>(); break;
-        case 2: wait_vm<16>(); break;  case 3: wait_vm<24>(); break;
-        case 4: wait_vm<32>(); break;  case 5: wait_vm<40>(); break;
-        case 6: wait_vm<48>(); break;  default: wait_vm<56>(); break;
-    }
-}
 
 template <int NPW, int LNM, bool KV, bool RES, int ACT, int RT, int NPART>
 __global__ void __launch_bounds__(256) __attribute__((amdgpu_waves_per_eu((NPART > 1 && !RES) ? 2 : 1)))
@@ -87,24 +71,8 @@
     float xr[kWsKS][8];
     float dr[LNM >= 2 ? kWsKS : 1][8];
     {
-        const float* ar = p.A + row * p.lda;
-#pragma unroll
-        for (int s = 0; s < kWsKS; ++s) {
-            const float4 a0 = *reinterpret_cast<const float4*>(ar + 32 * s + 8 * g);
-            const float4 a1 = *reinterpret_cast<const float4*>(ar + 32 * s + 8 * g + 4);
-            xr[s][0] = a0.x; xr[s][1] = a0.y; xr[s][2] = a0.z; xr[s][3] = a0.w;
-            xr[s][4] = a1.x; xr[s][5] = a1.y; xr[s][6] = a1.z; xr[s][7] = a1.w;
-        }
-        if constexpr (LNM >= 2) {
-            const float* dp = p.add + row * p.ld_add;
-#pragma unroll
-            for (int s = 0; s < kWsKS; ++s) {
-                const float4 d0 = *reinterpret_cast<const float4*>(dp + 32 * s + 8 * g);
-                const float4 d1 = *reinterpret_cast<const float4*>(dp + 32 * s + 8 * g + 4);
-                dr[s][0] = d0.x; dr[s][1] = d0.y; dr[s][2] = d0.z; dr[s][3] = d0.w;
-                dr[s][4] = d1.x; dr[s][5] = d1.y; dr[s][6] = d1.z; dr[s][7] = d1.w;
-            }
-        }
+        ws_load_row(p.A + row * p.lda, g, xr);
+        if constexpr (LNM >= 2) ws_load_row(p.add + row * p.ld_add, g, dr);
     }
     float4 rres[kResEarly ? RT : 1][4];
     if constexpr (kResEarly) {
@@ -119,12 +87,7 @@
     }
     __builtin_amdgcn_sched_barrier(0);
     auto issue = [&](int G, u32x4 (&slot)[8]) {
-        const int pass = G / kWsKS, s = G % kWsKS;
-#pragma unroll
-        for (int e = 0; e < 8; ++e) {
-            const int pp = e >> 1, tt = e & 1;
-            slot[e] = p.W[(int64_t)(pw0 + 4 * pass + pp) * kWsPanelU + (s * 2 + tt) * 64 + lane];
-        }
+        ws_issue_group(p.W, pw0 + 4 * (G / kWsKS), G % kWsKS, lane, slot);
     };
     constexpr int NG = NPASS * kWsKS;
     u32x4 ring[kWsRing][8];
@@ -143,21 +106,8 @@
         if constexpr (LNM == 3)
             if (tid < 64) { lng2[tid] = lpg2; lnb2[tid] = lpb2; }
         __syncthreads();
-        float sm = 0.f;
-#pragma unroll
-        for (int s = 0; s < kWsKS; ++s)
-            sm += ((xr[s][0] + xr[s][1]) + (xr[s][2] + xr[s][3])) +
-                  ((xr[s][4] + xr[s][5]) + (xr[s][6] + xr[s][7]));
-        const float mean = xg_sum(sm) / 256.f;
-        float sq = 0.f;
-#pragma unroll
-        for (int s = 0; s < kWsKS; ++s)
-#pragma unroll
-            for (int e = 0; e < 8; ++e) {
-                const float d = xr[s][e] - mean;
-                sq += d * d;
-            }
-        const float rstd = 1.0f / sqrtf(xg_sum(sq) / 256.f + p.eps);
+        float mean, rstd;
+        ws_ln_stats(xr, p.eps, mean, rstd);
         ln_mean = mean;
         ln_rstd = rstd;
         if (kSideLds && wv < RT) {
@@ -188,37 +138,17 @@
         }
     }
     {
-        float mx = 0.f;
-#pragma unroll
-        for (int s = 0; s < kWsKS; ++s) {
-            mx = fmaxf(mx, max3_abs(xr[s][0], xr[s][1], xr[s][2]));
-            mx = fmaxf(mx, max3_abs(xr[s][3], xr[s][4], xr[s][5]));
-            mx = fmaxf(mx, max3_abs(xr[s][6], xr[s][7], 0.f));
-        }
-        mx = xg_max(mx);
-        const int e = row_scale_exp(mx);
+        const int e = row_scale_exp(ws_row_absmax(xr));
         const float sc = __builtin_ldexpf(1.f, e);
         if (wv < RT) {
-#pragma unroll
-            for (int s = 0; s < kWsKS; ++s) {
-                u32x4 h, l;
-                split8_f16(xr[s], sc, h, l);
-                act[((wv * kWsKS + s) * 2 + 0) * 64 + lane] = h;
-                act[((wv * kWsKS + s) * 2 + 1) * 64 + lane] = l;
-            }
+            ws_write_image(xr, sc, wv, lane, act);
             if (g == 0) rowrs[16 * wv + c] = __builtin_ldexpf(1.f, -e);
         }
     }
     wait_lgkm0();
     __builtin_amdgcn_s_barrier();
 
-    auto read_act = [&](int s, u32x4 (&f)[2 * RT]) {
-#pragma unroll
-        for (int rt = 0; rt < RT; ++rt) {
-            f[2 * rt + 0] = act[((rt * kWsKS + s) * 2 + 0) * 64 + lane];
-            f[2 * rt + 1] = act[((rt * kWsKS + s) * 2 + 1) * 64 + lane];
-        }
-    };
+    auto read_act = [&](int s, u32x4 (&f)[2 * RT]) { ws_read_act<RT>(act, s, lane, f); };
     u32x4 fa[2][2 * RT];
     u32x4 fin[NPASS][RT][4];
     int kv_e[NPASS][2];
@@ -243,19 +173,7 @@
             if (s + 1 < kWsKS) read_act(s + 1, fa[(s + 1) & 1]);
             __builtin_amdgcn_sched_group_barrier(0x020, 8, 0);
             if (s + 1 < kWsKS) __builtin_amdgcn_sched_group_barrier(0x100, 2 * RT, 0);
-#pragma unroll
-            for (int rt = 0; rt < RT; ++rt) {
-                const f16x8 ah = __builtin_bit_cast(f16x8, cur[2 * rt + 0]);
-                const f16x8 al = __builtin_bit_cast(f16x8, cur[2 * rt + 1]);
-#pragma unroll
-                for (int pp = 0; pp < 4; ++pp) {
-                    const f16x8 wh = __builtin_bit_cast(f16x8, wf[2 * pp]);
-                    const f16x8 wl = __builtin_bit_cast(f16x8, wf[2 * pp + 1]);
-                    acc[rt][pp] = __builtin_amdgcn_mfma_f32_16x16x32_f16(wl, ah, acc[rt][pp], 0, 0, 0);
-                    acc[rt][pp] = __builtin_amdgcn_mfma_f32_16x16x32_f16(wh, al, acc[rt][pp], 0, 0, 0);
-                    acc[rt][pp] = __builtin_amdgcn_mfma_f32_16x16x32_f16(wh, ah, acc[rt][pp], 0, 0, 0);
-                }
-            }
+            ws_mfma_group<RT>(wf, cur, acc);
             __builtin_amdgcn_sched_group_barrier(0x008, 12 * RT, 0);
             __builtin_amdgcn_sched_barrier(0);
         }
diff --git a/boosting-fine-grained-feature-fusion-in-3d-point-cloud-registration_amd/csrc/ws_parts.h b/boosting-fine-grained-feature-fusion-in-3d-point-cloud-registration_amd/csrc/ws_parts.h
--- /dev/null
+++ b/boosting-fine-grained-feature-fusion-in-3d-point-cloud-registration_amd/csrc/ws_parts.h
@@ -0,0 +1,129 @@
+#pragma once
+#include "mfma.h"
+
+namespace fgr {
+
+constexpr int kWsKS = 8;
+constexpr int kWsPanelU = kWsKS * 128;
+#ifndef FGR_WS_RING
+#define FGR_WS_RING 3
+#endif
+constexpr int kWsRing = FGR_WS_RING;
+static_assert(kWsRing >= 2 && kWsRing <= 8, "vmcnt holds at most 63");
+
+__device__ __forceinline__ void wait_groups_ws(int n) {
+    switch (n) {
+        case 0: wait_vm<0>(); break;   case 1: wait_vm<8>(); break;
+        case 2: wait_vm<16>(); break;  case 3: wait_vm<24>(); break;
+        case 4: wait_vm<32>(); break;  case 5: wait_vm<40>(); break;
+        case 6: wait_vm<48>(); break;  default: wait_vm<56>(); break;
+    }
+}
+
+__device__ __forceinline__ void ws_load_row(const float* ar, int g, float (&xr)[kWsKS][8]) {
+#pragma unroll
+    for (int s = 0; s < kWsKS; ++s) {
+        const float4 a0 = *reinterpret_cast<const float4*>(ar + 32 * s + 8 * g);
+        const float4 a1 = *reinterpret_cast<const float4*>(ar + 32 * s + 8 * g + 4);
+        xr[s][0] = a0.x; xr[s][1] = a0.y; xr[s][2] = a0.z; xr[s][3] = a0.w;
+        xr[s][4] = a1.x; xr[s][5] = a1.y; xr[s][6] = a1.z; xr[s][7] = a1.w;
+    }
+}
+
+__device__ __forceinline__ void ws_ln_stats(const float (&xr)[kWsKS][8], float eps, float& mean,
+                                            float& rstd) {
+    float sm = 0.f;
+#pragma unroll
+    for (int s = 0; s < kWsKS; ++s)
+        sm += ((xr[s][0] + xr[s][1]) + (xr[s][2] + xr[s][3])) +
+              ((xr[s][4] + xr[s][5]) + (xr[s][6] + xr[s][7]));
+    mean = xg_sum(sm) / 256.f;
+    float sq = 0.f;
+#pragma unroll
+    for (int s = 0; s < kWsKS; ++s)
+#pragma unroll
+        for (int e = 0; e < 8; ++e) {
+            const float d = xr[s][e] - mean;
+            sq += d * d;
+        }
+    rstd = 1.0f / sqrtf(xg_sum(sq) / 256.f + eps);
+}
+
+__device__ __forceinline__ float ws_row_absmax(const float (&xr)[kWsKS][8]) {
+    float mx = 0.f;
+#pragma unroll
+    for (int s = 0; s < kWsKS; ++s) {
+        mx = fmaxf(mx, max3_abs(xr[s][0], xr[s][1], xr[s][2]));
+        mx = fmaxf(mx, max3_abs(xr[s][3], xr[s][4], xr[s][5]));
+        mx = fmaxf(mx, max3_abs(xr[s][6], xr[s][7], 0.f));
+    }
+    return xg_max(mx);
+}
+
+__device__ __forceinline__ void ws_write_image(const float (&xr)[kWsKS][8], float sc, int tile,
+                                               int lane, u32x4* act) {
+#pragma unroll
+    for (int s = 0; s < kWsKS; ++s) {
+        u32x4 h, l;
+        split8_f16(xr[s], sc, h, l);
+        act[((tile * kWsKS + s) * 2 + 0) * 64 + lane] = h;
+        act[((tile * kWsKS + s) * 2 + 1) * 64 + lane] = l;
+    }
+}
+
+template <int RT>
+__device__ __forceinline__ void ws_read_act(const u32x4* act, int s, int lane, u32x4 (&f)[2 * RT]) {
+#pragma unroll
+    for (int rt = 0; rt < RT; ++rt) {
+        f[2 * rt + 0] = act[((rt * kWsKS + s) * 2 + 0) * 64 + lane];
+        f[2 * rt + 1] = act[((rt * kWsKS + s) * 2 + 1) * 64 + lane];
+    }
+}
+
+__device__ __forceinline__ void ws_issue_group(const u32x4* W, int panel0, int s, int lane,
+                                               u32x4 (&slot)[8]) {
+#pragma unroll
+    for (int e = 0; e < 8; ++e) {
+        const int pp = e >> 1, tt = e & 1;
+        slot[e] = W[(int64_t)(panel0 + pp) * kWsPanelU + (s * 2 + tt) * 64 + lane];
+    }
+}
+
+template <int RT>
+__device__ __forceinline__ void ws_mfma_group(const u32x4 (&wf)[8], const u32x4 (&cur)[2 * RT],
+                                              f32x4 (&acc)[RT][4]) {
+#pragma unroll
+    for (int rt = 0; rt < RT; ++rt) {
+        const f16x8 ah = __builtin_bit_cast(f16x8, cur[2 * rt + 0]);
+        const f16x8 al = __builtin_bit_cast(f16x8, cur[2 * rt + 1]);
+#pragma unroll
+        for (int pp = 0; pp < 4; ++pp) {
+            const f16x8 wh = __builtin_bit_cast(f16x8, wf[2 * pp]);
+            const f16x8 wl = __builtin_bit_cast(f16x8, wf[2 * pp + 1]);
+            acc[rt][pp] = __builtin_amdgcn_mfma_f32_16x16x32_f16(wl, ah, acc[rt][pp], 0, 0, 0);
+            acc[rt][pp] = __builtin_amdgcn_mfma_f32_16x16x32_f16(wh, al, acc[rt][pp], 0, 0, 0);
+            acc[rt][pp] = __builtin_amdgcn_mfma_f32_16x16x32_f16(wh, ah, acc[rt][pp], 0, 0, 0);
+        }
+    }
+}
+
+template <int RT>
+__device__ __forceinline__ void ws_pass(const u32x4* W, int panel0, int lane, const u32x4* act,
+                                        u32x4 (&ring)[kWsRing][8], f32x4 (&acc)[RT][4]) {
+    u32x4 fa[2][2 * RT];
+    ws_read_act<RT>(act, 0, lane, fa[0]);
+#pragma unroll
+    for (int s = 0; s < kWsKS; ++s) {
+        if (s + kWsRing - 1 < kWsKS)
+            ws_issue_group(W, panel0, s + kWsRing - 1, lane, ring[(s + kWsRing - 1) % kWsRing]);
+        wait_groups_ws(kWsKS - 1 - s < kWsRing - 1 ? kWsKS - 1 - s : kWsRing - 1);
+        if (s + 1 < kWsKS) ws_read_act<RT>(act, s + 1, lane, fa[(s + 1) & 1]);
+        __builtin_amdgcn_sched_group_barrier(0x020, 8, 0);
+        if (s + 1 < kWsKS) __builtin_amdgcn_sched_group_barrier(0x100, 2 * RT, 0);
+        ws_mfma_group<RT>(ring[s % kWsRing], fa[s & 1], acc);
+        __builtin_amdgcn_sched_group_barrier(0x008, 12 * RT, 0);
+        __builtin_amdgcn_sched_barrier(0);
+    }
+}
+
+}
diff --git a/boosting-fine-grained-feature-fusion-in-3d-point-cloud-registration_amd/fgreg/_lib.py b/boosting-fine-grained-feature-fusion-in-3d-point-cloud-registration_amd/fgreg/_lib.py
--- a/boosting-fine-grained-feature-fusion-in-3d-point-cloud-registration_amd/fgreg/_lib.py
+++ b/boosting-fine-grained-feature-fusion-in-3d-point-cloud-registration_amd/fgreg/_lib.py
@@ -87,6 +87,9 @@
     'fgr_ffn_f16x3_act_supported': [_i32, _i32, _i32, _i32],
     'fgr_ffn_f16x3_act': [_vp, _i64, _vp, _vp, _f32, _vp, _vp, _vp, _vp, _vp, _vp, _i64, _i32,
                           _i32, _i32, _i32, _vp],
+    'fgr_ffn_f16x3_proj_supported': [_i32, _i32, _i32, _i32],
+    'fgr_ffn_f16x3_proj': [_vp, _i64, _vp, _vp, _vp, _i64, _vp, _vp, _f32, _vp, _vp, _vp, _vp,
+                           _vp, _vp, _i64, _i32, _i32, _i32, _i32, _vp],
     'fgr_gelu_fwd': [_vp, _vp, _i64, _vp],
     'fgr_gelu_bwd': [_vp, _vp, _vp, _i64, _vp],
     'fgr_pos_mlp_f16x3_supported': [_i64, _i32],
diff --git a/boosting-fine-grained-feature-fusion-in-3d-point-cloud-registration_amd/fgreg/ops.py b/boosting-fine-grained-feature-fusion-in-3d-point-cloud-registration_amd/fgreg/ops.py
--- a/boosting-fine-grained-feature-fusion-in-3d-point-cloud-registration_amd/fgreg/ops.py
+++ b/boosting-fine-grained-feature-fusion-in-3d-point-cloud-registration_amd/fgreg/ops.py
@@ -910,6 +910,40 @@
     return out
 
 
+PROJ_FUSE = True
+
+
+def ffn_proj_supported(m, d, f, act=ACT_RELU) -> bool:
+    return (PROJ_FUSE and FFN_FUSE
+            and bool(_lib.load().fgr_ffn_f16x3_proj_supported(m, d, f, act)))
+
+
+def ffn_proj(o, wo_img, bo, x, norm, w1_img, b1, w2_img, b2, bound, out=None,
+             act=ACT_RELU) -> torch.Tensor:
+    _dev(o, bo, x, b1, b2, bound)
+    m, d = x.shape
+    f = b1.numel()
+    assert o.shape == x.shape and bo.numel() == d and b2.numel() == d
+    assert x.dtype == torch.float32 and o.dtype == torch.float32
+    assert x.stride(1) == 1 and o.stride(1) == 1
+
+    def rows(t):
+        return t if (t.stride(0) % 4 == 0 and t.data_ptr() % 16 == 0) else t.contiguous()
+
+    x, o = rows(x), rows(o)
+    g, b = norm.weight.contiguous(), norm.bias.contiguous()
+    bo, b1, b2, bound = bo.contiguous(), b1.contiguous(), b2.contiguous(), bound.contiguous()
+    if out is None:
+        out = torch.empty((m, d), dtype=torch.float32, device=x.device)
+    t0 = _begin('gemm', ('ffn', m, d, f))
+    _lib.check(_lib.load().fgr_ffn_f16x3_proj(
+        _ptr(o), o.stride(0), _ptr(wo_img.img), _ptr(bo), _ptr(x), x.stride(0), _ptr(g), _ptr(b),
+        float(norm.eps), _ptr(w1_img.img), _ptr(b1), _ptr(w2_img.img), _ptr(b2), _ptr(bound),
+        _ptr(out), out.stride(0), m, d, f, int(act), _stream()), 'fgr_ffn_f16x3_proj')
+    _end('gemm', t0, 2 * m * d * d + 4 * m * d * f)
+    return out
+
+
 def gelu(z, out=None) -> torch.Tensor:
     _dev(z, out)
     assert z.dtype == torch.float32 and z.is_contiguous()
diff --git a/boosting-fine-grained-feature-fusion-in-3d-point-cloud-registration_amd/fgreg/transformer.py b/boosting-fine-grained-feature-fusion-in-3d-point-cloud-registration_amd/fgreg/transformer.py
--- a/boosting-fine-grained-feature-fusion-in-3d-point-cloud-registration_amd/fgreg/transformer.py
+++ b/boosting-fine-grained-feature-fusion-in-3d-point-cloud-registration_amd/fgreg/transformer.py
@@ -184,6 +184,18 @@
                              seg.cross_seg, record=rec)
         if rec is not None:
             self._store_maps(rec, seg)
+        f = self.linear1.out_features
+        if (rec is None and lin.MODE == 'f16x3' and ops.ATTN_MODE == 'f16x3' and fuse_in
+                and self.ca_val_has_pos_emb and pos is not None
+                and ops.ln_qkv_supported(n, d, self.nhead)
+                and ops.ffn_supported(n, d, f, self.act)
+                and ops.ffn_proj_supported(n, d, f, self.act)):
+            op = self.multihead_attn.out_proj
+            return ops.ffn_proj(o, lin.weight_image(op.weight, mode='f16x3'), op.bias, x,
+                                self.norm3, lin.weight_image(self.linear1.weight, mode='f16x3'),
+                                self.linear1.bias,
+                                lin.weight_image(self.linear2.weight, mode='ffn2'),
+                                self.linear2.bias, self._ffn_bound(), act=self.act), None
         x = linear(o, self.multihead_attn.out_proj.weight, self.multihead_attn.out_proj.bias,
                    residual=x)
         if lin.MODE == 'f16x3' and ops.ffn_supported(n, d, self.linear1.out_features, self.act):
diff --git a/include/fgreg.h b/include/fgreg.h
--- a/include/fgreg.h
+++ b/include/fgreg.h
@@ -194,6 +194,12 @@
                       float eps, const void* w1_img, const float* b1, const void* w2_img,
                       const float* b2, const float* bound, float* out, int64_t ldo, int32_t m,
                       int32_t d, int32_t f, int32_t act, void* stream);
+int fgr_ffn_f16x3_proj_supported(int32_t m, int32_t d, int32_t f, int32_t act);
+int fgr_ffn_f16x3_proj(const float* o, int64_t ld_o, const void* wo_img, const float* bo,
+                       const float* x, int64_t ldx, const float* gamma, const float* beta,
+                       float eps, const void* w1_img, const float* b1, const void* w2_img,
+                       const float* b2, const float* bound, float* out, int64_t ldo, int32_t m,
+                       int32_t d, int32_t f, int32_t act, void* stream);
 
 int fgr_pos_mlp_f16x3_supported(int64_t n, int32_t d_model);
 int fgr_pos_mlp_f16x3(const float* xyz, int64_t n, const float* w0, const float* b0,
```

Result: no change. 3300 pairs/s (median of 3 runs) (+0.1%).
